# sdu-zyx/Multi-modal-Food-Recommendation

Hardware: NVIDIA B200
Metric: train_epochs_per_s (higher is better)
Workload: dtype f32

## Files before the change

### include/foodrec_b200.h

```cpp
#ifndef FOODREC_B200_H
#define FOODREC_B200_H

#include <stdint.h>

#ifdef __cplusplus
extern "C" {
#endif

#define FR_OK 0
#define FR_EINVAL (-1)
#define FR_EUNSUPPORTED (-2)
#define FR_ECUDA (-3)

#define FR_SPMM_SEG 128

int fr_version(void);
const char *fr_last_error(void);
int64_t fr_launch_count(void);
int fr_profile_enable(int on);
int fr_profile_dump(char *buf, int64_t cap);

int fr_spmm_plan_sizes(const int32_t *row_ptr_host, int32_t n_rows, int32_t seg_len, int64_t *n_seg,
                       int64_t *n_long, int64_t *n_part);
int fr_spmm_plan_fill(const int32_t *row_ptr_host, int32_t n_rows, int32_t seg_len, int32_t *seg_host,
                      int32_t *long_rows_host);
int fr_spmm_csr_f32(const int32_t *seg, int64_t n_seg, const int32_t *long_rows, int64_t n_long,
                    const int32_t *col_idx, const float *val, int32_t d, const float *X, const float *Z,
                    float alpha, float beta, const float *bias, int32_t act, float *Y, float *partial,
                    int32_t *counters, void *stream);

int fr_spmm_csr_f32_split(const int32_t *seg, int64_t n_seg, const int32_t *long_rows, int64_t n_long,
                          const int32_t *col_idx, const float *val, int32_t d, const float *X0, const float *X1,
                          int32_t x_split, const float *Z0, const float *Z1, int32_t z_split, float alpha, float beta,
                          const float *bias, int32_t act, float *Y, float *partial, int32_t *counters, void *stream);

int fr_spmm_csr_f32_masked(const int32_t *seg, int64_t n_seg, const int32_t *long_rows, int64_t n_long,
                           const int32_t *col_idx, const float *val, int32_t d, const float *X, const float *Z,
                           float alpha, float beta, float *Y, float *partial, int32_t *counters, const uint8_t *x_mask,
                           uint8_t *y_mask, void *stream);

#define FR_SPMM_MAX_TASKS 4
typedef struct fr_spmm_task {
    const int32_t *seg;
    int64_t n_seg;
    const int32_t *long_rows;
    int64_t n_long;
    const int32_t *col_idx;
    const float *val;
    const float *X0, *X1;
    int32_t x_split;
    const float *Z0, *Z1;
    int32_t z_split;
    float alpha, beta;
    float *Y, *partial;
    int32_t *counters;
} fr_spmm_task;
int64_t fr_spmm_task_blocks(int64_t n_seg);
int fr_spmm_csr_f32_grouped(const fr_spmm_task *tasks_host, int32_t n_tasks, int32_t d, const int32_t *blk_map,
                            int64_t n_blocks, void *stream);

#define FR_MAX_REG_GROUPS 6
int64_t fr_rank_loss_ws_floats(void);
int fr_rank_loss_fwd(const float *emb, int32_t d, int64_t item_off, const int64_t *u, const int64_t *p,
                     const int64_t *n, int32_t B, float gamma, int32_t n_groups,
                     const float *const *reg_tab_host, const int64_t *const *reg_idx_host,
                     const int64_t *reg_cnt_host, float reg_den, float *out, float *coef, float *gnorm,
                     float *ws, void *stream);
int fr_rank_loss_bwd(const float *emb, int32_t d, int64_t item_off, const int64_t *u, const int64_t *p,
                     const int64_t *n, int32_t B, const float *coef, const float *g_out, float *d_emb,
                     int32_t n_groups, const float *const *reg_tab_host, const int64_t *const *reg_idx_host,
                     const int64_t *reg_cnt_host, const int64_t *reg_pad_host, float reg_den,
                     const float *gnorm, float *const *d_tab_host, uint8_t *emb_mask ,
                     void *stream);

int fr_bpr_scores_fwd(const float *pos, const float *neg, int64_t n, float gamma, float *out, float *coef, void *stream);
int fr_l2_norm_f32(const float *x, int64_t n, float *out, void *stream);

int fr_csr_from_coo(const int64_t *coo_rows, int64_t nnz, int32_t n_rows, int32_t *row_ptr, int32_t *scratch,
                    void *stream);

int fr_sum_rows(const float *const *tab_host, int32_t n_tabs, int32_t d, int64_t rows, float *out, void *stream);
int fr_spread_rows(const float *g, int32_t d, int64_t rows, float *const *d_tab_host, const int64_t *rows_total_host,
                   int32_t n_tabs, int32_t accumulate ,
                   const uint8_t *src_mask ,
                   uint8_t *const *mask_host , void *stream);

int fr_gather_rows(const float *tab, int32_t d, const int64_t *idx, int64_t n, float *out, void *stream);
int fr_scatter_add_rows(const float *g, int32_t d, const int64_t *idx, int64_t n, float *d_tab, void *stream);
int fr_pair_scores(const float *user_tab, const float *item_tab, int32_t d, const int64_t *user,
                   const int64_t *item, int64_t n, float *scores, void *stream);

int64_t fr_dcor_ws_floats(int32_t n);
int fr_dcor_fwd(const float *const *tab_host, int32_t V, int32_t d, const int64_t *idx, int32_t n,
                const int32_t *pairs_host, int32_t P, float scale, float *Dm, float *rowmean, float *out ,
                float *dfds, float *gm, float *ws, void *stream);
int fr_dcor_bwd(const float *const *tab_host, int32_t V, int32_t d, const int64_t *idx, int32_t n,
                const int32_t *pairs_host, int32_t P, const float *Dm, const float *rowmean,
                const float *dfds, const float *gm, const float *g_out, float *const *d_tab_host,
                uint8_t *const *mask_host ,
                float *ws , void *stream);
int64_t fr_dcor_bwd_ws_floats(int32_t n);

int fr_f32_to_bf16(const float *x, void *y_bf16, int64_t rows, int32_t d, int32_t l2_normalise, void *stream);
int64_t fr_gemm_topk_ws_bytes(int32_t M);
int fr_gemm_topk_bf16(const void *A_bf16, int32_t M, const void *B_bf16, int32_t N, int32_t K, float scale,
                      const float *bias, const int64_t *row_ids, const int64_t *hist_ptr, const int32_t *hist_idx,
                      int32_t topk, float *out_val, int32_t *out_idx, void *ws, int64_t ws_bytes, void *stream);
int fr_max_row_norm(const float *B, int64_t rows, int32_t d, float *out , void *stream);
int fr_rescore_topk_f32(const float *A, const int64_t *a_rows, const float *B, int32_t d, float scale,
                        const float *bias, int32_t metric , const int32_t *cand,
                        const float *cand_val, int32_t kc, int32_t M, int32_t k, float *out_val, void *out_idx,
                        int32_t idx64, const float *bmax, uint8_t *cert, void *stream);
int fr_exact_topk_f32(const float *A, const int64_t *a_rows, int32_t Mf, const float *B, int32_t N, int32_t d,
                      float scale, const float *bias, int32_t metric, const int64_t *hist_rows,
                      const int64_t *hist_ptr, const int32_t *hist_idx, int32_t k, float *scores_ws, float *out_val,
                      int64_t *out_idx, void *stream);
int64_t fr_exact_topk_thr_ws_bytes(int32_t Mf);
int fr_exact_topk_thr_f32(const float *A, const int64_t *a_rows, int32_t Mf, const float *B, int32_t N, int32_t d,
                          float scale, const float *bias, int32_t metric, const int64_t *hist_rows,
                          const int64_t *hist_ptr, const int32_t *hist_idx, int32_t k, const float *thr, void *ws,
                          float *out_val, int64_t *out_idx, int32_t *overflow, void *stream);

int fr_cosine_mean_fwd(const float *A, const float *T, const int64_t *idx, int64_t n, int32_t d, float *out, float *cosv,
                       float *na, float *nt, void *stream);
int fr_cosine_mean_bwd(const float *A, const float *T, const int64_t *idx, int64_t n, int32_t d, const float *cosv,
                       const float *na, const float *nt, const float *g_out, float *dA, float *dT, void *stream);

int64_t fr_infonce_ws_floats(int32_t n);
int fr_infonce_fwd(const float *hidden, int32_t b, int32_t d, float temperature, int32_t normalise, float *hn,
                   float *norm, float *G, float *lse, float *out, float *ws, void *stream);
int fr_infonce_bwd(const float *hn, const float *norm, const float *G, const float *lse, int32_t b, int32_t d,
                   float temperature, int32_t normalise, const float *g_out, float *d_hidden, void *stream);

int fr_schgn_attend(const float *user_key, const float *user_comp, int32_t nu, const int32_t *codes, int32_t slots,
                    const int32_t *nums, int32_t n_items, const float *ingre_key, const float *ingre_final,
                    const float *ingre_comp, const float *img_key, const float *comp_keys, const float *h_ingre,
                    const float *h_comp, int32_t d, float *att, float *logits, void *stream);
int fr_schgn_score(const float *user_final, const float *user_hidden, int32_t nu, const float *W_item,
                   const float *W_prod, const float *w_out, const float *comps, const float *att, const float *logits,
                   int32_t n_items, int32_t d, float *scores, void *stream);
int64_t fr_schgn_score_topk_ws_bytes(int32_t nu, int32_t n_items, int32_t k);
int fr_schgn_score_topk(const float *user_final, const float *user_hidden, int32_t nu, const float *W_item,
                        const float *W_prod, const float *w_out, const float *comps, const float *att, const float *logits,
                        int32_t n_items, int32_t d, const int64_t *user_ids, const int64_t *hist_ptr,
                        const int32_t *hist_idx, int32_t k, void *ws, float *out_val, int64_t *out_idx, void *stream);
#define FR_PAIRS_BAD_PTR 1
#define FR_PAIRS_BAD_ITEM 2
int64_t fr_schgn_attend_pairs_ws_bytes(int32_t nu, int64_t n_pairs, int32_t n_items);
int fr_schgn_attend_pairs(const float *user_key, const float *user_comp, int32_t nu, const int64_t *ptr,
                          const int32_t *items, int64_t n_pairs, const int32_t *codes, int32_t slots, const int32_t *nums,
                          int32_t n_items, const float *ingre_key, const float *ingre_final, const float *ingre_comp,
                          const float *img_key, const float *comp_keys, const float *h_ingre, const float *h_comp,
                          int32_t d, void *ws, int64_t ws_bytes, float *att, float *logits, int32_t *status,
                          void *stream);
int fr_schgn_score_pairs(const float *user_final, const float *user_hidden, int32_t nu, const int64_t *ptr,
                         const int32_t *items, int64_t n_pairs, const float *W_item, const float *W_prod,
                         const float *w_out, const float *comps, const float *att, const float *logits, int32_t n_items,
                         int32_t d, float *scores, void *stream);

int fr_comm_version(void);
int fr_comm_unique_id(void *id128);
int fr_comm_init(const void *id128, int32_t rank, int32_t world, void **comm);
int fr_comm_destroy(void *comm);
int fr_allgather_rows(void *comm, const float *x_local, int64_t rows_per_rank, int32_t d, float *x_full, void *stream);
int fr_reduce_scatter_rows(void *comm, const float *g_full, int64_t rows_per_rank, int32_t d, float *g_local, void *stream);
int fr_peer_alloc(int64_t bytes, void **ptr, void *handle64);
int fr_peer_open(const void *handle64, void **ptr);
int fr_peer_close(void *ptr);
int fr_peer_free(void *ptr);
int fr_push_rows(const float *src, int64_t rows, int32_t d, float *const *peers_host, int32_t n_peers, int64_t row_off,
                 void *stream);
int fr_spmm_csr_f32_push(const int32_t *seg, int64_t n_seg, const int32_t *long_rows, int64_t n_long,
                         const int32_t *col_idx, const float *val, int32_t d, const float *X, const float *Z, float alpha,
                         float beta, float *Y, float *partial, int32_t *counters, float *const *peers_host,
                         int32_t n_peers, int64_t row_off, void *stream);

#define FR_ADAM_MAX_TENSORS 64
typedef struct fr_adam_tensor {
    float *param;
    const float *grad;
    float *exp_avg;
    float *exp_avg_sq;
    int64_t n;
} fr_adam_tensor;
int fr_adam_step(const fr_adam_tensor *tensors_host, int32_t n_tensors, double lr, double beta1, double beta2, double eps,
                 int32_t *step_dev, float *scalars_dev, void *stream);

int fr_probe_gather(const float *tab, int32_t d, const int32_t *idx, int64_t n_idx, int32_t inflight, int32_t blocks,
                    float *out, void *stream);

int fr_sample_negatives(const int64_t *excl_ptr, const int32_t *excl_idx, const int64_t *users, int64_t n,
                        int32_t n_items, uint64_t seed, uint64_t step, int64_t *out_neg, int32_t *fail_count,
                        void *stream);

#define FR_EVAL_MAX_CUTOFFS 8
#define FR_TOPK_METRICS 5
int64_t fr_eval_metrics_ws_bytes(void);
int fr_topk_metrics(const void *top, int32_t idx64, int64_t n, int32_t K, const int64_t *pos_ptr, const int32_t *pos_idx,
                    const int32_t *pos_len, const int32_t *cutoffs_host, int32_t n_cut, const float *disc,
                    const float *ideal, double *sums, double *per_user, void *ws, void *stream);
int fr_by_user_metrics(const float *scores, const int64_t *ptr, const int32_t *n_pos, int64_t n, int32_t neg_num,
                       const int32_t *cutoffs_host, int32_t n_cut, double *sums, double *per_user, void *ws,
                       void *stream);

#ifdef __cplusplus
}
#endif
#endif
```

### multi-modal-food-recommendation_b200/_lib.py

```python
from __future__ import annotations

import ctypes as C
import os

_HERE = os.path.dirname(os.path.abspath(__file__))
LIB_PATH = os.path.join(_HERE, "libfoodrec_b200.so")


class FoodRecError(RuntimeError):
    pass


def _load():
    if not os.path.exists(LIB_PATH):
        raise FoodRecError(
            f"{LIB_PATH} is not built: run `make` (or `python -c 'import __graft_entry__ as g; g.build()'`) "
            "at the repo root. foodrec_b200 has no CPU or eager fallback.")
    import torch
    return C.CDLL(LIB_PATH, mode=C.RTLD_GLOBAL)


lib = _load()

_p, _i32, _i64, _f32 = C.c_void_p, C.c_int32, C.c_int64, C.c_float

SIGNATURES = {
    "fr_version": (C.c_int, []),
    "fr_last_error": (C.c_char_p, []),
    "fr_launch_count": (_i64, []),
    "fr_profile_enable": (C.c_int, [C.c_int]),
    "fr_profile_dump": (C.c_int, [C.c_char_p, _i64]),
    "fr_spmm_plan_sizes": (C.c_int, [_p, _i32, _i32, C.POINTER(_i64), C.POINTER(_i64), C.POINTER(_i64)]),
    "fr_spmm_plan_fill": (C.c_int, [_p, _i32, _i32, _p, _p]),
    "fr_spmm_csr_f32": (C.c_int, [_p, _i64, _p, _i64, _p, _p, _i32, _p, _p, _f32, _f32, _p, _i32, _p, _p, _p, _p]),
    "fr_spmm_csr_f32_split": (C.c_int, [_p, _i64, _p, _i64, _p, _p, _i32, _p, _p, _i32, _p, _p, _i32, _f32, _f32, _p, _i32,
                                        _p, _p, _p, _p]),
    "fr_spmm_task_blocks": (_i64, [_i64]),
    "fr_spmm_csr_f32_grouped": (C.c_int, [_p, _i32, _i32, _p, _i64, _p]),
    "fr_adam_step": (C.c_int, [_p, _i32, C.c_double, C.c_double, C.c_double, C.c_double, _p, _p, _p]),
    "fr_rank_loss_ws_floats": (_i64, []),
    "fr_rank_loss_fwd": (C.c_int, [_p, _i32, _i64, _p, _p, _p, _i32, _f32, _i32, _p, _p, _p, _f32, _p, _p, _p, _p, _p]),
    "fr_rank_loss_bwd": (C.c_int, [_p, _i32, _i64, _p, _p, _p, _i32, _p, _p, _p, _i32, _p, _p, _p, _p, _f32, _p, _p, _p, _p]),
    "fr_bpr_scores_fwd": (C.c_int, [_p, _p, _i64, _f32, _p, _p, _p]),
    "fr_l2_norm_f32": (C.c_int, [_p, _i64, _p, _p]),
    "fr_spmm_csr_f32_masked": (C.c_int, [_p, _i64, _p, _i64, _p, _p, _i32, _p, _p, _f32, _f32, _p, _p, _p, _p, _p, _p]),
    "fr_dcor_ws_floats": (_i64, [_i32]),
    "fr_dcor_fwd": (C.c_int, [_p, _i32, _i32, _p, _i32, _p, _i32, _f32, _p, _p, _p, _p, _p, _p, _p]),
    "fr_sum_rows": (C.c_int, [_p, _i32, _i32, _i64, _p, _p]),
    "fr_spread_rows": (C.c_int, [_p, _i32, _i64, _p, _p, _i32, _i32, _p, _p, _p]),
    "fr_dcor_bwd": (C.c_int, [_p, _i32, _i32, _p, _i32, _p, _i32, _p, _p, _p, _p, _p, _p, _p, _p, _p]),
    "fr_dcor_bwd_ws_floats": (_i64, [_i32]),
    "fr_f32_to_bf16": (C.c_int, [_p, _p, _i64, _i32, _i32, _p]),
    "fr_gemm_topk_ws_bytes": (_i64, [_i32]),
    "fr_gemm_topk_bf16": (C.c_int, [_p, _i32, _p, _i32, _i32, _f32, _p, _p, _p, _p, _i32, _p, _p, _p, _i64, _p]),
    "fr_max_row_norm": (C.c_int, [_p, _i64, _i32, _p, _p]),
    "fr_rescore_topk_f32": (C.c_int, [_p, _p, _p, _i32, _f32, _p, _i32, _p, _p, _i32, _i32, _i32, _p, _p, _i32, _p, _p, _p]),
    "fr_exact_topk_f32": (C.c_int, [_p, _p, _i32, _p, _i32, _i32, _f32, _p, _i32, _p, _p, _p, _i32, _p, _p, _p, _p]),
    "fr_exact_topk_thr_ws_bytes": (_i64, [_i32]),
    "fr_exact_topk_thr_f32": (C.c_int, [_p, _p, _i32, _p, _i32, _i32, _f32, _p, _i32, _p, _p, _p, _i32, _p, _p, _p, _p, _p, _p]),
    "fr_csr_from_coo": (C.c_int, [_p, _i64, _i32, _p, _p, _p]),
    "fr_cosine_mean_fwd": (C.c_int, [_p, _p, _p, _i64, _i32, _p, _p, _p, _p, _p]),
    "fr_cosine_mean_bwd": (C.c_int, [_p, _p, _p, _i64, _i32, _p, _p, _p, _p, _p, _p, _p]),
    "fr_infonce_ws_floats": (_i64, [_i32]),
    "fr_infonce_fwd": (C.c_int, [_p, _i32, _i32, _f32, _i32, _p, _p, _p, _p, _p, _p, _p]),
    "fr_infonce_bwd": (C.c_int, [_p, _p, _p, _p, _i32, _i32, _f32, _i32, _p, _p, _p]),
    "fr_gather_rows": (C.c_int, [_p, _i32, _p, _i64, _p, _p]),
    "fr_scatter_add_rows": (C.c_int, [_p, _i32, _p, _i64, _p, _p]),
    "fr_pair_scores": (C.c_int, [_p, _p, _i32, _p, _p, _i64, _p, _p]),
    "fr_comm_version": (C.c_int, []),
    "fr_comm_unique_id": (C.c_int, [_p]),
    "fr_comm_init": (C.c_int, [_p, _i32, _i32, _p]),
    "fr_comm_destroy": (C.c_int, [_p]),
    "fr_allgather_rows": (C.c_int, [_p, _p, _i64, _i32, _p, _p]),
    "fr_reduce_scatter_rows": (C.c_int, [_p, _p, _i64, _i32, _p, _p]),
    "fr_peer_alloc": (C.c_int, [_i64, _p, _p]),
    "fr_peer_open": (C.c_int, [_p, _p]),
    "fr_peer_close": (C.c_int, [_p]),
    "fr_peer_free": (C.c_int, [_p]),
    "fr_push_rows": (C.c_int, [_p, _i64, _i32, _p, _i32, _i64, _p]),
    "fr_spmm_csr_f32_push": (C.c_int, [_p, _i64, _p, _i64, _p, _p, _i32, _p, _p, _f32, _f32, _p, _p, _p, _p, _i32, _i64, _p]),
    "fr_probe_gather": (C.c_int, [_p, _i32, _p, _i64, _i32, _i32, _p, _p]),
    "fr_sample_negatives": (C.c_int, [_p, _p, _p, _i64, _i32, C.c_uint64, C.c_uint64, _p, _p, _p]),
    "fr_schgn_attend": (C.c_int, [_p, _p, _i32, _p, _i32, _p, _i32, _p, _p, _p, _p, _p, _p, _p, _i32, _p, _p, _p]),
    "fr_schgn_score": (C.c_int, [_p, _p, _i32, _p, _p, _p, _p, _p, _p, _i32, _i32, _p, _p]),
    "fr_schgn_score_topk_ws_bytes": (_i64, [_i32, _i32, _i32]),
    "fr_schgn_score_topk": (C.c_int, [_p, _p, _i32, _p, _p, _p, _p, _p, _p, _i32, _i32, _p, _p, _p, _i32, _p, _p, _p, _p]),
    "fr_schgn_attend_pairs_ws_bytes": (_i64, [_i32, _i64, _i32]),
    "fr_schgn_attend_pairs": (C.c_int, [_p, _p, _i32, _p, _p, _i64, _p, _i32, _p, _i32, _p, _p, _p, _p, _p, _p, _p, _i32,
                                        _p, _i64, _p, _p, _p, _p]),
    "fr_schgn_score_pairs": (C.c_int, [_p, _p, _i32, _p, _p, _i64, _p, _p, _p, _p, _p, _p, _i32, _i32, _p, _p]),
    "fr_eval_metrics_ws_bytes": (_i64, []),
    "fr_topk_metrics": (C.c_int, [_p, _i32, _i64, _i32, _p, _p, _p, _p, _i32, _p, _p, _p, _p, _p, _p]),
    "fr_by_user_metrics": (C.c_int, [_p, _p, _p, _i64, _i32, _p, _i32, _p, _p, _p, _p]),
}

class SpmmTask(C.Structure):
    _fields_ = [("seg", _p), ("n_seg", _i64), ("long_rows", _p), ("n_long", _i64), ("col_idx", _p), ("val", _p),
                ("X0", _p), ("X1", _p), ("x_split", _i32), ("Z0", _p), ("Z1", _p), ("z_split", _i32),
                ("alpha", _f32), ("beta", _f32), ("Y", _p), ("partial", _p), ("counters", _p)]


class AdamTensor(C.Structure):
    _fields_ = [("param", _p), ("grad", _p), ("exp_avg", _p), ("exp_avg_sq", _p), ("n", _i64)]


for _name, (_res, _args) in SIGNATURES.items():
    _fn = getattr(lib, _name)
    _fn.restype = _res
    _fn.argtypes = _args


def check(rc: int, what: str = ""):
    if rc != 0:
        msg = lib.fr_last_error().decode("utf-8", "replace")
        raise FoodRecError(f"{what or 'foodrec_b200'} failed (rc={rc}): {msg}")


def ptr(t):
    if t is None:
        return None
    if hasattr(t, "data_ptr"):
        return t.data_ptr()
    return t.ctypes.data


def stream_ptr():
    import torch
    return torch.cuda.current_stream().cuda_stream


def launch_count() -> int:
    return int(lib.fr_launch_count())


class kernel_profile:

    def __enter__(self):
        lib.fr_profile_dump(None, 0)
        lib.fr_profile_enable(1)
        self.result = {}
        return self

    def __exit__(self, *exc):
        lib.fr_profile_enable(0)
        buf = C.create_string_buffer(1 << 16)
        lib.fr_profile_dump(buf, len(buf))
        for line in buf.value.decode().splitlines():
            name, n, us = line.rsplit(",", 2)
            self.result[name] = (int(n), float(us))
        return False
```

### multi-modal-food-recommendation_b200/csrc/dcor.cu

```cuda
#include "common.cuh"

namespace {

constexpr int kMaxV = 3;
constexpr int kMaxP = 3;
constexpr int kThreads = 256;
constexpr int kRB2 = 4;
constexpr int kMaxD = 128;
constexpr float kEpsD = 1e-8f;

struct Views {
    const float *tab[kMaxV];
    float *dtab[kMaxV];
    unsigned char *mask[kMaxV];
    int V;
};
struct Pairs {
    int a[kMaxP], b[kMaxP];
    int P;
};

__device__ __forceinline__ float block_sum(float v, float *sh) {
    v = fr::warp_sum(v);
    const int lane = threadIdx.x & 31, w = threadIdx.x >> 5;
    __syncthreads();
    if (lane == 0) sh[w] = v;
    __syncthreads();
    float t = 0.f;
    for (int i = 0; i < kThreads / 32; ++i) t += sh[i];
    return t;
}

__device__ __forceinline__ double block_sum_d(double v, double *sh) {
#pragma unroll
    for (int o = 16; o > 0; o >>= 1) v += __shfl_xor_sync(0xffffffffu, v, o);
    const int lane = threadIdx.x & 31, w = threadIdx.x >> 5;
    __syncthreads();
    if (lane == 0) sh[w] = v;
    __syncthreads();
    double t = 0.0;
    for (int i = 0; i < kThreads / 32; ++i) t += sh[i];
    return t;
}

constexpr int kT = 64;
template <int D>
__global__ void __launch_bounds__(kThreads)
dcor_dist_kernel(Views vw, const int64_t *__restrict__ idx, int n, float *__restrict__ Dm,
                 float *__restrict__ rowpart, int n_tiles) {
    __shared__ __align__(16) float Xi[D][kT + 4];
    __shared__ __align__(16) float Xj[D][kT + 4];
    const int v = blockIdx.z;
    const float *__restrict__ tab = vw.tab[v];
    const int i0 = blockIdx.y * kT, j0 = blockIdx.x * kT;
    for (int t = threadIdx.x; t < kT * D; t += kThreads) {
        const int r = t / D, k = t - r * D;
        Xi[k][r] = (i0 + r < n) ? __ldg(tab + (size_t)idx[i0 + r] * D + k) : 0.f;
        Xj[k][r] = (j0 + r < n) ? __ldg(tab + (size_t)idx[j0 + r] * D + k) : 0.f;
    }
    __syncthreads();
    const int ty = threadIdx.x >> 4, tx = threadIdx.x & 15;
    float acc[4][4], ri[4] = {0.f, 0.f, 0.f, 0.f}, rj[4] = {0.f, 0.f, 0.f, 0.f};
#pragma unroll
    for (int a = 0; a < 4; ++a)
#pragma unroll
        for (int b = 0; b < 4; ++b) acc[a][b] = 0.f;
#pragma unroll 8
    for (int k = 0; k < D; ++k) {
        const float4 av = *reinterpret_cast<const float4 *>(&Xi[k][ty * 4]);
        const float4 bv = *reinterpret_cast<const float4 *>(&Xj[k][tx * 4]);
        const float a4[4] = {av.x, av.y, av.z, av.w}, b4[4] = {bv.x, bv.y, bv.z, bv.w};
#pragma unroll
        for (int a = 0; a < 4; ++a) {
            ri[a] = fmaf(a4[a], a4[a], ri[a]);
            rj[a] = fmaf(b4[a], b4[a], rj[a]);
#pragma unroll
            for (int b = 0; b < 4; ++b) acc[a][b] = fmaf(a4[a], b4[b], acc[a][b]);
        }
    }
    float *__restrict__ Dv = Dm + (size_t)v * n * n;
#pragma unroll
    for (int a = 0; a < 4; ++a) {
        const int i = i0 + ty * 4 + a;
        float d4[4], rs = 0.f;
#pragma unroll
        for (int b = 0; b < 4; ++b) {
            const float m = (ri[a] - 2.f * acc[a][b]) + rj[b];
            d4[b] = sqrtf(fmaxf(m, 0.f) + kEpsD);
            if (j0 + tx * 4 + b < n) rs += d4[b];
        }
        if (i < n) {
            if (j0 + tx * 4 + 3 < n && (n & 3) == 0)
                *reinterpret_cast<float4 *>(Dv + (size_t)i * n + j0 + tx * 4) = make_float4(d4[0], d4[1], d4[2], d4[3]);
            else
                for (int b = 0; b < 4; ++b)
                    if (j0 + tx * 4 + b < n) Dv[(size_t)i * n + j0 + tx * 4 + b] = d4[b];
        }
        rs += __shfl_xor_sync(0xffffffffu, rs, 8);
        rs += __shfl_xor_sync(0xffffffffu, rs, 4);
        rs += __shfl_xor_sync(0xffffffffu, rs, 2);
        rs += __shfl_xor_sync(0xffffffffu, rs, 1);
        if (tx == 0 && i < n) rowpart[((size_t)v * n_tiles + blockIdx.x) * n + i] = rs;
    }
}

__global__ void dcor_rowmean_kernel(const float *__restrict__ rowpart, int n, int n_tiles, int V,
                                    float *__restrict__ rowmean, double *__restrict__ rowmean64) {
    const int i = blockIdx.x * blockDim.x + threadIdx.x;
    const int v = blockIdx.y;
    if (i >= n) return;
    double s = 0.0;
    for (int t = 0; t < n_tiles; ++t) s += (double)rowpart[((size_t)v * n_tiles + t) * n + i];
    s /= (double)n;
    rowmean64[(size_t)v * n + i] = s;
    rowmean[(size_t)v * n + i] = (float)s;
}

__global__ void __launch_bounds__(kThreads)
dcor_dot_kernel(int V, Pairs pr, int n, const float *__restrict__ Dm, const double *__restrict__ rowmean,
                float *__restrict__ out, float *__restrict__ dfds, float *__restrict__ gm_out,
                float *__restrict__ ws, float scale) {
    __shared__ double red[kThreads / 32];
    __shared__ double gm[kMaxV];
    __shared__ double fin[6];
    __shared__ int last;
    double *__restrict__ part = reinterpret_cast<double *>(ws + 8);
    for (int v = 0; v < V; ++v) {
        double s = 0.0;
        for (int j = threadIdx.x; j < n; j += kThreads) s += rowmean[(size_t)v * n + j];
        s = block_sum_d(s, red);
        if (threadIdx.x == 0) gm[v] = s / (double)n;
    }
    __syncthreads();
    double acc[6] = {0.0, 0.0, 0.0, 0.0, 0.0, 0.0};
    const int i0 = blockIdx.x * kRB2;
    for (int r = 0; r < kRB2 && i0 + r < n; ++r) {
        const int i = i0 + r;
        double rmi[kMaxV];
        for (int v = 0; v < kMaxV; ++v) rmi[v] = v < V ? rowmean[(size_t)v * n + i] : 0.0;
#pragma unroll 4
        for (int j = threadIdx.x; j < n; j += kThreads) {
            double A[kMaxV];
#pragma unroll
            for (int v = 0; v < kMaxV; ++v)
                A[v] = v < V ? ((((double)__ldg(Dm + ((size_t)v * n + i) * n + j) - rowmean[(size_t)v * n + j]) - rmi[v]) + gm[v])
                             : 0.0;
            acc[0] = fma(A[0], A[0], acc[0]);
            acc[1] = fma(A[0], A[1], acc[1]);
            acc[2] = fma(A[0], A[2], acc[2]);
            acc[3] = fma(A[1], A[1], acc[3]);
            acc[4] = fma(A[1], A[2], acc[4]);
            acc[5] = fma(A[2], A[2], acc[5]);
        }
    }
    for (int q = 0; q < 6; ++q) {
        const double s = block_sum_d(acc[q], red);
        if (threadIdx.x == 0) __stcg(part + (size_t)blockIdx.x * 8 + q, s);
    }
    __threadfence();
    __syncthreads();
    if (threadIdx.x == 0) last = (atomicAdd(reinterpret_cast<int *>(ws), 1) == (int)gridDim.x - 1);
    __syncthreads();
    if (!last) return;
    __threadfence();
    if (threadIdx.x < 6) {
        double s = 0.0;
        for (unsigned b = 0; b < gridDim.x; ++b) s += __ldcg(part + (size_t)b * 8 + threadIdx.x);
        fin[threadIdx.x] = s / ((double)n * (double)n);
    }
    __syncthreads();
    if (threadIdx.x == 0) {
        auto S = [&](int a, int b) -> double {
            if (a > b) { const int t = a; a = b; b = t; }
            return fin[a * 3 + b - (a * (a + 1)) / 2];
        };
        double total = 0.0;
        for (int p = 0; p < pr.P; ++p) {
            const int a = pr.a[p], b = pr.b[p];
            const double sab = S(a, b), saa = S(a, a), sbb = S(b, b);
            const double cab = sqrt(fmax(sab, 0.0) + 1e-8);
            const double caa = sqrt(fmax(saa, 0.0) + 1e-8);
            const double cbb = sqrt(fmax(sbb, 0.0) + 1e-8);
            const double q = sqrt(fmax(caa * cbb, 0.0) + 1e-10);
            const double o = (double)scale * (cab / q);
            out[p] = (float)o;
            total += o;
            const double dq = -cab / (2.0 * q * q * q);
            dfds[p * 3 + 0] = sab > 0.0 ? (float)((double)scale / (2.0 * cab * q)) : 0.f;
            dfds[p * 3 + 1] = saa > 0.0 ? (float)((double)scale * dq * cbb / (2.0 * caa)) : 0.f;
            dfds[p * 3 + 2] = sbb > 0.0 ? (float)((double)scale * dq * caa / (2.0 * cbb)) : 0.f;
        }
        out[pr.P] = (float)total;
        for (int v = 0; v < V; ++v) gm_out[v] = (float)gm[v];
        *reinterpret_cast<int *>(ws) = 0;
    }
}

__global__ void __launch_bounds__(kThreads)
dcor_w_kernel(int V, Pairs pr, int n, const float *__restrict__ Dm, const float *__restrict__ rowmean,
              const float *__restrict__ gm, const float *__restrict__ dfds, const float *__restrict__ g_out,
              float *__restrict__ W, float *__restrict__ wsum) {
    __shared__ float Cm[kMaxV][kMaxV];
    __shared__ float gms[kMaxV];
    __shared__ float red[kThreads / 32];
    if (threadIdx.x == 0) {
        float c[kMaxV][kMaxV] = {};
        const float inv = 1.f / ((float)n * (float)n);
        for (int p = 0; p < pr.P; ++p) {
            const float g = __ldg(g_out + p);
            const int a = pr.a[p], b = pr.b[p];
            c[a][b] += g * dfds[p * 3 + 0] * inv;
            c[a][a] += 2.f * g * dfds[p * 3 + 1] * inv;
            c[b][a] += g * dfds[p * 3 + 0] * inv;
            c[b][b] += 2.f * g * dfds[p * 3 + 2] * inv;
        }
        for (int v = 0; v < kMaxV; ++v) {
            gms[v] = v < V ? gm[v] : 0.f;
            for (int w = 0; w < kMaxV; ++w) Cm[v][w] = c[v][w];
        }
    }
    __syncthreads();
    const float eps_d = sqrtf(kEpsD);
    const int i0 = blockIdx.x * kRB2;
    for (int r = 0; r < kRB2 && i0 + r < n; ++r) {
        const int i = i0 + r;
        float rmi[kMaxV], ws[kMaxV] = {0.f, 0.f, 0.f};
#pragma unroll
        for (int u = 0; u < kMaxV; ++u) rmi[u] = u < V ? __ldg(rowmean + (size_t)u * n + i) : 0.f;
#pragma unroll 2
        for (int j = threadIdx.x; j < n; j += kThreads) {
            float d[kMaxV], A[kMaxV];
#pragma unroll
            for (int u = 0; u < kMaxV; ++u) {
                d[u] = u < V ? __ldg(Dm + ((size_t)u * n + i) * n + j) : 1.f;
                A[u] = u < V ? ((d[u] - __ldg(rowmean + (size_t)u * n + j)) - rmi[u]) + gms[u] : 0.f;
            }
#pragma unroll
            for (int v = 0; v < kMaxV; ++v) {
                if (v < V) {
                    float g = 0.f;
#pragma unroll
                    for (int u = 0; u < kMaxV; ++u) g = fmaf(Cm[v][u], A[u], g);
                    const float w = (i != j && d[v] > eps_d) ? g / (2.f * d[v]) : 0.f;
                    W[((size_t)v * n + i) * n + j] = w;
                    ws[v] += w;
                }
            }
        }
        for (int v = 0; v < V; ++v) {
            const float t = block_sum(ws[v], red);
            if (threadIdx.x == 0) wsum[(size_t)v * n + i] = t;
        }
    }
}

template <int D>
__global__ void __launch_bounds__(kThreads)
dcor_wx_kernel(Views vw, const int64_t *__restrict__ idx, int n, const float *__restrict__ W,
               const float *__restrict__ wsum) {
    constexpr int RB = 32, JT = 32, KQ = D / 4;
    constexpr int RPT = RB * KQ / kThreads;
    static_assert(RB * KQ % kThreads == 0 && RB * JT == 4 * kThreads && JT * KQ <= 2 * kThreads, "tile/threads mismatch");
    __shared__ __align__(16) float Ws[2][RB][JT + 4];
    __shared__ __align__(16) float Xs[2][JT][D];
    const int v = blockIdx.y;
    float *__restrict__ dtab = vw.dtab[v];
    if (dtab == nullptr) return;
    const float *__restrict__ tab = vw.tab[v];
    const float *__restrict__ Wv = W + (size_t)v * n * n;
    const int i0 = blockIdx.x * RB;
    const int jt_total = (n + JT - 1) / JT, jt_per = (jt_total + gridDim.z - 1) / gridDim.z;
    const int jt_lo = blockIdx.z * jt_per, jt_hi = min(jt_total, jt_lo + jt_per);
    const int okq = threadIdx.x % KQ, orow = (threadIdx.x / KQ) * RPT;
    const int wr = threadIdx.x / (JT / 4), wc = (threadIdx.x % (JT / 4)) * 4;
    float4 wreg, xreg[2];
    auto fetch = [&](int jt) {
        const int j0 = jt * JT;
        const int i = i0 + wr;
        wreg = make_float4(0.f, 0.f, 0.f, 0.f);
        if (i < n) {
            if (j0 + wc + 3 < n && (n & 3) == 0) wreg = fr::ldg_f4(Wv + (size_t)i * n + j0 + wc);
            else {
                float t[4] = {0.f, 0.f, 0.f, 0.f};
                for (int e = 0; e < 4; ++e)
                    if (j0 + wc + e < n) t[e] = __ldg(Wv + (size_t)i * n + j0 + wc + e);
                wreg = make_float4(t[0], t[1], t[2], t[3]);
            }
        }
#pragma unroll
        for (int e = 0; e < 2; ++e) {
            const int t = threadIdx.x + e * kThreads;
            xreg[e] = make_float4(0.f, 0.f, 0.f, 0.f);
            if (t < JT * KQ) {
                const int r = t / KQ, q = t % KQ;
                if (j0 + r < n) xreg[e] = fr::ldg_f4(tab + (size_t)__ldg(idx + j0 + r) * D + 4 * q);
            }
        }
    };
    auto stash = [&](int buf) {
        *reinterpret_cast<float4 *>(&Ws[buf][wr][wc]) = wreg;
#pragma unroll
        for (int e = 0; e < 2; ++e) {
            const int t = threadIdx.x + e * kThreads;
            if (t < JT * KQ) *reinterpret_cast<float4 *>(&Xs[buf][t / KQ][4 * (t % KQ)]) = xreg[e];
        }
    };
    float4 acc[RPT];
#pragma unroll
    for (int a = 0; a < RPT; ++a) acc[a] = make_float4(0.f, 0.f, 0.f, 0.f);
    if (jt_lo < jt_hi) {
        fetch(jt_lo);
        stash(0);
        __syncthreads();
        for (int jt = jt_lo; jt < jt_hi; ++jt) {
            const int buf = (jt - jt_lo) & 1;
            if (jt + 1 < jt_hi) fetch(jt + 1);
#pragma unroll 8
            for (int c = 0; c < JT; ++c) {
                const float4 x = *reinterpret_cast<const float4 *>(&Xs[buf][c][4 * okq]);
#pragma unroll
                for (int a = 0; a < RPT; ++a) fr::fma4(acc[a], Ws[buf][orow + a][c], x);
            }
            if (jt + 1 < jt_hi) stash(buf ^ 1);
            __syncthreads();
        }
    }
#pragma unroll
    for (int a = 0; a < RPT; ++a) {
        const int i = i0 + orow + a;
        if (i >= n) continue;
        const size_t row = (size_t)__ldg(idx + i);
        float4 o = make_float4(-4.f * acc[a].x, -4.f * acc[a].y, -4.f * acc[a].z, -4.f * acc[a].w);
        if (blockIdx.z == 0) {
            const float w4 = 4.f * __ldg(wsum + (size_t)v * n + i);
            const float4 xi = fr::ldg_f4(tab + row * D + 4 * okq);
            o.x = fmaf(w4, xi.x, o.x);
            o.y = fmaf(w4, xi.y, o.y);
            o.z = fmaf(w4, xi.z, o.z);
            o.w = fmaf(w4, xi.w, o.w);
            if (vw.mask[v] != nullptr && okq == 0) vw.mask[v][row] = 1;
        }
        atomicAdd(reinterpret_cast<float4 *>(dtab + row * D + 4 * okq), o);
    }
}

int fill(Views &vw, Pairs &pr, int V, const float *const *tab, float *const *dtab, int P, const int32_t *pairs) {
    FR_REQUIRE(V >= 1 && V <= kMaxV && P >= 1 && P <= kMaxP && tab && pairs, "dcor: V=%d P=%d out of range", V, P);
    vw.V = V;
    for (int v = 0; v < kMaxV; ++v) {
        vw.tab[v] = v < V ? tab[v] : nullptr;
        vw.dtab[v] = (v < V && dtab) ? dtab[v] : nullptr;
        vw.mask[v] = nullptr;
        FR_REQUIRE(v >= V || tab[v], "dcor: null view table %d", v);
    }
    pr.P = P;
    for (int p = 0; p < kMaxP; ++p) {
        pr.a[p] = p < P ? pairs[2 * p] : 0;
        pr.b[p] = p < P ? pairs[2 * p + 1] : 0;
        FR_REQUIRE(p >= P || (pr.a[p] >= 0 && pr.a[p] < V && pr.b[p] >= 0 && pr.b[p] < V && pr.a[p] != pr.b[p]),
                   "dcor: pair %d out of range", p);
    }
    return FR_OK;
}

}

static int64_t dot_blocks(int n) { return (n + kRB2 - 1) / kRB2; }
static int64_t rm64_off(int n) { return 8 + 16 * dot_blocks(n); }
static int64_t rowpart_off(int n) { return rm64_off(n) + 2 * (int64_t)kMaxV * n; }
extern "C" int64_t fr_dcor_ws_floats(int32_t n) {
    return rowpart_off(n) + (int64_t)kMaxV * ((n + kT - 1) / kT) * n;
}

extern "C" int fr_dcor_fwd(const float *const *tab_host, int32_t V, int32_t d, const int64_t *idx, int32_t n,
                           const int32_t *pairs_host, int32_t P, float scale, float *Dm, float *rowmean, float *out,
                           float *dfds, float *gm, float *ws, void *stream) {
    FR_REQUIRE(idx && Dm && rowmean && out && dfds && gm && ws && n > 0, "fr_dcor_fwd: bad argument");
    Views vw;
    Pairs pr;
    if (int rc = fill(vw, pr, V, tab_host, nullptr, P, pairs_host)) return rc;
    cudaStream_t st = (cudaStream_t)stream;
    const int n_tiles = (n + kT - 1) / kT;
    FR_REQUIRE(((uintptr_t)ws & 7) == 0, "fr_dcor_fwd: workspace must be 8-byte aligned");
    float *rowpart = ws + rowpart_off(n);
    double *rowmean64 = reinterpret_cast<double *>(ws + rm64_off(n));
    dim3 g1(n_tiles, n_tiles, V);
    {
    fr::LaunchTimer _lt("dcor_dist_kernel", st);
    if (d == 64) dcor_dist_kernel<64><<<g1, kThreads, 0, st>>>(vw, idx, n, Dm, rowpart, n_tiles);
    else if (d == 32) dcor_dist_kernel<32><<<g1, kThreads, 0, st>>>(vw, idx, n, Dm, rowpart, n_tiles);
    else {
        fr::set_error("fr_dcor_fwd: d=%d unsupported (32, 64)", d);
        return FR_EUNSUPPORTED;
    }
    }
    if (int rc = fr::check_launch("fr_dcor_fwd/dist")) return rc;
    dcor_rowmean_kernel<<<dim3((n + 255) / 256, V), 256, 0, st>>>(rowpart, n, n_tiles, V, rowmean, rowmean64);
    if (int rc = fr::check_launch("fr_dcor_fwd/rowmean")) return rc;
    fr::LaunchTimer _lt2("dcor_dot_kernel", st);
    dcor_dot_kernel<<<(n + kRB2 - 1) / kRB2, kThreads, 0, st>>>(V, pr, n, Dm, rowmean64, out, dfds, gm, ws, scale);
    return fr::check_launch("fr_dcor_fwd/dot");
}

extern "C" int64_t fr_dcor_bwd_ws_floats(int32_t n) { return (int64_t)kMaxV * n * n + (int64_t)kMaxV * n; }

extern "C" int fr_dcor_bwd(const float *const *tab_host, int32_t V, int32_t d, const int64_t *idx, int32_t n,
                           const int32_t *pairs_host, int32_t P, const float *Dm, const float *rowmean,
                           const float *dfds, const float *gm, const float *g_out, float *const *d_tab_host,
                           uint8_t *const *mask_host, float *ws, void *stream) {
    FR_REQUIRE(idx && Dm && rowmean && dfds && gm && g_out && d_tab_host && ws && n > 0, "fr_dcor_bwd: bad argument");
    FR_REQUIRE(((uintptr_t)ws & 15) == 0, "fr_dcor_bwd: workspace must be 16-byte aligned");
    Views vw;
    Pairs pr;
    if (int rc = fill(vw, pr, V, tab_host, d_tab_host, P, pairs_host)) return rc;
    for (int v = 0; v < V; ++v)
        FR_REQUIRE(vw.dtab[v] == nullptr || ((uintptr_t)vw.dtab[v] & 15) == 0, "fr_dcor_bwd: gradient tables must be 16-byte aligned");
    if (mask_host)
        for (int v = 0; v < V; ++v) vw.mask[v] = mask_host[v];
    cudaStream_t st = (cudaStream_t)stream;
    float *W = ws, *wsum = ws + (size_t)kMaxV * n * n;
    {
        fr::LaunchTimer _lt("dcor_w_kernel", st);
        dcor_w_kernel<<<(n + kRB2 - 1) / kRB2, kThreads, 0, st>>>(V, pr, n, Dm, rowmean, gm, dfds, g_out, W, wsum);
        if (int rc = fr::check_launch("fr_dcor_bwd/w")) return rc;
    }
    dim3 g((n + 31) / 32, V, 8);
    fr::LaunchTimer _lt("dcor_wx_kernel", st);
    if (d == 64) dcor_wx_kernel<64><<<g, kThreads, 0, st>>>(vw, idx, n, W, wsum);
    else if (d == 32) dcor_wx_kernel<32><<<g, kThreads, 0, st>>>(vw, idx, n, W, wsum);
    else {
        fr::set_error("fr_dcor_bwd: d=%d unsupported (32, 64)", d);
        return FR_EUNSUPPORTED;
    }
    return fr::check_launch("fr_dcor_bwd");
}
```

### multi-modal-food-recommendation_b200/csrc/gather.cu

```cuda
#include "common.cuh"

namespace {

__global__ void gather_rows_kernel(const float *__restrict__ tab, int d4, const int64_t *__restrict__ idx,
                                   long long n, float *__restrict__ out) {
    const long long total = n * d4;
    for (long long i = (long long)blockIdx.x * blockDim.x + threadIdx.x; i < total;
         i += (long long)gridDim.x * blockDim.x) {
        const long long r = i / d4;
        const int c = (int)(i - r * d4);
        reinterpret_cast<float4 *>(out)[i] = fr::ldg_f4(tab + ((size_t)idx[r] * d4 + c) * 4);
    }
}

__global__ void scatter_add_rows_kernel(const float *__restrict__ g, int d, const int64_t *__restrict__ idx,
                                        long long n, float *__restrict__ d_tab) {
    const long long total = n * d;
    for (long long i = (long long)blockIdx.x * blockDim.x + threadIdx.x; i < total;
         i += (long long)gridDim.x * blockDim.x) {
        const long long r = i / d;
        const int c = (int)(i - r * d);
        atomicAdd(d_tab + (size_t)idx[r] * d + c, __ldg(g + i));
    }
}

__global__ void pair_scores_kernel(const float *__restrict__ ut, const float *__restrict__ it, int d,
                                   const int64_t *__restrict__ user, const int64_t *__restrict__ item, long long n,
                                   float *__restrict__ scores) {
    const int lane = threadIdx.x & 31;
    const long long w = ((long long)blockIdx.x * blockDim.x + threadIdx.x) >> 5;
    if (w >= n) return;
    const float *a = ut + (size_t)user[w] * d, *b = it + (size_t)item[w] * d;
    float s = 0.f;
    for (int k = lane; k < d; k += 32) s = fmaf(__ldg(a + k), __ldg(b + k), s);
    s = fr::warp_sum(s);
    if (lane == 0) scores[w] = s;
}

int grid1d(long long work, int block) {
    long long b = (work + block - 1) / block;
    return (int)std::max<long long>(1, std::min<long long>(b, (long long)fr::num_sms() * 16));
}

}

extern "C" int fr_gather_rows(const float *tab, int32_t d, const int64_t *idx, int64_t n, float *out, void *stream) {
    FR_REQUIRE(n >= 0 && d > 0 && d % 4 == 0, "fr_gather_rows: n=%lld d=%d (d must be a multiple of 4)", (long long)n, d);
    if (n == 0) return FR_OK;
    FR_REQUIRE(tab && idx && out, "fr_gather_rows: null pointer");
    fr::LaunchTimer _lt("gather_rows_kernel", (cudaStream_t)stream);
    gather_rows_kernel<<<grid1d(n * (d / 4), 256), 256, 0, (cudaStream_t)stream>>>(tab, d / 4, idx, n, out);
    return fr::check_launch("fr_gather_rows");
}

extern "C" int fr_scatter_add_rows(const float *g, int32_t d, const int64_t *idx, int64_t n, float *d_tab,
                                   void *stream) {
    FR_REQUIRE(n >= 0 && d > 0, "fr_scatter_add_rows: n=%lld d=%d", (long long)n, d);
    if (n == 0) return FR_OK;
    FR_REQUIRE(g && idx && d_tab, "fr_scatter_add_rows: null pointer");
    fr::LaunchTimer _lt("scatter_add_rows_kernel", (cudaStream_t)stream);
    scatter_add_rows_kernel<<<grid1d(n * d, 256), 256, 0, (cudaStream_t)stream>>>(g, d, idx, n, d_tab);
    return fr::check_launch("fr_scatter_add_rows");
}

extern "C" int fr_pair_scores(const float *user_tab, const float *item_tab, int32_t d, const int64_t *user,
                              const int64_t *item, int64_t n, float *scores, void *stream) {
    FR_REQUIRE(n >= 0 && d > 0, "fr_pair_scores: n=%lld d=%d", (long long)n, d);
    if (n == 0) return FR_OK;
    FR_REQUIRE(user_tab && item_tab && user && item && scores, "fr_pair_scores: null pointer");
    const long long blocks = (n * 32 + 255) / 256;
    fr::LaunchTimer _lt("pair_scores_kernel", (cudaStream_t)stream);
    pair_scores_kernel<<<(unsigned)blocks, 256, 0, (cudaStream_t)stream>>>(user_tab, item_tab, d, user, item, n, scores);
    return fr::check_launch("fr_pair_scores");
}

namespace {
__global__ void coo_count_kernel(const int64_t *__restrict__ rows, long long nnz, int *__restrict__ cnt) {
    for (long long i = (long long)blockIdx.x * blockDim.x + threadIdx.x; i < nnz; i += (long long)gridDim.x * blockDim.x)
        atomicAdd(cnt + rows[i], 1);
}
__global__ void scan_rows_kernel(const int *__restrict__ cnt, int n, int *__restrict__ row_ptr) {
    __shared__ int carry;
    __shared__ int buf[1024];
    if (threadIdx.x == 0) { carry = 0; row_ptr[0] = 0; }
    __syncthreads();
    for (int base = 0; base < n; base += 1024) {
        const int i = base + threadIdx.x;
        buf[threadIdx.x] = i < n ? cnt[i] : 0;
        __syncthreads();
        for (int o = 1; o < 1024; o <<= 1) {
            const int v = threadIdx.x >= o ? buf[threadIdx.x - o] : 0;
            __syncthreads();
            buf[threadIdx.x] += v;
            __syncthreads();
        }
        if (i < n) row_ptr[i + 1] = carry + buf[threadIdx.x];
        __syncthreads();
        if (threadIdx.x == 1023) carry += buf[1023];
        __syncthreads();
    }
}
}

extern "C" int fr_csr_from_coo(const int64_t *coo_rows, int64_t nnz, int32_t n_rows, int32_t *row_ptr, int32_t *scratch,
                               void *stream) {
    FR_REQUIRE(nnz >= 0 && n_rows >= 0, "fr_csr_from_coo: nnz=%lld n_rows=%d", (long long)nnz, n_rows);
    FR_REQUIRE(row_ptr && scratch && (nnz == 0 || coo_rows), "fr_csr_from_coo: null pointer");
    cudaStream_t st = (cudaStream_t)stream;
    cudaMemsetAsync(scratch, 0, sizeof(int32_t) * (size_t)std::max(n_rows, 1), st);
    if (nnz > 0) {
        coo_count_kernel<<<grid1d(nnz, 256), 256, 0, st>>>(coo_rows, nnz, scratch);
        if (int rc = fr::check_launch("fr_csr_from_coo/count")) return rc;
    }
    scan_rows_kernel<<<1, 1024, 0, st>>>(scratch, n_rows, row_ptr);
    return fr::check_launch("fr_csr_from_coo/scan");
}


namespace {
struct Tabs4 {
    const float *in[4];
    float *out[4];
    unsigned char *mask[4];
    long long rows_total[4];
    int n;
};
__global__ void sum_rows_kernel(Tabs4 t, long long n4, float *__restrict__ out) {
    for (long long i = (long long)blockIdx.x * blockDim.x + threadIdx.x; i < n4; i += (long long)gridDim.x * blockDim.x) {
        float4 a = fr::ldg_f4(t.in[0] + 4 * i);
        for (int v = 1; v < t.n; ++v) fr::add4(a, fr::ldg_f4(t.in[v] + 4 * i));
        reinterpret_cast<float4 *>(out)[i] = a;
    }
}
__global__ void spread_rows_kernel(Tabs4 t, long long n4_src, const float *__restrict__ g, int accumulate,
                                   const unsigned char *__restrict__ src_mask, int d4) {
    const int v = blockIdx.y;
    float4 *dst = reinterpret_cast<float4 *>(t.out[v]);
    if (dst == nullptr) return;
    if (t.mask[v] != nullptr) {
        const long long rows_src = n4_src / d4, rows_tot = t.rows_total[v] / d4;
        for (long long r = (long long)blockIdx.x * blockDim.x + threadIdx.x; r < (accumulate ? rows_src : rows_tot);
             r += (long long)gridDim.x * blockDim.x) {
            const unsigned char m = r < rows_src ? (src_mask ? src_mask[r] : (unsigned char)1) : (unsigned char)0;
            if (accumulate) { if (m) t.mask[v][r] = 1; }
            else t.mask[v][r] = m;
        }
    }
    if (accumulate) {
        for (long long i = (long long)blockIdx.x * blockDim.x + threadIdx.x; i < n4_src; i += (long long)gridDim.x * blockDim.x) {
            float4 a = dst[i];
            fr::add4(a, fr::ldg_f4(g + 4 * i));
            dst[i] = a;
        }
        return;
    }
    const long long tot4 = t.rows_total[v];
    for (long long i = (long long)blockIdx.x * blockDim.x + threadIdx.x; i < tot4; i += (long long)gridDim.x * blockDim.x)
        dst[i] = i < n4_src ? fr::ldg_f4(g + 4 * i) : make_float4(0.f, 0.f, 0.f, 0.f);
}
}

extern "C" int fr_sum_rows(const float *const *tab_host, int32_t n_tabs, int32_t d, int64_t rows, float *out, void *stream) {
    FR_REQUIRE(n_tabs >= 1 && n_tabs <= 4 && d > 0 && d % 4 == 0 && rows >= 0 && tab_host && out, "fr_sum_rows: bad argument");
    if (rows == 0) return FR_OK;
    Tabs4 t{};
    t.n = n_tabs;
    for (int v = 0; v < n_tabs; ++v) {
        FR_REQUIRE(tab_host[v], "fr_sum_rows: null table %d", v);
        t.in[v] = tab_host[v];
    }
    const long long n4 = rows * (d / 4);
    fr::LaunchTimer _lt("sum_rows_kernel", (cudaStream_t)stream);
    sum_rows_kernel<<<grid1d(n4, 256), 256, 0, (cudaStream_t)stream>>>(t, n4, out);
    return fr::check_launch("fr_sum_rows");
}

extern "C" int fr_spread_rows(const float *g, int32_t d, int64_t rows, float *const *d_tab_host, const int64_t *rows_total_host,
                              int32_t n_tabs, int32_t accumulate, const uint8_t *src_mask, uint8_t *const *mask_host,
                              void *stream) {
    FR_REQUIRE(n_tabs >= 1 && n_tabs <= 4 && d > 0 && d % 4 == 0 && rows >= 0 && g && d_tab_host && rows_total_host,
               "fr_spread_rows: bad argument");
    Tabs4 t{};
    t.n = n_tabs;
    long long mx = 0;
    for (int v = 0; v < n_tabs; ++v) {
        FR_REQUIRE(rows_total_host[v] >= rows, "fr_spread_rows: table %d shorter than the source", v);
        t.out[v] = d_tab_host[v];
        t.mask[v] = mask_host ? mask_host[v] : nullptr;
        t.rows_total[v] = rows_total_host[v] * (d / 4);
        mx = std::max(mx, t.rows_total[v]);
    }
    if (mx == 0) return FR_OK;
    fr::LaunchTimer _lt("spread_rows_kernel", (cudaStream_t)stream);
    spread_rows_kernel<<<dim3(grid1d(mx, 256), n_tabs), 256, 0, (cudaStream_t)stream>>>(t, rows * (d / 4), g, accumulate, src_mask, d / 4);
    return fr::check_launch("fr_spread_rows");
}

namespace {
__global__ void cosine_mean_fwd_kernel(const float *__restrict__ A, const float *__restrict__ T, const int64_t *__restrict__ idx,
                                       long long n, int d, float *__restrict__ cosv, float *__restrict__ na, float *__restrict__ nt) {
    const int lane = threadIdx.x & 31;
    const long long i = ((long long)blockIdx.x * blockDim.x + threadIdx.x) >> 5;
    if (i >= n) return;
    const float *a = A + (size_t)i * d, *t = T + (size_t)idx[i] * d;
    float dot = 0.f, sa = 0.f, st = 0.f;
    for (int k = lane; k < d; k += 32) {
        const float x = a[k], y = __ldg(t + k);
        dot = fmaf(x, y, dot);
        sa = fmaf(x, x, sa);
        st = fmaf(y, y, st);
    }
    dot = fr::warp_sum(dot);
    sa = fr::warp_sum(sa);
    st = fr::warp_sum(st);
    if (lane == 0) {
        const float x = fmaxf(sqrtf(sa), 1e-8f), y = fmaxf(sqrtf(st), 1e-8f);
        na[i] = x;
        nt[i] = y;
        cosv[i] = dot / (x * y);
    }
}
__global__ void mean_kernel(const float *__restrict__ v, long long n, float *__restrict__ out) {
    __shared__ float red[32];
    float s = 0.f;
    for (long long i = threadIdx.x; i < n; i += blockDim.x) s += v[i];
    s = fr::warp_sum(s);
    if ((threadIdx.x & 31) == 0) red[threadIdx.x >> 5] = s;
    __syncthreads();
    if (threadIdx.x == 0) {
        float t = 0.f;
        for (int w = 0; w < (int)(blockDim.x >> 5); ++w) t += red[w];
        out[0] = t / (float)n;
    }
}
__global__ void cosine_mean_bwd_kernel(const float *__restrict__ A, const float *__restrict__ T, const int64_t *__restrict__ idx,
                                       long long n, int d, const float *__restrict__ cosv, const float *__restrict__ na,
                                       const float *__restrict__ nt, const float *__restrict__ g_out, float *__restrict__ dA,
                                       float *__restrict__ dT) {
    const int lane = threadIdx.x & 31;
    const long long i = ((long long)blockIdx.x * blockDim.x + threadIdx.x) >> 5;
    if (i >= n) return;
    const size_t ao = (size_t)i * d, to = (size_t)idx[i] * d;
    const float g = __ldg(g_out) / (float)n, c = cosv[i], x = na[i], y = nt[i];
    const bool ax = x > 1e-8f, ty = y > 1e-8f;
    for (int k = lane; k < d; k += 32) {
        const float a = A[ao + k], t = __ldg(T + to + k);
        if (dA != nullptr) dA[ao + k] = g * (t / (x * y) - (ax ? c * a / (x * x) : 0.f));
        if (dT != nullptr) atomicAdd(dT + to + k, g * (a / (x * y) - (ty ? c * t / (y * y) : 0.f)));
    }
}
}

extern "C" int fr_cosine_mean_fwd(const float *A, const float *T, const int64_t *idx, int64_t n, int32_t d, float *out,
                                  float *cosv, float *na, float *nt, void *stream) {
    FR_REQUIRE(A && T && idx && out && cosv && na && nt && n > 0 && d > 0, "fr_cosine_mean_fwd: bad argument");
    cudaStream_t st = (cudaStream_t)stream;
    {
        fr::LaunchTimer _lt("cosine_mean_fwd_kernel", st);
        cosine_mean_fwd_kernel<<<(unsigned)((n * 32 + 255) / 256), 256, 0, st>>>(A, T, idx, n, d, cosv, na, nt);
    }
    if (int rc = fr::check_launch("fr_cosine_mean_fwd")) return rc;
    mean_kernel<<<1, 1024, 0, st>>>(cosv, n, out);
    return fr::check_launch("fr_cosine_mean_fwd/mean");
}

extern "C" int fr_cosine_mean_bwd(const float *A, const float *T, const int64_t *idx, int64_t n, int32_t d, const float *cosv,
                                  const float *na, const float *nt, const float *g_out, float *dA, float *dT, void *stream) {
    FR_REQUIRE(A && T && idx && cosv && na && nt && g_out && n > 0 && d > 0, "fr_cosine_mean_bwd: bad argument");
    fr::LaunchTimer _lt("cosine_mean_bwd_kernel", (cudaStream_t)stream);
    cosine_mean_bwd_kernel<<<(unsigned)((n * 32 + 255) / 256), 256, 0, (cudaStream_t)stream>>>(A, T, idx, n, d, cosv, na, nt,
                                                                                              g_out, dA, dT);
    return fr::check_launch("fr_cosine_mean_bwd");
}
```

### multi-modal-food-recommendation_b200/csrc/rank_loss.cu

```cuda
#include "common.cuh"

namespace {

constexpr int kWarps = 8;

struct Groups {
    const float *tab[FR_MAX_REG_GROUPS];
    const int64_t *idx[FR_MAX_REG_GROUPS];
    float *dtab[FR_MAX_REG_GROUPS];
    long long start[FR_MAX_REG_GROUPS + 1];
    long long pad[FR_MAX_REG_GROUPS];
    int n;
};

__device__ __forceinline__ float dot_rows(const float *__restrict__ a, const float *__restrict__ b, int d, int lane) {
    float s = 0.f;
    for (int k = lane; k < d; k += 32) s = fmaf(__ldg(a + k), __ldg(b + k), s);
    return s;
}

__global__ void __launch_bounds__(kWarps * 32)
rank_loss_fwd_kernel(const float *__restrict__ emb, int d, long long item_off, const int64_t *__restrict__ u,
                     const int64_t *__restrict__ p, const int64_t *__restrict__ n, int B, float gamma, Groups g,
                     float reg_den, float *__restrict__ out, float *__restrict__ coef, float *__restrict__ gnorm,
                     float *__restrict__ ws) {
    __shared__ float sh[kWarps][1 + FR_MAX_REG_GROUPS];
    __shared__ int last;
    const int lane = threadIdx.x & 31, wib = threadIdx.x >> 5;
    const long long n_tasks = B + g.start[g.n];
    const long long warps_total = (long long)gridDim.x * kWarps;
    float part[1 + FR_MAX_REG_GROUPS];
#pragma unroll
    for (int i = 0; i <= FR_MAX_REG_GROUPS; ++i) part[i] = 0.f;

    for (long long t = (long long)blockIdx.x * kWarps + wib; t < n_tasks; t += warps_total) {
        if (t < B) {
            const float *ue = emb + (size_t)u[t] * d;
            const float *pe = emb + (size_t)(item_off + p[t]) * d;
            const float *ne = emb + (size_t)(item_off + n[t]) * d;
            float x = 0.f;
            for (int k = lane; k < d; k += 32) {
                const float uv = __ldg(ue + k);
                x = fmaf(uv, __ldg(pe + k) - __ldg(ne + k), x);
            }
            x = fr::warp_sum(x);
            const float sg = 1.f / (1.f + expf(-x));
            part[0] += -logf(gamma + sg);
            if (lane == 0) coef[t] = -(sg * (1.f - sg)) / ((gamma + sg) * (float)B);
        } else {
            const long long q = t - B;
            int gi = 0;
#pragma unroll
            for (int i = 1; i < FR_MAX_REG_GROUPS; ++i)
                if (i < g.n && q >= g.start[i]) gi = i;
            const long long id = g.idx[gi][q - g.start[gi]];
            const float *row = g.tab[gi] + (size_t)id * d;
            const float s = fr::warp_sum(dot_rows(row, row, d, lane));
#pragma unroll
            for (int i = 0; i < FR_MAX_REG_GROUPS; ++i)
                if (i == gi) part[1 + i] += s;
        }
    }
    if (lane == 0) {
#pragma unroll
        for (int i = 0; i <= FR_MAX_REG_GROUPS; ++i) sh[wib][i] = part[i];
    }
    __syncthreads();
    if (threadIdx.x <= FR_MAX_REG_GROUPS) {
        float s = 0.f;
        for (int w = 0; w < kWarps; ++w) s += sh[w][threadIdx.x];
        __stcg(ws + 8 + (size_t)blockIdx.x * 8 + threadIdx.x, s);
    }
    __threadfence();
    __syncthreads();
    if (threadIdx.x == 0) last = (atomicAdd(reinterpret_cast<int *>(ws), 1) == (int)gridDim.x - 1);
    __syncthreads();
    if (!last) return;
    __threadfence();
    if (threadIdx.x <= FR_MAX_REG_GROUPS) {
        float s = 0.f;
        for (unsigned b = 0; b < gridDim.x; ++b) s += __ldcg(ws + 8 + (size_t)b * 8 + threadIdx.x);
        sh[0][threadIdx.x] = s;
    }
    __syncthreads();
    if (threadIdx.x == 0) {
        out[0] = sh[0][0] / (float)B;
        float r = 0.f;
        for (int i = 0; i < g.n; ++i) {
            const float nr = sqrtf(sh[0][1 + i]);
            gnorm[i] = nr;
            r += nr;
        }
        out[1] = r / reg_den;
        *reinterpret_cast<int *>(ws) = 0;
    }
}

__global__ void __launch_bounds__(kWarps * 32)
rank_loss_bwd_kernel(const float *__restrict__ emb, int d, long long item_off, const int64_t *__restrict__ u,
                     const int64_t *__restrict__ p, const int64_t *__restrict__ n, int B,
                     const float *__restrict__ coef, const float *__restrict__ g_out, float *__restrict__ d_emb,
                     Groups g, float reg_den, const float *__restrict__ gnorm, unsigned char *__restrict__ emb_mask) {
    const int lane = threadIdx.x & 31, wib = threadIdx.x >> 5;
    const long long n_tasks = B + g.start[g.n];
    const long long warps_total = (long long)gridDim.x * kWarps;
    const float g_mf = __ldg(g_out), g_reg = __ldg(g_out + 1);
    for (long long t = (long long)blockIdx.x * kWarps + wib; t < n_tasks; t += warps_total) {
        if (t < B) {
            if (d_emb == nullptr) continue;
            const size_t ur = (size_t)u[t] * d, pr = (size_t)(item_off + p[t]) * d, nr = (size_t)(item_off + n[t]) * d;
            const float c = coef[t] * g_mf;
            if (emb_mask != nullptr && lane < 3)
                emb_mask[lane == 0 ? u[t] : (item_off + (lane == 1 ? p[t] : n[t]))] = 1;
            for (int k = lane; k < d; k += 32) {
                const float uv = __ldg(emb + ur + k), pv = __ldg(emb + pr + k), nv = __ldg(emb + nr + k);
                atomicAdd(d_emb + ur + k, c * (pv - nv));
                atomicAdd(d_emb + pr + k, c * uv);
                atomicAdd(d_emb + nr + k, -c * uv);
            }
        } else {
            const long long q = t - B;
            int gi = 0;
#pragma unroll
            for (int i = 1; i < FR_MAX_REG_GROUPS; ++i)
                if (i < g.n && q >= g.start[i]) gi = i;
            if (g.dtab[gi] == nullptr) continue;
            const long long id = g.idx[gi][q - g.start[gi]];
            if (id == g.pad[gi]) continue;
            const float nr = __ldg(gnorm + gi);
            const float sc = nr > 0.f ? g_reg / (reg_den * nr) : 0.f;
            const float *row = g.tab[gi] + (size_t)id * d;
            float *drow = g.dtab[gi] + (size_t)id * d;
            for (int k = lane; k < d; k += 32) atomicAdd(drow + k, sc * __ldg(row + k));
        }
    }
}

__global__ void __launch_bounds__(1024)
bpr_scores_kernel(const float *__restrict__ pos, const float *__restrict__ neg, long long n, float gamma,
                  float *__restrict__ out, float *__restrict__ coef) {
    __shared__ float sh[32];
    float s = 0.f;
    for (long long i = threadIdx.x; i < n; i += blockDim.x) {
        const float x = pos[i] - neg[i];
        const float sg = 1.f / (1.f + expf(-x));
        s += -logf(gamma + sg);
        coef[i] = -(sg * (1.f - sg)) / ((gamma + sg) * (float)n);
    }
    s = fr::warp_sum(s);
    if ((threadIdx.x & 31) == 0) sh[threadIdx.x >> 5] = s;
    __syncthreads();
    if (threadIdx.x < 32) {
        s = fr::warp_sum(threadIdx.x < (blockDim.x >> 5) ? sh[threadIdx.x] : 0.f);
        if (threadIdx.x == 0) out[0] = s / (float)n;
    }
}

__global__ void __launch_bounds__(1024)
l2_norm_kernel(const float *__restrict__ x, long long n, float *__restrict__ out) {
    __shared__ float sh[32];
    float s = 0.f;
    for (long long i = threadIdx.x; i < n; i += blockDim.x) s = fmaf(x[i], x[i], s);
    s = fr::warp_sum(s);
    if ((threadIdx.x & 31) == 0) sh[threadIdx.x >> 5] = s;
    __syncthreads();
    if (threadIdx.x < 32) {
        s = fr::warp_sum(threadIdx.x < (blockDim.x >> 5) ? sh[threadIdx.x] : 0.f);
        if (threadIdx.x == 0) out[0] = sqrtf(s);
    }
}

int fill_groups(Groups &g, int n_groups, const float *const *tab, const int64_t *const *idx, const int64_t *cnt,
                const int64_t *pad, float *const *dtab) {
    FR_REQUIRE(n_groups >= 0 && n_groups <= FR_MAX_REG_GROUPS, "rank_loss: n_groups=%d out of range", n_groups);
    g.n = n_groups;
    g.start[0] = 0;
    for (int i = 0; i < FR_MAX_REG_GROUPS; ++i) {
        const bool on = i < n_groups;
        FR_REQUIRE(!on || (tab[i] && cnt[i] >= 0 && (idx[i] || cnt[i] == 0)), "rank_loss: bad regulariser group %d", i);
        g.tab[i] = on ? tab[i] : nullptr;
        g.idx[i] = on ? idx[i] : nullptr;
        g.dtab[i] = (on && dtab) ? dtab[i] : nullptr;
        g.pad[i] = (on && pad) ? pad[i] : -1;
        g.start[i + 1] = g.start[i] + (on ? cnt[i] : 0);
    }
    return FR_OK;
}

int grid_for(long long n_tasks) {
    long long b = (n_tasks + kWarps - 1) / kWarps;
    const long long cap = (long long)fr::num_sms() * 4;
    return (int)std::max<long long>(1, std::min(b, cap));
}

}

extern "C" int64_t fr_rank_loss_ws_floats(void) { return 8 + 8 * (int64_t)fr::num_sms() * 4; }

extern "C" int fr_rank_loss_fwd(const float *emb, int32_t d, int64_t item_off, const int64_t *u, const int64_t *p,
                                const int64_t *n, int32_t B, float gamma, int32_t n_groups,
                                const float *const *reg_tab_host, const int64_t *const *reg_idx_host,
                                const int64_t *reg_cnt_host, float reg_den, float *out, float *coef, float *gnorm,
                                float *ws, void *stream) {
    FR_REQUIRE(emb && u && p && n && out && coef && gnorm && ws, "fr_rank_loss_fwd: null pointer");
    FR_REQUIRE(B > 0 && d > 0, "fr_rank_loss_fwd: B=%d d=%d", B, d);
    Groups g;
    if (int rc = fill_groups(g, n_groups, reg_tab_host, reg_idx_host, reg_cnt_host, nullptr, nullptr)) return rc;
    const int grid = grid_for(B + g.start[g.n]);
    fr::LaunchTimer _lt("rank_loss_fwd_kernel", (cudaStream_t)stream);
    rank_loss_fwd_kernel<<<grid, kWarps * 32, 0, (cudaStream_t)stream>>>(emb, d, item_off, u, p, n, B, gamma, g,
                                                                         reg_den, out, coef, gnorm, ws);
    return fr::check_launch("fr_rank_loss_fwd");
}

extern "C" int fr_rank_loss_bwd(const float *emb, int32_t d, int64_t item_off, const int64_t *u, const int64_t *p,
                                const int64_t *n, int32_t B, const float *coef, const float *g_out, float *d_emb,
                                int32_t n_groups, const float *const *reg_tab_host,
                                const int64_t *const *reg_idx_host, const int64_t *reg_cnt_host,
                                const int64_t *reg_pad_host, float reg_den, const float *gnorm,
                                float *const *d_tab_host, uint8_t *emb_mask, void *stream) {
    FR_REQUIRE(emb && u && p && n && coef && g_out && gnorm, "fr_rank_loss_bwd: null pointer");
    FR_REQUIRE(B > 0 && d > 0, "fr_rank_loss_bwd: B=%d d=%d", B, d);
    Groups g;
    if (int rc = fill_groups(g, n_groups, reg_tab_host, reg_idx_host, reg_cnt_host, reg_pad_host, d_tab_host))
        return rc;
    const int grid = grid_for(B + g.start[g.n]);
    fr::LaunchTimer _lt("rank_loss_bwd_kernel", (cudaStream_t)stream);
    rank_loss_bwd_kernel<<<grid, kWarps * 32, 0, (cudaStream_t)stream>>>(emb, d, item_off, u, p, n, B, coef, g_out,
                                                                         d_emb, g, reg_den, gnorm, emb_mask);
    return fr::check_launch("fr_rank_loss_bwd");
}

extern "C" int fr_bpr_scores_fwd(const float *pos, const float *neg, int64_t n, float gamma, float *out, float *coef,
                                 void *stream) {
    FR_REQUIRE(pos && neg && out && coef, "fr_bpr_scores_fwd: null pointer");
    FR_REQUIRE(n > 0, "fr_bpr_scores_fwd: n=%lld", (long long)n);
    fr::LaunchTimer _lt("bpr_scores_kernel", (cudaStream_t)stream);
    bpr_scores_kernel<<<1, 1024, 0, (cudaStream_t)stream>>>(pos, neg, n, gamma, out, coef);
    return fr::check_launch("fr_bpr_scores_fwd");
}

extern "C" int fr_l2_norm_f32(const float *x, int64_t n, float *out, void *stream) {
    FR_REQUIRE(x && out, "fr_l2_norm_f32: null pointer");
    FR_REQUIRE(n > 0, "fr_l2_norm_f32: n=%lld", (long long)n);
    fr::LaunchTimer _lt("l2_norm_kernel", (cudaStream_t)stream);
    l2_norm_kernel<<<1, 1024, 0, (cudaStream_t)stream>>>(x, n, out);
    return fr::check_launch("fr_l2_norm_f32");
}
```

### multi-modal-food-recommendation_b200/csrc/spmm.cu

```cuda
#include <stdlib.h>

#include <algorithm>
#include <vector>

#include "common.cuh"

namespace {

constexpr int kWarpsPerBlock = 8;
#ifndef FR_GROUP_MIN_BLOCKS
#define FR_GROUP_MIN_BLOCKS 4
#endif

struct Split {
    const float *X1_adj;
    int x_split;
    const float *Z1_adj;
    int z_split;
    const unsigned char *x_mask;
    unsigned char *y_mask;
    float *peer[8];
    int n_peers;
    long long row_off;
};

template <int D, int ACT, bool PUSH = false>
__device__ __forceinline__ bool epilogue_store(float4 acc, int row, int off, const float *__restrict__ Z,
                                               float alpha, float beta, const float *__restrict__ bias,
                                               float *__restrict__ Y, const Split *sp = nullptr) {
    float4 y = make_float4(alpha * acc.x, alpha * acc.y, alpha * acc.z, alpha * acc.w);
    const size_t o = (size_t)row * D + off;
    if (Z != nullptr) {
        const float4 z = fr::ldg_f4(Z + o);
        y.x = fmaf(beta, z.x, y.x);
        y.y = fmaf(beta, z.y, y.y);
        y.z = fmaf(beta, z.z, y.z);
        y.w = fmaf(beta, z.w, y.w);
    }
    if (bias != nullptr) {
        const float4 b = fr::ldg_f4(bias + off);
        fr::add4(y, b);
    }
    if (ACT == 1) {
        y.x = tanhf(y.x);
        y.y = tanhf(y.y);
        y.z = tanhf(y.z);
        y.w = tanhf(y.w);
    }
    if (!PUSH || Y != nullptr) *reinterpret_cast<float4 *>(Y + o) = y;
    if (PUSH) {
        const size_t po = (size_t)(sp->row_off + row) * D + off;
#pragma unroll
        for (int q = 0; q < 8; ++q)
            if (q < sp->n_peers) *reinterpret_cast<float4 *>(sp->peer[q] + po) = y;
    }
    return (y.x != 0.f) | (y.y != 0.f) | (y.z != 0.f) | (y.w != 0.f);
}

template <int D, int LPR, int U, int ACT, bool SPLIT, bool MASKED, bool PUSH = false>
__device__ __forceinline__ void
spmm_group_body(const long long w, const int4 *__restrict__ seg, long long n_seg, const int4 *__restrict__ long_rows,
                const int *__restrict__ col, const float *__restrict__ val, const float *__restrict__ X,
                const float *__restrict__ Z, float alpha, float beta, const float *__restrict__ bias,
                float *__restrict__ Y, float *__restrict__ partial, int *__restrict__ counters, const Split &sp) {
    constexpr int G = 32 / LPR, VPL = D / (4 * LPR);
    static_assert(VPL >= 1 && LPR % U == 0, "bad group shape");
    if (w * G >= n_seg) return;
    const int lane = threadIdx.x & 31;
    const int g = lane / LPR, lg = lane % LPR;
    const long long sidx = w * G + g;
    int4 s = make_int4(0, 0, 0, -2);
    if (sidx < n_seg) s = __ldg(seg + sidx);
    int maxlen = s.z;
#pragma unroll
    for (int o = 16; o >= LPR; o >>= 1) maxlen = max(maxlen, __shfl_xor_sync(0xffffffffu, maxlen, o));
    const int *__restrict__ cp = col + s.y;
    const float *__restrict__ vp = val + s.y;
    const float *__restrict__ Xo = X + lg * 4;
    const float *__restrict__ X1o = sp.X1_adj + lg * 4;

    float4 acc[VPL];
#pragma unroll
    for (int t = 0; t < VPL; ++t) acc[t] = make_float4(0.f, 0.f, 0.f, 0.f);
    for (int base = 0; base < maxlen; base += LPR) {
        const int cnt = max(0, min(LPR, s.z - base));
        int c = 0;
        float v = 0.f;
        if (lg < cnt) {
            c = __ldg(cp + base + lg);
            v = __ldg(vp + base + lg);
            if (MASKED && sp.x_mask[c] == 0) c = -1;
        }
        const int lim = min(LPR, maxlen - base);
        for (int j = 0; j < lim; j += U) {
            float4 x[U][VPL];
            float vv[U];
#pragma unroll
            for (int u = 0; u < U; ++u) {
                const int e = j + u;
                const int cj = __shfl_sync(0xffffffffu, c, e, LPR);
                vv[u] = __shfl_sync(0xffffffffu, v, e, LPR);
                const float *xr = ((!SPLIT || cj < sp.x_split) ? Xo : X1o) + (size_t)cj * D;
                if (e < cnt && (!MASKED || cj >= 0)) {
#pragma unroll
                    for (int t = 0; t < VPL; ++t) x[u][t] = fr::ldg_f4(xr + 4 * LPR * t);
                } else {
                    vv[u] = 0.f;
#pragma unroll
                    for (int t = 0; t < VPL; ++t) x[u][t] = make_float4(0.f, 0.f, 0.f, 0.f);
                }
            }
#pragma unroll
            for (int u = 0; u < U; ++u)
#pragma unroll
                for (int t = 0; t < VPL; ++t) fr::fma4(acc[t], vv[u], x[u][t]);
        }
    }
    if (s.w == -2) return;
    const unsigned gmask = (LPR == 32) ? 0xffffffffu : (((1u << LPR) - 1u) << (g * LPR));
    if (s.w < 0) {
        bool nz = false;
#pragma unroll
        for (int t = 0; t < VPL; ++t)
            nz |= epilogue_store<D, ACT, PUSH>(acc[t], s.x, 4 * (lg + LPR * t),
                                               (Z != nullptr && s.x >= sp.z_split) ? sp.Z1_adj : Z, alpha, beta, bias, Y, &sp);
        if (sp.y_mask != nullptr) {
            nz = __any_sync(gmask, nz);
            if (lg == 0) sp.y_mask[s.x] = nz ? 1 : 0;
        }
        return;
    }
    int id = s.w;
    int4 lr = __ldg(long_rows + id);
    int slot = s.x;
    for (;;) {
#pragma unroll
        for (int t = 0; t < VPL; ++t)
            __stcg(reinterpret_cast<float4 *>(partial + ((size_t)lr.z + slot) * D + 4 * (lg + LPR * t)), acc[t]);
        __threadfence();
        __syncwarp(gmask);
        int ticket = 0;
        if (lg == 0) ticket = atomicAdd(counters + id, 1);
        ticket = __shfl_sync(gmask, ticket, g * LPR);
        if (ticket != lr.y - 1) return;
        __threadfence();
#pragma unroll
        for (int t = 0; t < VPL; ++t) {
            float4 tot = make_float4(0.f, 0.f, 0.f, 0.f);
            const float *pp = partial + (size_t)lr.z * D + 4 * (lg + LPR * t);
            int k = 0;
            for (; k + 8 <= lr.y; k += 8) {
                float4 p8[8];
#pragma unroll
                for (int u = 0; u < 8; ++u) p8[u] = fr::ldcg_f4(pp + (size_t)(k + u) * D);
#pragma unroll
                for (int u = 0; u < 8; ++u) fr::add4(tot, p8[u]);
            }
            for (; k < lr.y; ++k) fr::add4(tot, fr::ldcg_f4(pp + (size_t)k * D));
            acc[t] = tot;
        }
        if (lg == 0) counters[id] = 0;
        if (lr.w >= 0) break;
        const int parent = -lr.w - 1;
        const int4 pr = __ldg(long_rows + parent);
        slot = id - pr.x;
        id = parent;
        lr = pr;
    }
    bool nz_long = false;
#pragma unroll
    for (int t = 0; t < VPL; ++t)
        nz_long |= epilogue_store<D, ACT, PUSH>(acc[t], lr.w, 4 * (lg + LPR * t),
                                                (Z != nullptr && lr.w >= sp.z_split) ? sp.Z1_adj : Z, alpha, beta, bias, Y, &sp);
    if (sp.y_mask != nullptr) {
        nz_long = __any_sync(gmask, nz_long);
        if (lg == 0) sp.y_mask[lr.w] = nz_long ? 1 : 0;
    }
}

template <int D, int LPR, int U, int ACT, bool SPLIT, bool MASKED, bool PUSH = false>
__global__ void __launch_bounds__(kWarpsPerBlock * 32, FR_GROUP_MIN_BLOCKS)
spmm_group_kernel(const int4 *__restrict__ seg, long long n_seg, const int4 *__restrict__ long_rows,
                  const int *__restrict__ col, const float *__restrict__ val, const float *__restrict__ X,
                  const float *__restrict__ Z, float alpha, float beta, const float *__restrict__ bias,
                  float *__restrict__ Y, float *__restrict__ partial, int *__restrict__ counters, Split sp) {
    const long long w = ((long long)blockIdx.x * blockDim.x + threadIdx.x) >> 5;
    spmm_group_body<D, LPR, U, ACT, SPLIT, MASKED, PUSH>(w, seg, n_seg, long_rows, col, val, X, Z, alpha, beta, bias, Y, partial,
                                                         counters, sp);
}

struct GroupedTask {
    const int4 *seg;
    long long n_seg;
    const int4 *long_rows;
    const int *col;
    const float *val;
    const float *X, *X1_adj, *Z, *Z1_adj;
    float *Y, *partial;
    int *counters;
    int x_split, z_split;
    float alpha, beta;
};
struct GroupedParams {
    GroupedTask t[FR_SPMM_MAX_TASKS];
};

template <int D>
__global__ void __launch_bounds__(kWarpsPerBlock * 32, FR_GROUP_MIN_BLOCKS)
spmm_grouped_kernel(const __grid_constant__ GroupedParams P, const int2 *__restrict__ blk_map) {
    const int2 m = __ldg(blk_map + blockIdx.x);
    const GroupedTask &T = P.t[m.x];
    Split sp;
    sp.X1_adj = T.X1_adj;
    sp.x_split = T.x_split;
    sp.Z1_adj = T.Z1_adj;
    sp.z_split = T.z_split;
    sp.x_mask = nullptr;
    sp.y_mask = nullptr;
    sp.n_peers = 0;
    sp.row_off = 0;
    const long long w = (long long)m.y * kWarpsPerBlock + (threadIdx.x >> 5);
    spmm_group_body<D, 8, 4, 0, true, false, false>(w, T.seg, T.n_seg, T.long_rows, T.col, T.val, T.X, T.Z, T.alpha, T.beta,
                                                    nullptr, T.Y, T.partial, T.counters, sp);
}

template <int D, int LPR, int U, int ACT>
int launch_group_shape(const int4 *seg, int64_t n_seg, const int4 *lrows, const int *col, const float *val,
                       const float *X, const float *Z, float alpha, float beta, const float *bias, float *Y,
                       float *partial, int *counters, cudaStream_t st, Split sp) {
    constexpr int G = 32 / LPR;
    const long long warps = (n_seg + G - 1) / G;
    const long long blocks = (warps + kWarpsPerBlock - 1) / kWarpsPerBlock;
    if (blocks > 0x7fffffffLL) {
        fr::set_error("fr_spmm_csr_f32: too many segments (%lld)", (long long)n_seg);
        return FR_EUNSUPPORTED;
    }
    fr::LaunchTimer _lt("spmm_group_kernel", st);
    if (sp.n_peers > 0) {
        if constexpr (ACT == 0 && LPR == 8 && U == 4) {
            spmm_group_kernel<D, LPR, U, 0, false, false, true><<<(unsigned)blocks, kWarpsPerBlock * 32, 0, st>>>(
                seg, n_seg, lrows, col, val, X, Z, alpha, beta, bias, Y, partial, counters, sp);
            return fr::check_launch("fr_spmm_csr_f32_push");
        } else {
            fr::set_error("fr_spmm_csr_f32_push: needs act = 0 and the default kernel shape");
            return FR_EUNSUPPORTED;
        }
    }
    if (sp.x_split != 0x7fffffff)
        spmm_group_kernel<D, LPR, U, ACT, true, false><<<(unsigned)blocks, kWarpsPerBlock * 32, 0, st>>>(
            seg, n_seg, lrows, col, val, X, Z, alpha, beta, bias, Y, partial, counters, sp);
    else if (sp.x_mask != nullptr)
        spmm_group_kernel<D, LPR, U, ACT, false, true><<<(unsigned)blocks, kWarpsPerBlock * 32, 0, st>>>(
            seg, n_seg, lrows, col, val, X, Z, alpha, beta, bias, Y, partial, counters, sp);
    else
        spmm_group_kernel<D, LPR, U, ACT, false, false><<<(unsigned)blocks, kWarpsPerBlock * 32, 0, st>>>(
            seg, n_seg, lrows, col, val, X, Z, alpha, beta, bias, Y, partial, counters, sp);
    return fr::check_launch("fr_spmm_csr_f32(group)");
}

template <int D>
int launch(const int4 *seg, int64_t n_seg, const int4 *lrows, const int *col, const float *val, const float *X,
           const float *Z, float alpha, float beta, const float *bias, int act, float *Y, float *partial,
           int *counters, cudaStream_t st, Split sp) {
    if (act == 0) return launch_group_shape<D, 8, 4, 0>(seg, n_seg, lrows, col, val, X, Z, alpha, beta, bias, Y, partial, counters, st, sp);
    return launch_group_shape<D, 8, 4, 1>(seg, n_seg, lrows, col, val, X, Z, alpha, beta, bias, Y, partial, counters, st, sp);
}

struct PlanCounts {
    int64_t n_seg = 0, n_long = 0, n_part = 0;
};

constexpr int64_t kFlatFold = 16;
struct FoldShape {
    int64_t per, children;
};
FoldShape fold_shape(int64_t k) {
    if (k <= kFlatFold) return {k, 0};
    int64_t per = 1;
    while (per * per < k) ++per;
    return {per, (k + per - 1) / per};
}

PlanCounts count_plan(const int32_t *rp, int32_t n_rows, int64_t SEG) {
    PlanCounts c;
    for (int32_t r = 0; r < n_rows; ++r) {
        const int64_t deg = (int64_t)rp[r + 1] - rp[r];
        const int64_t k = deg <= SEG ? 1 : (deg + SEG - 1) / SEG;
        c.n_seg += k;
        if (k > 1) {
            const FoldShape f = fold_shape(k);
            c.n_long += f.children ? f.children + 1 : 1;
            c.n_part += k + f.children;
        }
    }
    return c;
}

}

extern "C" int fr_spmm_plan_sizes(const int32_t *row_ptr_host, int32_t n_rows, int32_t seg_len, int64_t *n_seg,
                                  int64_t *n_long, int64_t *n_part) {
    FR_REQUIRE(row_ptr_host && n_seg && n_long && n_part && n_rows >= 0, "fr_spmm_plan_sizes: bad argument");
    FR_REQUIRE(seg_len >= 8 && seg_len <= FR_SPMM_SEG, "fr_spmm_plan_sizes: seg_len=%d outside [8, %d]", seg_len, FR_SPMM_SEG);
    for (int32_t r = 0; r < n_rows; ++r)
        FR_REQUIRE(row_ptr_host[r + 1] >= row_ptr_host[r], "fr_spmm_plan_sizes: row_ptr not monotone at %d", r);
    const PlanCounts c = count_plan(row_ptr_host, n_rows, seg_len);
    FR_REQUIRE(c.n_long <= 0x7fffffffLL && c.n_part <= 0x7fffffffLL && c.n_seg <= 0x7fffffffLL,
               "fr_spmm_plan_sizes: plan too large for 32-bit ids");
    *n_seg = c.n_seg;
    *n_long = c.n_long;
    *n_part = c.n_part;
    return FR_OK;
}

extern "C" int fr_spmm_plan_fill(const int32_t *row_ptr_host, int32_t n_rows, int32_t seg_len, int32_t *seg_host,
                                 int32_t *long_rows_host) {
    FR_REQUIRE(row_ptr_host && seg_host && n_rows >= 0, "fr_spmm_plan_fill: bad argument");
    FR_REQUIRE(seg_len >= 8 && seg_len <= FR_SPMM_SEG, "fr_spmm_plan_fill: seg_len=%d outside [8, %d]", seg_len, FR_SPMM_SEG);
    const int64_t SEG = seg_len;
    const int32_t *rp = row_ptr_host;
    int64_t s = 0, nl = 0, pb = 0;
    struct LongSeg { int32_t key, q[4]; };
    std::vector<LongSeg> lsegs;
    const bool by_position = n_rows >= 262144;
    for (int32_t r = 0; r < n_rows; ++r) {
        const int64_t deg = (int64_t)rp[r + 1] - rp[r];
        if (deg <= SEG) continue;
        FR_REQUIRE(long_rows_host, "fr_spmm_plan_fill: long_rows_host is null but row %d is long", r);
        const int64_t k = (deg + SEG - 1) / SEG;
        const FoldShape f = fold_shape(k);
        const int64_t entries = f.children ? f.children : 1;
        const int64_t parent = nl + entries;
        for (int64_t c = 0; c < entries; ++c) {
            const int64_t first = c * f.per, cnt = std::min<int64_t>(f.per, k - first);
            int32_t *lr = long_rows_host + 4 * (nl + c);
            lr[0] = (int32_t)first;
            lr[1] = (int32_t)cnt;
            lr[2] = (int32_t)pb;
            lr[3] = f.children ? (int32_t)(-(parent + 1)) : r;
            for (int64_t i = first; i < first + cnt; ++i, ++s) {
                LongSeg ls;
                ls.key = by_position ? (int32_t)((i << 16) / k) : 0;
                ls.q[0] = (int32_t)(i - first);
                ls.q[1] = rp[r] + (int32_t)(i * SEG);
                ls.q[2] = (int32_t)std::min<int64_t>(SEG, deg - i * SEG);
                ls.q[3] = (int32_t)(nl + c);
                lsegs.push_back(ls);
            }
            pb += cnt;
        }
        if (f.children) {
            int32_t *lr = long_rows_host + 4 * parent;
            lr[0] = (int32_t)nl;
            lr[1] = (int32_t)f.children;
            lr[2] = (int32_t)pb;
            lr[3] = r;
            pb += f.children;
        }
        nl += entries + (f.children ? 1 : 0);
    }
    std::stable_sort(lsegs.begin(), lsegs.end(), [](const LongSeg &a, const LongSeg &b) { return a.key < b.key; });
    for (size_t i = 0; i < lsegs.size(); ++i)
        for (int j = 0; j < 4; ++j) seg_host[4 * i + j] = lsegs[i].q[j];
    std::vector<int64_t> start((size_t)SEG + 2, 0);
    for (int32_t r = 0; r < n_rows; ++r) {
        const int64_t deg = (int64_t)rp[r + 1] - rp[r];
        if (deg <= SEG) start[SEG - deg + 1] += 1;
    }
    for (int i = 1; i <= SEG + 1; ++i) start[i] += start[i - 1];
    for (int32_t r = 0; r < n_rows; ++r) {
        const int64_t deg = (int64_t)rp[r + 1] - rp[r];
        if (deg > SEG) continue;
        int32_t *q = seg_host + 4 * (s + start[SEG - deg]++);
        q[0] = r;
        q[1] = rp[r];
        q[2] = (int32_t)deg;
        q[3] = -1;
    }
    return FR_OK;
}

static int spmm_entry(const int32_t *seg, int64_t n_seg, const int32_t *long_rows, int64_t n_long,
                      const int32_t *col_idx, const float *val, int32_t d, const float *X0, const float *X1,
                      int32_t x_split, const float *Z0, const float *Z1, int32_t z_split, float alpha,
                      float beta, const float *bias, int32_t act, float *Y, float *partial,
                      int32_t *counters, const uint8_t *x_mask, uint8_t *y_mask, void *stream,
                      float *const *peers_host = nullptr, int32_t n_peers = 0, int64_t row_off = 0) {
    FR_REQUIRE(n_seg >= 0 && n_long >= 0, "fr_spmm_csr_f32: negative extent");
    if (n_seg == 0) return FR_OK;
    FR_REQUIRE(seg && X0 && (Y || n_peers > 0), "fr_spmm_csr_f32: null seg/X/Y");
    FR_REQUIRE(n_long == 0 || (long_rows && partial && counters), "fr_spmm_csr_f32: long rows need workspace");
    FR_REQUIRE(act == 0 || act == 1, "fr_spmm_csr_f32: act must be 0 or 1");
    FR_REQUIRE((((uintptr_t)X0 | (uintptr_t)X1 | (uintptr_t)Y | (uintptr_t)Z0 | (uintptr_t)Z1 | (uintptr_t)bias |
                 (uintptr_t)partial | (uintptr_t)seg | (uintptr_t)long_rows) & 15) == 0,
               "fr_spmm_csr_f32: pointers must be 16-byte aligned");
    FR_REQUIRE(Y == nullptr || (X0 != Y && X1 != Y), "fr_spmm_csr_f32: in-place propagation is not supported");
    FR_REQUIRE(x_split >= 0 && z_split >= 0 && (X1 != nullptr || x_split == 0) && (Z1 == nullptr || Z0 != nullptr),
               "fr_spmm_csr_f32_split: bad split arguments");
    Split sp;
    sp.x_split = X1 ? x_split : 0x7fffffff;
    sp.X1_adj = X1 ? X1 - (size_t)x_split * d : X0;
    sp.z_split = Z1 ? z_split : 0x7fffffff;
    sp.Z1_adj = Z1 ? Z1 - (size_t)z_split * d : Z0;
    FR_REQUIRE(x_mask == nullptr || X1 == nullptr, "fr_spmm_csr_f32_masked: a row mask needs a single-table X");
    sp.x_mask = x_mask;
    sp.y_mask = y_mask;
    FR_REQUIRE(n_peers >= 0 && n_peers <= 8 && row_off >= 0 && (n_peers == 0 || peers_host != nullptr),
               "fr_spmm_csr_f32_push: 1..8 peer tables");
    FR_REQUIRE(n_peers == 0 || (X1 == nullptr && Z1 == nullptr && x_mask == nullptr && y_mask == nullptr && act == 0),
               "fr_spmm_csr_f32_push: single-table operands, no masks, no activation");
    sp.n_peers = n_peers;
    sp.row_off = row_off;
    for (int q = 0; q < 8; ++q) {
        sp.peer[q] = q < n_peers ? peers_host[q] : nullptr;
        FR_REQUIRE(q >= n_peers || (sp.peer[q] != nullptr && ((uintptr_t)sp.peer[q] & 15) == 0 && sp.peer[q] != X0),
                   "fr_spmm_csr_f32_push: peer tables must be non-null, 16-byte aligned and distinct from X");
    }
    cudaStream_t st = (cudaStream_t)stream;
    const int4 *sg = reinterpret_cast<const int4 *>(seg);
    const int4 *lr = reinterpret_cast<const int4 *>(long_rows);
    switch (d) {
        case 32: return launch<32>(sg, n_seg, lr, col_idx, val, X0, Z0, alpha, beta, bias, act, Y, partial, counters, st, sp);
        case 64: return launch<64>(sg, n_seg, lr, col_idx, val, X0, Z0, alpha, beta, bias, act, Y, partial, counters, st, sp);
        case 128: return launch<128>(sg, n_seg, lr, col_idx, val, X0, Z0, alpha, beta, bias, act, Y, partial, counters, st, sp);
        default:
            fr::set_error("fr_spmm_csr_f32: d=%d unsupported (32, 64, 128)", d);
            return FR_EUNSUPPORTED;
    }
}

extern "C" int fr_spmm_csr_f32_split(const int32_t *seg, int64_t n_seg, const int32_t *long_rows, int64_t n_long,
                                     const int32_t *col_idx, const float *val, int32_t d, const float *X0, const float *X1,
                                     int32_t x_split, const float *Z0, const float *Z1, int32_t z_split, float alpha,
                                     float beta, const float *bias, int32_t act, float *Y, float *partial,
                                     int32_t *counters, void *stream) {
    return spmm_entry(seg, n_seg, long_rows, n_long, col_idx, val, d, X0, X1, x_split, Z0, Z1, z_split, alpha, beta, bias, act,
                      Y, partial, counters, nullptr, nullptr, stream);
}

extern "C" int fr_spmm_csr_f32_push(const int32_t *seg, int64_t n_seg, const int32_t *long_rows, int64_t n_long,
                                    const int32_t *col_idx, const float *val, int32_t d, const float *X, const float *Z,
                                    float alpha, float beta, float *Y, float *partial, int32_t *counters,
                                    float *const *peers_host, int32_t n_peers, int64_t row_off, void *stream) {
    FR_REQUIRE(n_peers >= 1, "fr_spmm_csr_f32_push: at least one destination table");
    return spmm_entry(seg, n_seg, long_rows, n_long, col_idx, val, d, X, nullptr, 0, Z, nullptr, 0, alpha, beta, nullptr, 0, Y,
                      partial, counters, nullptr, nullptr, stream, peers_host, n_peers, row_off);
}

extern "C" int fr_spmm_csr_f32_masked(const int32_t *seg, int64_t n_seg, const int32_t *long_rows, int64_t n_long,
                                      const int32_t *col_idx, const float *val, int32_t d, const float *X, const float *Z,
                                      float alpha, float beta, float *Y, float *partial, int32_t *counters,
                                      const uint8_t *x_mask, uint8_t *y_mask, void *stream) {
    return spmm_entry(seg, n_seg, long_rows, n_long, col_idx, val, d, X, nullptr, 0, Z, nullptr, 0, alpha, beta, nullptr, 0, Y,
                      partial, counters, x_mask, y_mask, stream);
}

extern "C" int fr_spmm_csr_f32(const int32_t *seg, int64_t n_seg, const int32_t *long_rows, int64_t n_long,
                               const int32_t *col_idx, const float *val, int32_t d, const float *X, const float *Z,
                               float alpha, float beta, const float *bias, int32_t act, float *Y, float *partial,
                               int32_t *counters, void *stream) {
    return fr_spmm_csr_f32_split(seg, n_seg, long_rows, n_long, col_idx, val, d, X, nullptr, 0, Z, nullptr, 0, alpha, beta,
                                 bias, act, Y, partial, counters, stream);
}

extern "C" int64_t fr_spmm_task_blocks(int64_t n_seg) {
    return (n_seg + 4 * kWarpsPerBlock - 1) / (4 * kWarpsPerBlock);
}

extern "C" int fr_spmm_csr_f32_grouped(const fr_spmm_task *tasks_host, int32_t n_tasks, int32_t d, const int32_t *blk_map,
                                       int64_t n_blocks, void *stream) {
    FR_REQUIRE(tasks_host && n_tasks >= 1 && n_tasks <= FR_SPMM_MAX_TASKS, "fr_spmm_csr_f32_grouped: 1..%d tasks", FR_SPMM_MAX_TASKS);
    FR_REQUIRE(blk_map && n_blocks >= 0 && n_blocks <= 0x7fffffffLL, "fr_spmm_csr_f32_grouped: bad block map");
    if (n_blocks == 0) return FR_OK;
    GroupedParams P;
    int64_t blocks = 0;
    for (int t = 0; t < FR_SPMM_MAX_TASKS; ++t) {
        GroupedTask &T = P.t[t];
        if (t >= n_tasks) {
            T = P.t[0];
            continue;
        }
        const fr_spmm_task &h = tasks_host[t];
        FR_REQUIRE(h.n_seg >= 0 && h.n_long >= 0 && h.seg && h.X0 && h.Y, "fr_spmm_csr_f32_grouped: task %d: null pointer", t);
        FR_REQUIRE(h.n_long == 0 || (h.long_rows && h.partial && h.counters), "fr_spmm_csr_f32_grouped: task %d: long rows need workspace", t);
        FR_REQUIRE((((uintptr_t)h.X0 | (uintptr_t)h.X1 | (uintptr_t)h.Y | (uintptr_t)h.Z0 | (uintptr_t)h.Z1 | (uintptr_t)h.partial |
                     (uintptr_t)h.seg | (uintptr_t)h.long_rows) & 15) == 0, "fr_spmm_csr_f32_grouped: task %d: pointers must be 16-byte aligned", t);
        FR_REQUIRE(h.X0 != h.Y && h.X1 != h.Y, "fr_spmm_csr_f32_grouped: task %d: in-place propagation is not supported", t);
        FR_REQUIRE(h.x_split >= 0 && h.z_split >= 0 && (h.X1 != nullptr || h.x_split == 0) && (h.Z1 == nullptr || h.Z0 != nullptr),
                   "fr_spmm_csr_f32_grouped: task %d: bad split arguments", t);
        T.seg = reinterpret_cast<const int4 *>(h.seg);
        T.n_seg = h.n_seg;
        T.long_rows = reinterpret_cast<const int4 *>(h.long_rows);
        T.col = h.col_idx;
        T.val = h.val;
        T.X = h.X0;
        T.x_split = h.X1 ? h.x_split : 0x7fffffff;
        T.X1_adj = h.X1 ? h.X1 - (size_t)h.x_split * d : h.X0;
        T.Z = h.Z0;
        T.z_split = h.Z1 ? h.z_split : 0x7fffffff;
        T.Z1_adj = h.Z1 ? h.Z1 - (size_t)h.z_split * d : h.Z0;
        T.Y = h.Y;
        T.partial = h.partial;
        T.counters = h.counters;
        T.alpha = h.alpha;
        T.beta = h.beta;
        blocks += fr_spmm_task_blocks(h.n_seg);
    }
    FR_REQUIRE(blocks == n_blocks, "fr_spmm_csr_f32_grouped: block map has %lld entries, the tasks need %lld", (long long)n_blocks,
               (long long)blocks);
    cudaStream_t st = (cudaStream_t)stream;
    const int2 *bm = reinterpret_cast<const int2 *>(blk_map);
    fr::LaunchTimer _lt("spmm_grouped_kernel", st);
    switch (d) {
        case 32: spmm_grouped_kernel<32><<<(unsigned)n_blocks, kWarpsPerBlock * 32, 0, st>>>(P, bm); break;
        case 64: spmm_grouped_kernel<64><<<(unsigned)n_blocks, kWarpsPerBlock * 32, 0, st>>>(P, bm); break;
        case 128: spmm_grouped_kernel<128><<<(unsigned)n_blocks, kWarpsPerBlock * 32, 0, st>>>(P, bm); break;
        default:
            fr::set_error("fr_spmm_csr_f32_grouped: d=%d unsupported (32, 64, 128)", d);
            return FR_EUNSUPPORTED;
    }
    return fr::check_launch("fr_spmm_csr_f32_grouped");
}
```

### multi-modal-food-recommendation_b200/models/pricai_modelx.py

```python
from __future__ import annotations

import numpy as np
import torch
import torch.nn as nn

from .. import graph as G
from .. import ops
from ..common.init import xavier_uniform_initialization
from ..common.loss import BPRLoss, EmbLoss
from ._base import DotProductRecommender


class PRICAI_ModelX(DotProductRecommender):
    def __init__(self, config, dataset):
        super().__init__(config, dataset)
        self.config = config
        self.dataset = dataset
        self.n_ingredients = dataset.num_ingredients
        self.n_cal_level = dataset.num_calories_level
        self.n_health_level = (len(dataset.health_level_multi_hot[0]) if config["use_health_level_multi_hot"]
                               else dataset.num_health_level)
        self.interaction_matrix = dataset.train_coo_matrix
        self.latent_dim = config["embedding_size"]
        self.n_ri_layers = config["n_ri_layers"]
        self.n_mm_layers = config["n_mm_layers"]
        self.n_ui_layers = config["n_ui_layers"]
        self.reg_weight = config["reg_weight"]
        self.loss_cl = config["loss_cl"]
        self.knn_k = config["knn_k"]
        self.mm_image_weight = config["mm_image_weight"]
        self.n_cluster = config["n_cluster"]

        self.user_embedding = nn.Embedding(self.n_users, self.latent_dim)
        self.item_embedding = nn.Embedding(self.n_items, self.latent_dim)
        self.ingre_embedding = nn.Embedding(self.n_ingredients + 1, self.latent_dim, padding_idx=self.n_ingredients)
        self.mf_loss = BPRLoss()
        self.reg_loss = EmbLoss()

        dev = self.device
        self.g_ui = G.norm_adj_user_item(self.interaction_matrix, self.n_users, self.n_items, dev)
        self.g_image = G.norm_adj_item_side(dataset.image_cluster_triples, self.n_items, self.n_cluster, dev)
        self.g_text = G.norm_adj_item_side(dataset.text_cluster_triples, self.n_items, self.n_cluster, dev)
        self.g_ingre = G.norm_adj_item_side(dataset.rIngre_triples, self.n_items, self.n_ingredients, dev)

        self.proj_ingre = nn.Linear(self.latent_dim, self.latent_dim)
        self.proj_text = nn.Linear(self.latent_dim, self.latent_dim)
        self.proj_image = nn.Linear(self.latent_dim, self.latent_dim)
        self.image_prototype_embedding = nn.Embedding(self.n_cluster, self.latent_dim)
        self.text_prototype_embedding = nn.Embedding(self.n_cluster, self.latent_dim)
        self.apply(xavier_uniform_initialization)

        self.v_center = self.t_center = None
        if config["use_center_embedding"]:
            root = config["interaction_data_path"]
            self.v_center = torch.tensor(np.load(root + "mm_cluster/image_center.npy").astype(np.float32)).to(dev)
            self.t_center = torch.tensor(np.load(root + "mm_cluster/text_center.npy").astype(np.float32)).to(dev)
        if self.v_center is not None:
            self.image_prototype_embedding = nn.Embedding.from_pretrained(self.v_center, freeze=False)
            self.image_trs = nn.Linear(self.v_center.shape[1], self.latent_dim)
            nn.init.xavier_normal_(self.image_trs.weight)
        if self.t_center is not None:
            self.text_prototype_embedding = nn.Embedding.from_pretrained(self.t_center, freeze=False)
            self.text_trs = nn.Linear(self.t_center.shape[1], self.latent_dim)
            nn.init.xavier_normal_(self.text_trs.weight)

    def _side_streams(self):
        st = getattr(self, "_streams", None)
        if st is None:
            dev = self.item_embedding.weight.device
            st = self._streams = [torch.cuda.Stream(device=dev) for _ in range(2)]
        return st

    def _propagate_all(self, side_fn=None):
        I = self.n_items
        item_w = self.item_embedding.weight
        cur = torch.cuda.current_stream()
        if getattr(self, "fork_streams", True):
            s1, s2 = self._side_streams()
        else:
            s1 = s2 = cur
        if getattr(self, "group_item_graphs", True):
            image_proto = self.image_prototype_embedding.weight
            if self.v_center is not None:
                image_proto = self.image_trs(image_proto)
            text_proto = self.text_prototype_embedding.weight
            if self.t_center is not None:
                text_proto = self.text_trs(text_proto)
            grp = getattr(self, "_item_group", None)
            if grp is None:
                grp = self._item_group = ops.PropGroup([self.g_ingre, self.g_image, self.g_text])
            ing, img, txt = ops.propagate_mean_grouped(grp, [item_w, item_w, item_w],
                                                       [self.ingre_embedding.weight[:-1], image_proto, text_proto],
                                                       self.n_ri_layers)
        else:
            s1.wait_stream(cur)
            s2.wait_stream(cur)
            ing = ops.propagate_mean(self.g_ingre, item_w, self.n_ri_layers, bottom=self.ingre_embedding.weight[:-1])
            with torch.cuda.stream(s1):
                image_proto = self.image_prototype_embedding.weight
                if self.v_center is not None:
                    image_proto = self.image_trs(image_proto)
                img = ops.propagate_mean(self.g_image, item_w, self.n_ri_layers, bottom=image_proto)
            with torch.cuda.stream(s2):
                text_proto = self.text_prototype_embedding.weight
                if self.t_center is not None:
                    text_proto = self.text_trs(text_proto)
                txt = ops.propagate_mean(self.g_text, item_w, self.n_ri_layers, bottom=text_proto)
            cur.wait_stream(s1)
            cur.wait_stream(s2)
            for t in (img, txt):
                t.record_stream(cur)
        side = None
        if side_fn is not None:
            item_emb, side = side_fn(img, txt, ing)
        else:
            item_emb = ing[:I] + img[:I] + txt[:I]
        all_emb = ops.propagate_mean(self.g_ui, self.user_embedding.weight, self.n_ui_layers, bottom=item_emb)
        if side_fn is not None:
            return all_emb, (img, txt, ing), side
        return all_emb, (img, txt, ing)

    def forward(self):
        all_emb, (img, txt, ing) = self._propagate_all()
        I = self.n_items
        return all_emb[:self.n_users], all_emb[self.n_users:], (img[:I], txt[:I], ing[:I])

    def calculate_loss(self, batch_data):
        user, pos_item, neg_item = batch_data["u_id"], batch_data["pos_i_id"], batch_data["neg_i_id"]
        all_item = torch.cat([pos_item, neg_item], dim=0)
        fork = getattr(self, "fork_streams", True)

        def views(img, txt, ing):
            return ops.item_views([img, txt, ing], all_item, [(0, 1), (0, 2), (2, 1)], self.loss_cl, self.n_items,
                                  side_stream=self._side_streams()[0] if fork else None)
        all_emb, _, cl_loss = self._propagate_all(side_fn=views)
        uw, iw = self.user_embedding.weight, self.item_embedding.weight
        mf_loss_g, reg = ops.rank_loss(all_emb, self.n_users, user, pos_item, neg_item,
                                       [(uw, user), (iw, pos_item), (iw, neg_item)],
                                       reg_den=float(neg_item.shape[0]) / self.reg_weight, gamma=self.mf_loss.gamma)
        if fork:
            cur = torch.cuda.current_stream()
            cur.wait_stream(self._side_streams()[0])
            cl_loss.record_stream(cur)
        return mf_loss_g, cl_loss, reg.reshape(1)

    def CL_loss(self, hidden, hidden_norm=True, temperature=0.5):
        return ops.info_nce(hidden, temperature=temperature, hidden_norm=hidden_norm)

    def correlation_distance(self, x, y):
        return ops.correlation_distance(x, y)
```

### multi-modal-food-recommendation_b200/ops.py

```python
from __future__ import annotations

import ctypes as C

import torch

from . import _lib
from .graph import PropGraph

_L = _lib.lib
PROFILE = None


def _chk_f32(t: torch.Tensor, name: str):
    if t.device.type != "cuda":
        raise _lib.FoodRecError(f"{name} must be a CUDA tensor (foodrec_b200 has no CPU path), got {t.device}")
    if t.dtype != torch.float32 or not t.is_contiguous():
        raise _lib.FoodRecError(f"{name} must be contiguous float32, got {t.dtype} contiguous={t.is_contiguous()}")


def _idx(t: torch.Tensor, name: str) -> torch.Tensor:
    if t.device.type != "cuda":
        raise _lib.FoodRecError(f"{name} must be a CUDA tensor, got {t.device}")
    return t.contiguous() if t.dtype == torch.int64 else t.to(torch.int64).contiguous()


_ROW_MASKS = {}
USE_ROW_MASKS = True


def _register_mask(t: torch.Tensor, mask: torch.Tensor):
    if USE_ROW_MASKS:
        _ROW_MASKS[(t.data_ptr(), tuple(t.shape))] = (t, mask)


def _take_mask(t: torch.Tensor):
    hit = _ROW_MASKS.pop((t.data_ptr(), tuple(t.shape)), None)
    if hit is None:
        return None
    mask = hit[1]
    base = mask._base if mask._base is not None else mask
    base.record_stream(torch.cuda.current_stream())
    return mask


def spmm_masked(graph: PropGraph, X, Z, alpha, beta, x_mask, want_mask: bool):
    d = X.shape[1]
    out = torch.empty((graph.n_rows, d), dtype=torch.float32, device=X.device)
    y_mask = torch.empty(graph.n_rows, dtype=torch.uint8, device=X.device) if want_mask else None
    prof = PROFILE
    if prof is not None:
        ev0 = torch.cuda.Event(enable_timing=True)
        ev0.record()
    _lib.check(_L.fr_spmm_csr_f32_masked(
        graph.seg.data_ptr(), graph.n_seg, graph.long_rows.data_ptr(), graph.n_long, graph.col.data_ptr(),
        graph.val.data_ptr(), d, X.data_ptr(), _lib.ptr(Z), float(alpha), float(beta), out.data_ptr(),
        graph.partial(d).data_ptr(), graph.counters.data_ptr(), x_mask.data_ptr(), _lib.ptr(y_mask),
        _lib.stream_ptr()), "fr_spmm_csr_f32_masked")
    if prof is not None:
        ev1 = torch.cuda.Event(enable_timing=True)
        ev1.record()
        prof.append((ev0, ev1, graph.spmm_bytes(d), graph, Z is not None))
    return out, y_mask


def propagate_mean_masked(graph: PropGraph, g: torch.Tensor, n_layers: int, mask: torch.Tensor):
    inv = 1.0 / (n_layers + 1)
    t, m = g, mask
    for layer in range(n_layers):
        last = layer == n_layers - 1
        t, m = spmm_masked(graph, t, g, inv if last else 1.0, inv if last else 1.0, m, want_mask=True)
    return t, m


def spmm(graph: PropGraph, X: torch.Tensor, Z: torch.Tensor | None = None, alpha: float = 1.0, beta: float = 0.0,
         bias: torch.Tensor | None = None, act: int = 0, out: torch.Tensor | None = None,
         X1: torch.Tensor | None = None, Z1: torch.Tensor | None = None) -> torch.Tensor:
    _chk_f32(X, "X")
    rows = X.shape[0] + (X1.shape[0] if X1 is not None else 0)
    if rows != graph.n_cols:
        raise _lib.FoodRecError(f"X has {rows} rows, graph has {graph.n_cols} columns")
    d = X.shape[1]
    if out is None:
        out = torch.empty((graph.n_rows, d), dtype=torch.float32, device=X.device)
    for t, name in ((X1, "X1"), (Z, "Z"), (Z1, "Z1"), (bias, "bias")):
        if t is not None:
            _chk_f32(t, name)
    if Z is not None and Z.shape[0] + (Z1.shape[0] if Z1 is not None else 0) != graph.n_rows:
        raise _lib.FoodRecError("Z does not have one row per graph row")
    prof = PROFILE
    if prof is not None:
        ev0 = torch.cuda.Event(enable_timing=True)
        ev0.record()
    _lib.check(_L.fr_spmm_csr_f32_split(
        graph.seg.data_ptr(), graph.n_seg, graph.long_rows.data_ptr(), graph.n_long, graph.col.data_ptr(),
        graph.val.data_ptr(), d, X.data_ptr(), _lib.ptr(X1), X.shape[0] if X1 is not None else 0, _lib.ptr(Z), _lib.ptr(Z1),
        Z.shape[0] if (Z is not None and Z1 is not None) else 0, float(alpha), float(beta), _lib.ptr(bias), int(act), out.data_ptr(),
        graph.partial(d).data_ptr(), graph.counters.data_ptr(), _lib.stream_ptr()), "fr_spmm_csr_f32")
    if prof is not None:
        ev1 = torch.cuda.Event(enable_timing=True)
        ev1.record()
        prof.append((ev0, ev1, graph.spmm_bytes(d), graph, Z is not None))
    return out


def propagate_mean_raw(graph: PropGraph, ego: torch.Tensor, n_layers: int, ego1: torch.Tensor | None = None) -> torch.Tensor:
    if n_layers == 0:
        return ego.clone() if ego1 is None else torch.cat((ego, ego1), 0)
    inv = 1.0 / (n_layers + 1)
    t, t1 = ego, ego1
    for layer in range(n_layers):
        last = layer == n_layers - 1
        t = spmm(graph, t, Z=ego, alpha=inv if last else 1.0, beta=inv if last else 1.0, X1=t1, Z1=ego1)
        t1 = None
    return t


class _PropagateMean(torch.autograd.Function):
    @staticmethod
    def forward(ctx, ego, graph, n_layers):
        ctx.graph, ctx.n_layers = graph, n_layers
        return propagate_mean_raw(graph, ego.contiguous(), n_layers)

    @staticmethod
    def backward(ctx, g):
        gt = ctx.graph.T
        if gt is None:
            raise _lib.FoodRecError("graph has no transpose plan; build it with a `.T`")
        g = g.contiguous()
        mask = _take_mask(g) if ctx.n_layers > 0 else None
        if mask is not None:
            r, rm = propagate_mean_masked(gt, g, ctx.n_layers, mask)
            _register_mask(r, rm)
            return r, None, None
        return propagate_mean_raw(gt, g, ctx.n_layers), None, None


class _PropagateMean2(torch.autograd.Function):

    @staticmethod
    def forward(ctx, top, bottom, graph, n_layers):
        ctx.graph, ctx.n_layers, ctx.n_top = graph, n_layers, top.shape[0]
        return propagate_mean_raw(graph, top.contiguous(), n_layers, bottom.contiguous())

    @staticmethod
    def backward(ctx, g):
        gt = ctx.graph.T
        if gt is None:
            raise _lib.FoodRecError("graph has no transpose plan; build it with a `.T`")
        g = g.contiguous()
        mask = _take_mask(g) if ctx.n_layers > 0 else None
        if mask is not None:
            r, rm = propagate_mean_masked(gt, g, ctx.n_layers, mask)
            top, bottom = r[:ctx.n_top], r[ctx.n_top:]
            _register_mask(top, rm[:ctx.n_top])
            _register_mask(bottom, rm[ctx.n_top:])
            return top, bottom, None, None
        r = propagate_mean_raw(gt, g, ctx.n_layers)
        return r[:ctx.n_top], r[ctx.n_top:], None, None


def propagate_mean(graph: PropGraph, ego: torch.Tensor, n_layers: int, bottom: torch.Tensor | None = None) -> torch.Tensor:
    if bottom is None:
        return _PropagateMean.apply(ego, graph, n_layers)
    return _PropagateMean2.apply(ego, bottom, graph, n_layers)


class PropGroup:

    def __init__(self, graphs):
        import numpy as np
        self.graphs = list(graphs)
        if not 1 <= len(self.graphs) <= 4:
            raise _lib.FoodRecError("a PropGroup holds 1..4 graphs")
        nb = [int(_L.fr_spmm_task_blocks(g.n_seg)) for g in self.graphs]
        task = np.concatenate([np.full(n, t, dtype=np.int32) for t, n in enumerate(nb)])
        blk = np.concatenate([np.arange(n, dtype=np.int32) for n in nb])
        key = np.concatenate([(np.arange(n) + 0.5) / max(n, 1) for n in nb])
        order = np.argsort(key, kind="stable")
        self.n_blocks = int(task.size)
        self.blk_map = torch.from_numpy(np.stack([task[order], blk[order]], 1).copy()).to(self.graphs[0].device)
        self._T = None

    @property
    def T(self):
        if self._T is None:
            ts = [g.T for g in self.graphs]
            if any(t is None for t in ts):
                raise _lib.FoodRecError("a graph of the group has no transpose plan")
            self._T = self if all(t is g for t, g in zip(ts, self.graphs)) else PropGroup(ts)
        return self._T


def spmm_grouped(group: PropGroup, Xs, Zs, alpha: float, beta: float, X1s=None, Z1s=None, outs=None):
    n = len(group.graphs)
    X1s = X1s or [None] * n
    Z1s = Z1s or [None] * n
    d = Xs[0].shape[1]
    given, outs, tasks = outs, [], (_lib.SpmmTask * n)()
    prof = PROFILE
    for t, g in enumerate(group.graphs):
        X, X1, Z, Z1 = Xs[t], X1s[t], Zs[t], Z1s[t]
        for a, name in ((X, "X"), (X1, "X1"), (Z, "Z"), (Z1, "Z1")):
            if a is not None:
                _chk_f32(a, name)
        if X.shape[0] + (X1.shape[0] if X1 is not None else 0) != g.n_cols or X.shape[1] != d:
            raise _lib.FoodRecError(f"task {t}: operand rows do not match the graph")
        out = given[t] if given is not None else torch.empty((g.n_rows, d), dtype=torch.float32, device=X.device)
        outs.append(out)
        tk = tasks[t]
        tk.seg, tk.n_seg, tk.long_rows, tk.n_long = g.seg.data_ptr(), g.n_seg, g.long_rows.data_ptr(), g.n_long
        tk.col_idx, tk.val = g.col.data_ptr(), g.val.data_ptr()
        tk.X0, tk.X1, tk.x_split = X.data_ptr(), _lib.ptr(X1), X.shape[0] if X1 is not None else 0
        tk.Z0, tk.Z1 = _lib.ptr(Z), _lib.ptr(Z1)
        tk.z_split = Z.shape[0] if (Z is not None and Z1 is not None) else 0
        tk.alpha, tk.beta = float(alpha), float(beta)
        tk.Y, tk.partial, tk.counters = out.data_ptr(), g.partial(d).data_ptr(), g.counters.data_ptr()
    if prof is not None:
        ev0 = torch.cuda.Event(enable_timing=True)
        ev0.record()
    _lib.check(_L.fr_spmm_csr_f32_grouped(tasks, n, d, group.blk_map.data_ptr(), group.n_blocks, _lib.stream_ptr()),
               "fr_spmm_csr_f32_grouped")
    if prof is not None:
        ev1 = torch.cuda.Event(enable_timing=True)
        ev1.record()
        prof.append((ev0, ev1, sum(g.spmm_bytes(d) for g in group.graphs), group, Zs[0] is not None))
    return outs


def _propagate_mean_grouped_raw(group, tops, bottoms, n_layers):
    inv = 1.0 / (n_layers + 1)
    t, t1 = list(tops), list(bottoms)
    for layer in range(n_layers):
        last = layer == n_layers - 1
        t = spmm_grouped(group, t, list(tops), inv if last else 1.0, inv if last else 1.0, X1s=t1, Z1s=list(bottoms))
        t1 = [None] * len(t)
    return t


class _PropagateMeanGrouped(torch.autograd.Function):

    @staticmethod
    def forward(ctx, group, n_layers, *tabs):
        n = len(group.graphs)
        tops, bottoms = [t.contiguous() for t in tabs[:n]], [t.contiguous() for t in tabs[n:]]
        ctx.group, ctx.n_layers, ctx.n_top = group, n_layers, [t.shape[0] for t in tops]
        ctx.shared_top = n > 1 and all(t.data_ptr() == tops[0].data_ptr() and t.shape == tops[0].shape for t in tops)
        return tuple(_propagate_mean_grouped_raw(group, tops, bottoms, n_layers))

    @staticmethod
    def backward(ctx, *gs):
        gt = ctx.group.T
        gs = list(gs)
        d = next(g.shape[1] for g in gs if g is not None)
        for k, g in enumerate(gs):
            if g is None:
                gr = ctx.group.graphs[k]
                gs[k] = torch.zeros((gr.n_rows, d), dtype=torch.float32, device=gr.device)
            else:
                gs[k] = g.contiguous()
                _take_mask(gs[k])
        r = _propagate_mean_grouped_raw(gt, gs, [None] * len(gs), ctx.n_layers)
        tops = [x[:nt] for x, nt in zip(r, ctx.n_top)]
        bottoms = [x[nt:] for x, nt in zip(r, ctx.n_top)]
        if ctx.shared_top:
            total = torch.empty((ctx.n_top[0], d), dtype=torch.float32, device=r[0].device)
            _lib.check(_L.fr_sum_rows(_ptr_array(r), len(r), d, ctx.n_top[0], total.data_ptr(), _lib.stream_ptr()), "fr_sum_rows")
            tops = [total] + [None] * (len(r) - 1)
        return (None, None, *tops, *bottoms)


def propagate_mean_grouped(group: PropGroup, tops, bottoms, n_layers: int):
    if n_layers == 0:
        return [torch.cat((a, b), 0) for a, b in zip(tops, bottoms)]
    return list(_PropagateMeanGrouped.apply(group, n_layers, *tops, *bottoms))


class _SpmmBiasTanh(torch.autograd.Function):
    @staticmethod
    def forward(ctx, x, bias, graph):
        y = spmm(graph, x.contiguous(), bias=bias.contiguous(), act=1)
        ctx.save_for_backward(y)
        ctx.graph = graph
        return y

    @staticmethod
    def backward(ctx, g):
        (y,) = ctx.saved_tensors
        dpre = (g * (1.0 - y * y)).contiguous()
        return spmm(ctx.graph.T, dpre), dpre.sum(0), None


def gcn_propagate_tanh(graph: PropGraph, h: torch.Tensor, bias: torch.Tensor) -> torch.Tensor:
    return _SpmmBiasTanh.apply(h, bias, graph)


_WS = {}


def _workspace(device) -> torch.Tensor:
    ws = _WS.get(device)
    if ws is None:
        ws = torch.zeros(int(_L.fr_rank_loss_ws_floats()), dtype=torch.float32, device=device)
        _WS[device] = ws
    return ws


def _ptr_array(tensors):
    return (C.c_void_p * max(len(tensors), 1))(*[None if t is None else t.data_ptr() for t in tensors])


class _RankLoss(torch.autograd.Function):

    @staticmethod
    def forward(ctx, emb, item_off, u, p, n, gamma, reg_den, reg_idx, reg_pad, *reg_tabs):
        _chk_f32(emb, "emb")
        B, d = u.numel(), emb.shape[1]
        for t in reg_tabs:
            _chk_f32(t, "regulariser table")
            if t.shape[1] != d:
                raise _lib.FoodRecError("regulariser tables must share the embedding width")
        dev = emb.device
        out = torch.empty(2, dtype=torch.float32, device=dev)
        coef = torch.empty(B, dtype=torch.float32, device=dev)
        gnorm = torch.empty(max(len(reg_tabs), 1), dtype=torch.float32, device=dev)
        cnt = (C.c_int64 * max(len(reg_tabs), 1))(*[int(i.numel()) for i in reg_idx])
        _lib.check(_L.fr_rank_loss_fwd(
            emb.data_ptr(), d, int(item_off), u.data_ptr(), p.data_ptr(), n.data_ptr(), B, float(gamma),
            len(reg_tabs), _ptr_array(reg_tabs), _ptr_array(reg_idx), cnt, float(reg_den), out.data_ptr(),
            coef.data_ptr(), gnorm.data_ptr(), _workspace(dev).data_ptr(), _lib.stream_ptr()), "fr_rank_loss_fwd")
        ctx.save_for_backward(emb, u, p, n, coef, gnorm, *reg_idx, *reg_tabs)
        ctx.meta = (int(item_off), float(reg_den), len(reg_tabs), tuple(int(x) for x in reg_pad))
        return out[0], out[1]

    @staticmethod
    def backward(ctx, g_mf, g_reg):
        item_off, reg_den, ng, pads = ctx.meta
        emb, u, p, n, coef, gnorm = ctx.saved_tensors[:6]
        reg_idx = ctx.saved_tensors[6:6 + ng]
        reg_tabs = ctx.saved_tensors[6 + ng:6 + 2 * ng]
        B, d = u.numel(), emb.shape[1]
        g_out = torch.stack([g_mf.reshape(()), g_reg.reshape(())]).to(torch.float32).contiguous()
        shapes = [emb.shape] if ctx.needs_input_grad[0] else []
        keys = []
        for k, t in enumerate(reg_tabs):
            if ctx.needs_input_grad[9 + k] and t.data_ptr() not in keys:
                keys.append(t.data_ptr())
                shapes.append(t.shape)
        _ROW_MASKS.clear()
        n_flat = sum(sh[0] * sh[1] for sh in shapes)
        want_mask = USE_ROW_MASKS and ctx.needs_input_grad[0]
        n_mask_words = (emb.shape[0] + 3) // 4 if want_mask else 0
        flat = torch.zeros(n_flat + n_mask_words, dtype=torch.float32, device=emb.device)
        emb_mask = flat[n_flat:].view(torch.uint8)[:emb.shape[0]] if want_mask else None
        views, o = [], 0
        for sh in shapes:
            views.append(flat[o:o + sh[0] * sh[1]].view(sh[0], sh[1]))
            o += sh[0] * sh[1]
        d_emb = views.pop(0) if ctx.needs_input_grad[0] else None
        uniq = dict(zip(keys, views))
        d_tabs = [uniq[t.data_ptr()] if ctx.needs_input_grad[9 + k] else None for k, t in enumerate(reg_tabs)]
        cnt = (C.c_int64 * max(ng, 1))(*[int(i.numel()) for i in reg_idx])
        pad = (C.c_int64 * max(ng, 1))(*pads)
        _lib.check(_L.fr_rank_loss_bwd(
            emb.data_ptr(), d, item_off, u.data_ptr(), p.data_ptr(), n.data_ptr(), B, coef.data_ptr(),
            g_out.data_ptr(), _lib.ptr(d_emb), ng, _ptr_array(reg_tabs), _ptr_array(reg_idx), cnt, pad, reg_den,
            gnorm.data_ptr(), _ptr_array(d_tabs), _lib.ptr(emb_mask), _lib.stream_ptr()), "fr_rank_loss_bwd")
        if emb_mask is not None:
            _register_mask(d_emb, emb_mask)
        seen, grads = set(), []
        for k, t in enumerate(reg_tabs):
            if d_tabs[k] is None or t.data_ptr() in seen:
                grads.append(None)
            else:
                seen.add(t.data_ptr())
                grads.append(d_tabs[k])
        return (d_emb, None, None, None, None, None, None, None, None, *grads)


def rank_loss(emb: torch.Tensor, item_off: int, u, p, n, reg_groups, reg_den: float, gamma: float = 1e-10):
    u, p, n = _idx(u, "u"), _idx(p, "p"), _idx(n, "n")
    tabs = [g[0] for g in reg_groups]
    idxs = [_idx(g[1].reshape(-1), "reg idx") for g in reg_groups]
    pads = [(-1 if (len(g) < 3 or g[2] is None) else int(g[2])) for g in reg_groups]
    return _RankLoss.apply(emb, item_off, u, p, n, gamma, reg_den, idxs, pads, *tabs)


class _GatherRows(torch.autograd.Function):
    @staticmethod
    def forward(ctx, tab, idx):
        _chk_f32(tab, "table")
        out = torch.empty((idx.numel(), tab.shape[1]), dtype=torch.float32, device=tab.device)
        _lib.check(_L.fr_gather_rows(tab.data_ptr(), tab.shape[1], idx.data_ptr(), idx.numel(), out.data_ptr(),
                                     _lib.stream_ptr()), "fr_gather_rows")
        ctx.save_for_backward(idx)
        ctx.shape = tab.shape
        return out

    @staticmethod
    def backward(ctx, g):
        (idx,) = ctx.saved_tensors
        d_tab = torch.zeros(ctx.shape, dtype=torch.float32, device=g.device)
        g = g.contiguous()
        _lib.check(_L.fr_scatter_add_rows(g.data_ptr(), g.shape[1], idx.data_ptr(), idx.numel(), d_tab.data_ptr(),
                                          _lib.stream_ptr()), "fr_scatter_add_rows")
        return d_tab, None


def gather_rows(tab: torch.Tensor, idx: torch.Tensor) -> torch.Tensor:
    return _GatherRows.apply(tab.contiguous(), _idx(idx, "idx"))


class _CosineMean(torch.autograd.Function):
    @staticmethod
    def forward(ctx, A, T, idx):
        _chk_f32(A, "A")
        _chk_f32(T, "table")
        n, d, dev = A.shape[0], A.shape[1], A.device
        out = torch.empty(1, dtype=torch.float32, device=dev)
        state = torch.empty((3, n), dtype=torch.float32, device=dev)
        _lib.check(_L.fr_cosine_mean_fwd(A.data_ptr(), T.data_ptr(), idx.data_ptr(), n, d, out.data_ptr(),
                                         state[0].data_ptr(), state[1].data_ptr(), state[2].data_ptr(), _lib.stream_ptr()),
                   "fr_cosine_mean_fwd")
        ctx.save_for_backward(A, T, idx, state)
        return out[0]

    @staticmethod
    def backward(ctx, g):
        A, T, idx, state = ctx.saved_tensors
        n, d = A.shape
        g = g.to(torch.float32).reshape(1).contiguous()
        dA = torch.empty_like(A) if ctx.needs_input_grad[0] else None
        dT = torch.zeros_like(T) if ctx.needs_input_grad[1] else None
        _lib.check(_L.fr_cosine_mean_bwd(A.data_ptr(), T.data_ptr(), idx.data_ptr(), n, d, state[0].data_ptr(),
                                         state[1].data_ptr(), state[2].data_ptr(), g.data_ptr(), _lib.ptr(dA), _lib.ptr(dT),
                                         _lib.stream_ptr()), "fr_cosine_mean_bwd")
        return dA, dT, None


def cosine_mean(A: torch.Tensor, table: torch.Tensor, idx: torch.Tensor) -> torch.Tensor:
    return _CosineMean.apply(A.contiguous(), table.contiguous(), _idx(idx.reshape(-1), "idx"))


def pair_scores(user_tab: torch.Tensor, item_tab: torch.Tensor, user: torch.Tensor, item: torch.Tensor):
    user_tab, item_tab = user_tab.detach(), item_tab.detach()
    if not user_tab.is_contiguous():
        user_tab = user_tab.contiguous()
    if not item_tab.is_contiguous():
        item_tab = item_tab.contiguous()
    _chk_f32(user_tab, "user table")
    _chk_f32(item_tab, "item table")
    user, item = _idx(user, "user"), _idx(item, "item")
    out = torch.empty(user.numel(), dtype=torch.float32, device=user_tab.device)
    _lib.check(_L.fr_pair_scores(user_tab.data_ptr(), item_tab.data_ptr(), user_tab.shape[1], user.data_ptr(),
                                 item.data_ptr(), user.numel(), out.data_ptr(), _lib.stream_ptr()), "fr_pair_scores")
    return out


_DCOR_WS = {}


def _dcor_ws(device, n):
    need = int(_L.fr_dcor_ws_floats(n))
    ws = _DCOR_WS.get(device)
    if ws is None or ws.numel() < need:
        ws = torch.zeros(need, dtype=torch.float32, device=device)
        _DCOR_WS[device] = ws
    return ws


def _dcor_forward(tabs, idx, pairs, scale):
    V, P, n, d = len(tabs), len(pairs), idx.numel(), tabs[0].shape[1]
    for t in tabs:
        _chk_f32(t, "view table")
    dev = tabs[0].device
    Dm = torch.empty((V, n, n), dtype=torch.float32, device=dev)
    rowmean = torch.empty((V, n), dtype=torch.float32, device=dev)
    out = torch.empty(P + 1, dtype=torch.float32, device=dev)
    dfds = torch.empty(3 * P, dtype=torch.float32, device=dev)
    gm = torch.empty(V, dtype=torch.float32, device=dev)
    pr = (C.c_int32 * (2 * P))(*[int(x) for ab in pairs for x in ab])
    _lib.check(_L.fr_dcor_fwd(_ptr_array(tabs), V, d, idx.data_ptr(), n, pr, P, float(scale), Dm.data_ptr(),
                              rowmean.data_ptr(), out.data_ptr(), dfds.data_ptr(), gm.data_ptr(),
                              _dcor_ws(dev, n).data_ptr(), _lib.stream_ptr()), "fr_dcor_fwd")
    return out, (Dm, rowmean, dfds, gm)


def _dcor_backward(tabs, idx, pairs, state, g_terms, d_tabs, masks=None):
    Dm, rowmean, dfds, gm = state
    V, P, n, d = len(tabs), len(pairs), idx.numel(), tabs[0].shape[1]
    pr = (C.c_int32 * (2 * P))(*[x for ab in pairs for x in ab])
    ws = torch.empty(int(_L.fr_dcor_bwd_ws_floats(n)), dtype=torch.float32, device=idx.device)
    _lib.check(_L.fr_dcor_bwd(_ptr_array(tabs), V, d, idx.data_ptr(), n, pr, P, Dm.data_ptr(), rowmean.data_ptr(),
                              dfds.data_ptr(), gm.data_ptr(), g_terms.data_ptr(), _ptr_array(d_tabs),
                              _ptr_array(masks) if masks is not None else None, ws.data_ptr(), _lib.stream_ptr()), "fr_dcor_bwd")


def _term_grads(g_terms, g_total, P):
    if g_terms is None:
        return g_total.to(torch.float32).reshape(1).expand(P).contiguous()
    g = g_terms.to(torch.float32)
    if g_total is not None:
        g = g + g_total.reshape(1)
    return g.contiguous()


class _DcorTerms(torch.autograd.Function):

    @staticmethod
    def forward(ctx, idx, pairs, scale, *tabs):
        pairs = [tuple(int(x) for x in ab) for ab in pairs]
        out, state = _dcor_forward(tabs, idx, pairs, scale)
        ctx.save_for_backward(idx, *state, *tabs)
        ctx.pairs = pairs
        return out[:len(pairs)], out[len(pairs):]

    @staticmethod
    def backward(ctx, g_terms, g_total):
        idx = ctx.saved_tensors[0]
        state, tabs = ctx.saved_tensors[1:5], ctx.saved_tensors[5:]
        g = _term_grads(g_terms, g_total, len(ctx.pairs))
        d_tabs = [torch.zeros_like(t) if ctx.needs_input_grad[3 + k] else None for k, t in enumerate(tabs)]
        _dcor_backward(tabs, idx, ctx.pairs, state, g, d_tabs)
        return (None, None, None, *d_tabs)


def dcor_terms(tabs, idx: torch.Tensor, pairs, scale: float = 1.0, with_total: bool = False):
    terms, total = _DcorTerms.apply(_idx(idx.reshape(-1), "idx"), list(pairs), float(scale), *[t.contiguous() for t in tabs])
    return (terms, total) if with_total else terms


class _GradHolder:

    def __init__(self):
        self.d_tabs = None
        self.masks = None
        self.stream = None
        self.done = False
        self.consumed = False
        self._armed = False

    def arm(self):
        if self._armed:
            return
        self._armed = True

        def _end_of_pass():
            lost = self.done and not self.consumed
            self.d_tabs = self.masks = self.stream = None
            self.done = self.consumed = self._armed = False
            if lost:
                raise _lib.FoodRecError(
                    "ops.item_views: the contrastive total was back-propagated without item_emb in the same backward "
                    "pass, so its table gradients were not delivered. Differentiate the summed loss in one pass, or "
                    "use ops.dcor_terms(...) for a stand-alone contrastive term.")
        torch.autograd.Variable._execution_engine.queue_callback(_end_of_pass)


class _DcorTotalInto(torch.autograd.Function):
    @staticmethod
    def forward(ctx, idx, pairs, scale, holder, *tabs):
        pairs = [tuple(int(x) for x in ab) for ab in pairs]
        out, state = _dcor_forward(tabs, idx, pairs, scale)
        ctx.save_for_backward(idx, *state, *tabs)
        ctx.pairs, ctx.holder = pairs, holder
        return out[len(pairs):]

    @staticmethod
    def backward(ctx, g_total):
        idx = ctx.saved_tensors[0]
        state, tabs = ctx.saved_tensors[1:5], ctx.saved_tensors[5:]
        h = ctx.holder
        h.arm()
        d_tabs = [torch.zeros_like(t) for t in tabs]
        masks = None
        if USE_ROW_MASKS and not h.consumed:
            masks = [torch.zeros(t.shape[0], dtype=torch.uint8, device=t.device) for t in tabs]
        _dcor_backward(tabs, idx, ctx.pairs, state, _term_grads(None, g_total, len(ctx.pairs)), d_tabs, masks)
        if h.consumed:
            return (None, None, None, None, *d_tabs)
        h.d_tabs, h.masks, h.stream, h.done = d_tabs, masks, torch.cuda.current_stream(), True
        return (None, None, None, None) + (None,) * len(tabs)


class _SumRowsInto(torch.autograd.Function):
    @staticmethod
    def forward(ctx, n_items, holder, *tabs):
        d = tabs[0].shape[1]
        for t in tabs:
            _chk_f32(t, "table")
        out = torch.empty((n_items, d), dtype=torch.float32, device=tabs[0].device)
        _lib.check(_L.fr_sum_rows(_ptr_array(tabs), len(tabs), d, n_items, out.data_ptr(), _lib.stream_ptr()), "fr_sum_rows")
        ctx.n_items, ctx.holder = n_items, holder
        ctx.shapes = [tuple(t.shape) for t in tabs]
        ctx.dev = tabs[0].device
        return out

    @staticmethod
    def backward(ctx, g_item):
        h, d = ctx.holder, ctx.shapes[0][1]
        h.arm()
        g_item = g_item.contiguous()
        rows = (C.c_int64 * len(ctx.shapes))(*[int(sh[0]) for sh in ctx.shapes])
        src_mask = _take_mask(g_item)
        if h.done and not h.consumed:
            cur = torch.cuda.current_stream()
            if h.stream is not None and h.stream != cur:
                cur.wait_stream(h.stream)
                for t in h.d_tabs + (h.masks or []):
                    t.record_stream(cur)
            d_tabs, masks, acc = h.d_tabs, h.masks, 1
        else:
            d_tabs, acc = [torch.empty(sh, dtype=torch.float32, device=ctx.dev) for sh in ctx.shapes], 0
            masks = ([torch.empty(sh[0], dtype=torch.uint8, device=ctx.dev) for sh in ctx.shapes]
                     if (USE_ROW_MASKS and src_mask is not None) else None)
        h.consumed = True
        _lib.check(_L.fr_spread_rows(g_item.data_ptr(), d, ctx.n_items, _ptr_array(d_tabs), rows, len(d_tabs), acc,
                                     _lib.ptr(src_mask), _ptr_array(masks) if masks is not None else None,
                                     _lib.stream_ptr()), "fr_spread_rows")
        if masks is not None:
            for t, m in zip(d_tabs, masks):
                _register_mask(t, m)
        return (None, None, *d_tabs)


def item_views(tabs, idx: torch.Tensor, pairs, scale: float, n_items: int, side_stream=None):
    tabs = [t.contiguous() for t in tabs]
    idx = _idx(idx.reshape(-1), "idx")
    holder = _GradHolder()
    item_emb = _SumRowsInto.apply(int(n_items), holder, *tabs)
    if side_stream is None:
        total = _DcorTotalInto.apply(idx, list(pairs), float(scale), holder, *tabs)
    else:
        cur = torch.cuda.current_stream()
        side_stream.wait_stream(cur)
        with torch.cuda.stream(side_stream):
            total = _DcorTotalInto.apply(idx, list(pairs), float(scale), holder, *tabs)
    return item_emb, total


def correlation_distance(x: torch.Tensor, y: torch.Tensor) -> torch.Tensor:
    idx = torch.arange(x.shape[0], device=x.device)
    return dcor_terms([x, y], idx, [(0, 1)])


class _InfoNCE(torch.autograd.Function):
    @staticmethod
    def forward(ctx, hidden, temperature, hidden_norm):
        _chk_f32(hidden, "hidden")
        b, d = hidden.shape[0] // 2, hidden.shape[1]
        n, dev = 2 * b, hidden.device
        hn = torch.empty((n, d), dtype=torch.float32, device=dev)
        norm = torch.empty(n, dtype=torch.float32, device=dev)
        G = torch.empty((n, n), dtype=torch.float32, device=dev)
        lse = torch.empty(n, dtype=torch.float32, device=dev)
        out = torch.empty(1, dtype=torch.float32, device=dev)
        ws = torch.empty(int(_L.fr_infonce_ws_floats(n)), dtype=torch.float32, device=dev)
        _lib.check(_L.fr_infonce_fwd(hidden.data_ptr(), b, d, float(temperature), int(bool(hidden_norm)), hn.data_ptr(),
                                     norm.data_ptr(), G.data_ptr(), lse.data_ptr(), out.data_ptr(), ws.data_ptr(),
                                     _lib.stream_ptr()), "fr_infonce_fwd")
        ctx.save_for_backward(hn, norm, G, lse)
        ctx.meta = (b, d, float(temperature), int(bool(hidden_norm)), hidden.shape[0])
        return out[0]

    @staticmethod
    def backward(ctx, g):
        hn, norm, G, lse = ctx.saved_tensors
        b, d, tau, nrm, rows = ctx.meta
        g = g.to(torch.float32).reshape(1).contiguous()
        dh = torch.empty((rows, d), dtype=torch.float32, device=hn.device)
        if rows > 2 * b:
            dh[2 * b:].zero_()
        _lib.check(_L.fr_infonce_bwd(hn.data_ptr(), norm.data_ptr(), G.data_ptr(), lse.data_ptr(), b, d, tau, nrm,
                                     g.data_ptr(), dh.data_ptr(), _lib.stream_ptr()), "fr_infonce_bwd")
        return dh, None, None


def info_nce(hidden: torch.Tensor, temperature: float = 0.5, hidden_norm: bool = True) -> torch.Tensor:
    return _InfoNCE.apply(hidden.contiguous(), float(temperature), bool(hidden_norm))
```

### multi-modal-food-recommendation_b200/train.py

```python
from __future__ import annotations

import torch


def mark_parameters_updated(model):
    model._param_generation = getattr(model, "_param_generation", 0) + 1
    if getattr(model, "_eval_cache", None) is not None:
        model._eval_cache = None


def eager_step(model, optimizer, batch, grad_hook=None):
    optimizer.zero_grad()
    losses = model.calculate_loss(batch)
    loss = sum(losses) if isinstance(losses, tuple) else losses
    loss.backward()
    if grad_hook is not None:
        grad_hook(model)
    optimizer.step()
    mark_parameters_updated(model)
    return losses


def allreduce_mean_grads(group=None):
    import torch.distributed as dist
    world = dist.get_world_size(group)

    def hook(model):
        for p in model.parameters():
            if p.grad is not None:
                dist.all_reduce(p.grad, group=group)
                p.grad.div_(world)
    return hook


class OverlappedGradAllReduce:

    def __init__(self, model, group=None):
        import torch.distributed as dist
        self.dist, self.group = dist, group
        dev = next(model.parameters()).device
        self.comm = torch.cuda.Stream(device=dev)
        self.handles = [p.register_post_accumulate_grad_hook(self._hook) for p in model.parameters() if p.requires_grad]

    def _hook(self, p):
        cur = torch.cuda.current_stream()
        self.comm.wait_stream(cur)
        with torch.cuda.stream(self.comm):
            self.dist.all_reduce(p.grad, op=self.dist.ReduceOp.AVG, group=self.group)

    def __call__(self, model=None):
        torch.cuda.current_stream().wait_stream(self.comm)

    def remove(self):
        for h in self.handles:
            h.remove()


class FusedAdam(torch.optim.Optimizer):

    def __init__(self, params, lr=1e-3, betas=(0.9, 0.999), eps=1e-8):
        super().__init__(params, dict(lr=lr, betas=betas, eps=eps))
        self._dev_state = {}

    @torch.no_grad()
    def step(self, closure=None):
        from . import _lib
        loss = None
        if closure is not None:
            with torch.enable_grad():
                loss = closure()
        for gi, group in enumerate(self.param_groups):
            ps = [p for p in group["params"] if p.grad is not None]
            if not ps:
                continue
            dev = ps[0].device
            if dev.type != "cuda":
                raise _lib.FoodRecError("FusedAdam needs CUDA parameters (foodrec_b200 has no CPU path)")
            ds = self._dev_state.get(gi)
            if ds is None:
                ds = self._dev_state[gi] = (torch.zeros(1, dtype=torch.int32, device=dev),
                                            torch.zeros(2, dtype=torch.float32, device=dev))
            tensors = (_lib.AdamTensor * len(ps))()
            for t, p in zip(tensors, ps):
                if p.dtype != torch.float32 or not p.is_contiguous() or p.grad.is_sparse:
                    raise _lib.FoodRecError("FusedAdam handles contiguous fp32 parameters with dense gradients")
                st = self.state[p]
                if not st:
                    st["exp_avg"] = torch.zeros_like(p, memory_format=torch.preserve_format)
                    st["exp_avg_sq"] = torch.zeros_like(p, memory_format=torch.preserve_format)
                g = p.grad if p.grad.is_contiguous() else p.grad.contiguous()
                t.param, t.grad, t.exp_avg, t.exp_avg_sq = p.data_ptr(), g.data_ptr(), st["exp_avg"].data_ptr(), st["exp_avg_sq"].data_ptr()
                t.n = p.numel()
            b1, b2 = group["betas"]
            _lib.check(_lib.lib.fr_adam_step(tensors, len(ps), float(group["lr"]), float(b1), float(b2), float(group["eps"]),
                                             ds[0].data_ptr(), ds[1].data_ptr(), _lib.stream_ptr()), "fr_adam_step")
        return loss


class GraphedTrainStep:

    def __init__(self, model, optimizer, example_batch: dict, keys=None, warmup: int = 3, grad_hook=None):
        self.model, self.optimizer = model, optimizer
        dev = next(model.parameters()).device
        self.keys = list(keys) if keys is not None else list(example_batch.keys())
        self.static = {k: torch.empty_like(example_batch[k], device=dev).copy_(example_batch[k]) for k in self.keys}
        side = torch.cuda.Stream(device=dev)
        side.wait_stream(torch.cuda.current_stream(dev))
        with torch.cuda.stream(side):
            for _ in range(warmup):
                eager_step(model, optimizer, self.static, grad_hook)
        torch.cuda.current_stream(dev).wait_stream(side)
        torch.cuda.synchronize(dev)
        self.graph = torch.cuda.CUDAGraph()
        optimizer.zero_grad(set_to_none=True)
        with torch.cuda.graph(self.graph):
            losses = model.calculate_loss(self.static)
            loss = sum(losses) if isinstance(losses, tuple) else losses
            loss.backward()
            if grad_hook is not None:
                grad_hook(model)
            optimizer.step()
            self.losses = losses if isinstance(losses, tuple) else (losses,)
            self.loss_vec = torch.stack([l.detach().reshape(()).float() for l in self.losses])

    def __call__(self, batch: dict):
        for k in self.keys:
            self.static[k].copy_(batch[k], non_blocking=True)
        self.graph.replay()
        mark_parameters_updated(self.model)
        return self.losses

    def loss_values(self):
        return self.loss_vec.tolist()


class DeviceBatchSampler:

    def __init__(self, dataset, batch_size: int, device, seed: int = 0, drop_last: bool = False):
        import numpy as np
        coo = dataset.train_coo_matrix
        self.n_items, self.batch_size, self.device = int(dataset.n_items), int(batch_size), torch.device(device)
        u = np.asarray(coo.row, dtype=np.int64)
        i = np.asarray(coo.col, dtype=np.int64)
        self.users = torch.from_numpy(u).to(self.device)
        self.items = torch.from_numpy(i).to(self.device)
        eu, ei = [u], [i]
        n_users = int(dataset.n_users)
        vt = getattr(dataset, "validTestRatings", None)
        if vt is not None:
            us = np.fromiter((uu for uu, items in vt.items() for _ in items), dtype=np.int64)
            it = np.fromiter((j for items in vt.values() for j in items), dtype=np.int64)
            eu.append(us)
            ei.append(it)
        else:
            for name, owners in (("validRatings", "valid_users"), ("testRatings", "test_users")):
                lists = getattr(dataset, name, None)
                if lists is None:
                    continue
                ids = getattr(dataset, owners, None)
                if ids is None:
                    if len(lists) != n_users:
                        raise ValueError(f"dataset.{name} has {len(lists)} lists for {n_users} users and no "
                                         f"dataset.{owners} to map them: cannot attribute held-out items")
                    ids = np.arange(n_users, dtype=np.int64)
                ids = np.asarray(ids, dtype=np.int64)
                if ids.shape[0] != len(lists):
                    raise ValueError(f"dataset.{owners} and dataset.{name} differ in length")
                lens = np.fromiter((len(x) for x in lists), dtype=np.int64, count=len(lists))
                eu.append(np.repeat(ids, lens))
                ei.append(np.fromiter((j for x in lists for j in x), dtype=np.int64, count=int(lens.sum())))
        keys = np.unique(np.concatenate(eu) * self.n_items + np.concatenate(ei))
        ptr = np.zeros(int(dataset.n_users) + 1, dtype=np.int64)
        np.cumsum(np.bincount(keys // self.n_items, minlength=int(dataset.n_users)), out=ptr[1:])
        self.excl_ptr = torch.from_numpy(ptr).to(self.device)
        self.excl_idx = torch.from_numpy((keys % self.n_items).astype(np.int32)).to(self.device)
        self.seed, self.drop_last, self._step = int(seed), drop_last, 0
        self._fail = torch.zeros(1, dtype=torch.int32, device=self.device)
        self._gen = torch.Generator(device=self.device)
        self._gen.manual_seed(self.seed)

    def __len__(self):
        n = self.users.numel()
        return n // self.batch_size if self.drop_last else -(-n // self.batch_size)

    def negatives(self, users: torch.Tensor) -> torch.Tensor:
        from . import _lib
        users = users.to(self.device, torch.int64).contiguous()
        out = torch.empty_like(users)
        self._step += 1
        _lib.check(_lib.lib.fr_sample_negatives(
            self.excl_ptr.data_ptr(), self.excl_idx.data_ptr(), users.data_ptr(), users.numel(), self.n_items,
            self.seed & (2 ** 64 - 1), self._step, out.data_ptr(), self._fail.data_ptr(), _lib.stream_ptr()),
            "fr_sample_negatives")
        return out

    def failures(self) -> int:
        return int(self._fail.item())

    def __iter__(self):
        perm = torch.randperm(self.users.numel(), device=self.device, generator=self._gen)
        for b in range(len(self)):
            sel = perm[b * self.batch_size:(b + 1) * self.batch_size]
            u = self.users[sel]
            yield {"u_id": u, "pos_i_id": self.items[sel], "neg_i_id": self.negatives(u)}
```

Measured before the change: 0.9037.

## Compact dcor gradients into per-row buffers and fuse them into spread_rows

The dcor backward now writes gradients into a compact (V, n, d) buffer indexed by sampled row, instead of zeroing and atomically accumulating into full-size gradient tables. Those compact rows are then atomically added during the spread_rows pass that already writes the item-table gradients. This removes the full-table zeros_like allocations and a separate accumulate pass. The change also passes separate MF and reg gradient seeds to rank loss so it can produce sparse gradients, and calls backward on the loss terms directly rather than on their sum. In exchange it adds a row-range partitioned spread kernel with a capped grid and a per-row atomic add loop, which could reduce parallelism on large tables.

```diff
diff --git a/include/foodrec_b200.h b/include/foodrec_b200.h
--- a/include/foodrec_b200.h
+++ b/include/foodrec_b200.h
@@ -37,7 +37,8 @@
 int fr_spmm_csr_f32_masked(const int32_t *seg, int64_t n_seg, const int32_t *long_rows, int64_t n_long,
                            const int32_t *col_idx, const float *val, int32_t d, const float *X, const float *Z,
                            float alpha, float beta, float *Y, float *partial, int32_t *counters, const uint8_t *x_mask,
-                           uint8_t *y_mask, void *stream);
+                           uint8_t *y_mask, const uint8_t *z_mask ,
+                           void *stream);
 
 #define FR_SPMM_MAX_TASKS 4
 typedef struct fr_spmm_task {
@@ -65,9 +66,9 @@
                      const int64_t *n, int32_t B, float gamma, int32_t n_groups,
                      const float *const *reg_tab_host, const int64_t *const *reg_idx_host,
                      const int64_t *reg_cnt_host, float reg_den, float *out, float *coef, float *gnorm,
-                     float *ws, void *stream);
+                     float *ws, float *d_emb, uint8_t *emb_mask, int64_t n_rows, void *stream);
 int fr_rank_loss_bwd(const float *emb, int32_t d, int64_t item_off, const int64_t *u, const int64_t *p,
-                     const int64_t *n, int32_t B, const float *coef, const float *g_out, float *d_emb,
+                     const int64_t *n, int32_t B, const float *coef, const float *g_mf, const float *g_reg, float *d_emb,
                      int32_t n_groups, const float *const *reg_tab_host, const int64_t *const *reg_idx_host,
                      const int64_t *reg_cnt_host, const int64_t *reg_pad_host, float reg_den,
                      const float *gnorm, float *const *d_tab_host, uint8_t *emb_mask ,
@@ -84,6 +85,9 @@
                    int32_t n_tabs, int32_t accumulate ,
                    const uint8_t *src_mask ,
                    uint8_t *const *mask_host , void *stream);
+int fr_spread_rows_add(const float *g, int32_t d, int64_t rows, float *const *d_tab_host, const int64_t *rows_total_host,
+                       int32_t n_tabs, int32_t accumulate, const uint8_t *src_mask, uint8_t *const *mask_host,
+                       const float *const *add_host, const int64_t *add_idx, int32_t n_add, void *stream);
 
 int fr_gather_rows(const float *tab, int32_t d, const int64_t *idx, int64_t n, float *out, void *stream);
 int fr_scatter_add_rows(const float *g, int32_t d, const int64_t *idx, int64_t n, float *d_tab, void *stream);
@@ -100,6 +104,10 @@
                 uint8_t *const *mask_host ,
                 float *ws , void *stream);
 int64_t fr_dcor_bwd_ws_floats(int32_t n);
+int fr_dcor_bwd_rows(const float *const *tab_host, int32_t V, int32_t d, const int64_t *idx, int32_t n,
+                     const int32_t *pairs_host, int32_t P, const float *Dm, const float *rowmean,
+                     const float *dfds, const float *gm, const float *g_out, float *const *d_rows_host,
+                     float *ws, void *stream);
 
 int fr_f32_to_bf16(const float *x, void *y_bf16, int64_t rows, int32_t d, int32_t l2_normalise, void *stream);
 int64_t fr_gemm_topk_ws_bytes(int32_t M);
diff --git a/multi-modal-food-recommendation_b200/_lib.py b/multi-modal-food-recommendation_b200/_lib.py
--- a/multi-modal-food-recommendation_b200/_lib.py
+++ b/multi-modal-food-recommendation_b200/_lib.py
@@ -39,17 +39,21 @@
     "fr_spmm_csr_f32_grouped": (C.c_int, [_p, _i32, _i32, _p, _i64, _p]),
     "fr_adam_step": (C.c_int, [_p, _i32, C.c_double, C.c_double, C.c_double, C.c_double, _p, _p, _p]),
     "fr_rank_loss_ws_floats": (_i64, []),
-    "fr_rank_loss_fwd": (C.c_int, [_p, _i32, _i64, _p, _p, _p, _i32, _f32, _i32, _p, _p, _p, _f32, _p, _p, _p, _p, _p]),
-    "fr_rank_loss_bwd": (C.c_int, [_p, _i32, _i64, _p, _p, _p, _i32, _p, _p, _p, _i32, _p, _p, _p, _p, _f32, _p, _p, _p, _p]),
+    "fr_rank_loss_fwd": (C.c_int, [_p, _i32, _i64, _p, _p, _p, _i32, _f32, _i32, _p, _p, _p, _f32, _p, _p, _p, _p, _p, _p, _i64,
+                                   _p]),
+    "fr_rank_loss_bwd": (C.c_int, [_p, _i32, _i64, _p, _p, _p, _i32, _p, _p, _p, _p, _i32, _p, _p, _p, _p, _f32, _p, _p, _p,
+                                   _p]),
     "fr_bpr_scores_fwd": (C.c_int, [_p, _p, _i64, _f32, _p, _p, _p]),
     "fr_l2_norm_f32": (C.c_int, [_p, _i64, _p, _p]),
-    "fr_spmm_csr_f32_masked": (C.c_int, [_p, _i64, _p, _i64, _p, _p, _i32, _p, _p, _f32, _f32, _p, _p, _p, _p, _p, _p]),
+    "fr_spmm_csr_f32_masked": (C.c_int, [_p, _i64, _p, _i64, _p, _p, _i32, _p, _p, _f32, _f32, _p, _p, _p, _p, _p, _p, _p]),
     "fr_dcor_ws_floats": (_i64, [_i32]),
     "fr_dcor_fwd": (C.c_int, [_p, _i32, _i32, _p, _i32, _p, _i32, _f32, _p, _p, _p, _p, _p, _p, _p]),
     "fr_sum_rows": (C.c_int, [_p, _i32, _i32, _i64, _p, _p]),
     "fr_spread_rows": (C.c_int, [_p, _i32, _i64, _p, _p, _i32, _i32, _p, _p, _p]),
     "fr_dcor_bwd": (C.c_int, [_p, _i32, _i32, _p, _i32, _p, _i32, _p, _p, _p, _p, _p, _p, _p, _p, _p]),
     "fr_dcor_bwd_ws_floats": (_i64, [_i32]),
+    "fr_dcor_bwd_rows": (C.c_int, [_p, _i32, _i32, _p, _i32, _p, _i32, _p, _p, _p, _p, _p, _p, _p, _p]),
+    "fr_spread_rows_add": (C.c_int, [_p, _i32, _i64, _p, _p, _i32, _i32, _p, _p, _p, _p, _i32, _p]),
     "fr_f32_to_bf16": (C.c_int, [_p, _p, _i64, _i32, _i32, _p]),
     "fr_gemm_topk_ws_bytes": (_i64, [_i32]),
     "fr_gemm_topk_bf16": (C.c_int, [_p, _i32, _p, _i32, _i32, _f32, _p, _p, _p, _p, _i32, _p, _p, _p, _i64, _p]),
diff --git a/multi-modal-food-recommendation_b200/csrc/dcor.cu b/multi-modal-food-recommendation_b200/csrc/dcor.cu
--- a/multi-modal-food-recommendation_b200/csrc/dcor.cu
+++ b/multi-modal-food-recommendation_b200/csrc/dcor.cu
@@ -14,6 +14,7 @@
     float *dtab[kMaxV];
     unsigned char *mask[kMaxV];
     int V;
+    int compact;
 };
 struct Pairs {
     int a[kMaxP], b[kMaxP];
@@ -199,10 +200,16 @@
 __global__ void __launch_bounds__(kThreads)
 dcor_w_kernel(int V, Pairs pr, int n, const float *__restrict__ Dm, const float *__restrict__ rowmean,
               const float *__restrict__ gm, const float *__restrict__ dfds, const float *__restrict__ g_out,
-              float *__restrict__ W, float *__restrict__ wsum) {
+              float *__restrict__ W, float *__restrict__ wsum, Views vw, int d) {
     __shared__ float Cm[kMaxV][kMaxV];
     __shared__ float gms[kMaxV];
     __shared__ float red[kThreads / 32];
+    if (vw.compact)
+        for (int v = 0; v < V; ++v) {
+            if (vw.dtab[v] == nullptr) continue;
+            const int r0 = blockIdx.x * kRB2, r1 = min(n, r0 + kRB2);
+            for (int e = threadIdx.x; e < (r1 - r0) * d; e += kThreads) vw.dtab[v][(size_t)r0 * d + e] = 0.f;
+        }
     if (threadIdx.x == 0) {
         float c[kMaxV][kMaxV] = {};
         const float inv = 1.f / ((float)n * (float)n);
@@ -330,6 +337,7 @@
         const int i = i0 + orow + a;
         if (i >= n) continue;
         const size_t row = (size_t)__ldg(idx + i);
+        const size_t drow = vw.compact ? (size_t)i : row;
         float4 o = make_float4(-4.f * acc[a].x, -4.f * acc[a].y, -4.f * acc[a].z, -4.f * acc[a].w);
         if (blockIdx.z == 0) {
             const float w4 = 4.f * __ldg(wsum + (size_t)v * n + i);
@@ -340,13 +348,14 @@
             o.w = fmaf(w4, xi.w, o.w);
             if (vw.mask[v] != nullptr && okq == 0) vw.mask[v][row] = 1;
         }
-        atomicAdd(reinterpret_cast<float4 *>(dtab + row * D + 4 * okq), o);
+        atomicAdd(reinterpret_cast<float4 *>(dtab + drow * D + 4 * okq), o);
     }
 }
 
 int fill(Views &vw, Pairs &pr, int V, const float *const *tab, float *const *dtab, int P, const int32_t *pairs) {
     FR_REQUIRE(V >= 1 && V <= kMaxV && P >= 1 && P <= kMaxP && tab && pairs, "dcor: V=%d P=%d out of range", V, P);
     vw.V = V;
+    vw.compact = 0;
     for (int v = 0; v < kMaxV; ++v) {
         vw.tab[v] = v < V ? tab[v] : nullptr;
         vw.dtab[v] = (v < V && dtab) ? dtab[v] : nullptr;
@@ -404,15 +413,16 @@
 
 extern "C" int64_t fr_dcor_bwd_ws_floats(int32_t n) { return (int64_t)kMaxV * n * n + (int64_t)kMaxV * n; }
 
-extern "C" int fr_dcor_bwd(const float *const *tab_host, int32_t V, int32_t d, const int64_t *idx, int32_t n,
-                           const int32_t *pairs_host, int32_t P, const float *Dm, const float *rowmean,
-                           const float *dfds, const float *gm, const float *g_out, float *const *d_tab_host,
-                           uint8_t *const *mask_host, float *ws, void *stream) {
+static int dcor_bwd(const float *const *tab_host, int32_t V, int32_t d, const int64_t *idx, int32_t n,
+                    const int32_t *pairs_host, int32_t P, const float *Dm, const float *rowmean, const float *dfds,
+                    const float *gm, const float *g_out, float *const *d_tab_host, uint8_t *const *mask_host, float *ws,
+                    int compact, void *stream) {
     FR_REQUIRE(idx && Dm && rowmean && dfds && gm && g_out && d_tab_host && ws && n > 0, "fr_dcor_bwd: bad argument");
     FR_REQUIRE(((uintptr_t)ws & 15) == 0, "fr_dcor_bwd: workspace must be 16-byte aligned");
     Views vw;
     Pairs pr;
     if (int rc = fill(vw, pr, V, tab_host, d_tab_host, P, pairs_host)) return rc;
+    vw.compact = compact;
     for (int v = 0; v < V; ++v)
         FR_REQUIRE(vw.dtab[v] == nullptr || ((uintptr_t)vw.dtab[v] & 15) == 0, "fr_dcor_bwd: gradient tables must be 16-byte aligned");
     if (mask_host)
@@ -421,7 +431,7 @@
     float *W = ws, *wsum = ws + (size_t)kMaxV * n * n;
     {
         fr::LaunchTimer _lt("dcor_w_kernel", st);
-        dcor_w_kernel<<<(n + kRB2 - 1) / kRB2, kThreads, 0, st>>>(V, pr, n, Dm, rowmean, gm, dfds, g_out, W, wsum);
+        dcor_w_kernel<<<(n + kRB2 - 1) / kRB2, kThreads, 0, st>>>(V, pr, n, Dm, rowmean, gm, dfds, g_out, W, wsum, vw, d);
         if (int rc = fr::check_launch("fr_dcor_bwd/w")) return rc;
     }
     dim3 g((n + 31) / 32, V, 8);
@@ -434,3 +444,17 @@
     }
     return fr::check_launch("fr_dcor_bwd");
 }
+
+extern "C" int fr_dcor_bwd(const float *const *tab_host, int32_t V, int32_t d, const int64_t *idx, int32_t n,
+                           const int32_t *pairs_host, int32_t P, const float *Dm, const float *rowmean,
+                           const float *dfds, const float *gm, const float *g_out, float *const *d_tab_host,
+                           uint8_t *const *mask_host, float *ws, void *stream) {
+    return dcor_bwd(tab_host, V, d, idx, n, pairs_host, P, Dm, rowmean, dfds, gm, g_out, d_tab_host, mask_host, ws, 0, stream);
+}
+
+extern "C" int fr_dcor_bwd_rows(const float *const *tab_host, int32_t V, int32_t d, const int64_t *idx, int32_t n,
+                                const int32_t *pairs_host, int32_t P, const float *Dm, const float *rowmean,
+                                const float *dfds, const float *gm, const float *g_out, float *const *d_rows_host,
+                                float *ws, void *stream) {
+    return dcor_bwd(tab_host, V, d, idx, n, pairs_host, P, Dm, rowmean, dfds, gm, g_out, d_rows_host, nullptr, ws, 1, stream);
+}
diff --git a/multi-modal-food-recommendation_b200/csrc/gather.cu b/multi-modal-food-recommendation_b200/csrc/gather.cu
--- a/multi-modal-food-recommendation_b200/csrc/gather.cu
+++ b/multi-modal-food-recommendation_b200/csrc/gather.cu
@@ -122,6 +122,7 @@
     const float *in[4];
     float *out[4];
     unsigned char *mask[4];
+    const float *add[4];
     long long rows_total[4];
     int n;
 };
@@ -133,30 +134,43 @@
     }
 }
 __global__ void spread_rows_kernel(Tabs4 t, long long n4_src, const float *__restrict__ g, int accumulate,
-                                   const unsigned char *__restrict__ src_mask, int d4) {
+                                   const unsigned char *__restrict__ src_mask, int d4, const int64_t *__restrict__ add_idx,
+                                   int n_add) {
     const int v = blockIdx.y;
     float4 *dst = reinterpret_cast<float4 *>(t.out[v]);
     if (dst == nullptr) return;
+    const long long rows_src = n4_src / d4, rows_tot = t.rows_total[v] / d4;
+    const long long R = accumulate ? rows_src : rows_tot;
+    const long long per = (R + gridDim.x - 1) / gridDim.x;
+    const long long r0 = blockIdx.x * per, r1 = min(R, r0 + per);
+    if (r0 >= r1) return;
     if (t.mask[v] != nullptr) {
-        const long long rows_src = n4_src / d4, rows_tot = t.rows_total[v] / d4;
-        for (long long r = (long long)blockIdx.x * blockDim.x + threadIdx.x; r < (accumulate ? rows_src : rows_tot);
-             r += (long long)gridDim.x * blockDim.x) {
+        for (long long r = r0 + threadIdx.x; r < r1; r += blockDim.x) {
             const unsigned char m = r < rows_src ? (src_mask ? src_mask[r] : (unsigned char)1) : (unsigned char)0;
             if (accumulate) { if (m) t.mask[v][r] = 1; }
             else t.mask[v][r] = m;
         }
     }
     if (accumulate) {
-        for (long long i = (long long)blockIdx.x * blockDim.x + threadIdx.x; i < n4_src; i += (long long)gridDim.x * blockDim.x) {
+        for (long long i = r0 * d4 + threadIdx.x; i < r1 * d4; i += blockDim.x) {
             float4 a = dst[i];
             fr::add4(a, fr::ldg_f4(g + 4 * i));
             dst[i] = a;
         }
         return;
     }
-    const long long tot4 = t.rows_total[v];
-    for (long long i = (long long)blockIdx.x * blockDim.x + threadIdx.x; i < tot4; i += (long long)gridDim.x * blockDim.x)
+    for (long long i = r0 * d4 + threadIdx.x; i < r1 * d4; i += blockDim.x)
         dst[i] = i < n4_src ? fr::ldg_f4(g + 4 * i) : make_float4(0.f, 0.f, 0.f, 0.f);
+    const float *add = t.add[v];
+    if (add == nullptr) return;
+    __syncthreads();
+    for (int i = threadIdx.x; i < n_add; i += blockDim.x) {
+        const long long r = __ldg(add_idx + i);
+        if (r < r0 || r >= r1) continue;
+        for (int q = 0; q < d4; ++q)
+            atomicAdd(dst + r * d4 + q, fr::ldg_f4(add + ((size_t)i * d4 + q) * 4));
+        if (t.mask[v] != nullptr) t.mask[v][r] = 1;
+    }
 }
 }
 
@@ -175,11 +189,14 @@
     return fr::check_launch("fr_sum_rows");
 }
 
-extern "C" int fr_spread_rows(const float *g, int32_t d, int64_t rows, float *const *d_tab_host, const int64_t *rows_total_host,
-                              int32_t n_tabs, int32_t accumulate, const uint8_t *src_mask, uint8_t *const *mask_host,
-                              void *stream) {
+extern "C" int fr_spread_rows_add(const float *g, int32_t d, int64_t rows, float *const *d_tab_host,
+                                  const int64_t *rows_total_host, int32_t n_tabs, int32_t accumulate, const uint8_t *src_mask,
+                                  uint8_t *const *mask_host, const float *const *add_host, const int64_t *add_idx, int32_t n_add,
+                                  void *stream) {
     FR_REQUIRE(n_tabs >= 1 && n_tabs <= 4 && d > 0 && d % 4 == 0 && rows >= 0 && g && d_tab_host && rows_total_host,
                "fr_spread_rows: bad argument");
+    FR_REQUIRE(n_add >= 0 && (n_add == 0 || (add_host && add_idx && !accumulate)),
+               "fr_spread_rows_add: compact rows need their indices and accumulate = 0");
     Tabs4 t{};
     t.n = n_tabs;
     long long mx = 0;
@@ -187,13 +204,24 @@
         FR_REQUIRE(rows_total_host[v] >= rows, "fr_spread_rows: table %d shorter than the source", v);
         t.out[v] = d_tab_host[v];
         t.mask[v] = mask_host ? mask_host[v] : nullptr;
+        t.add[v] = n_add > 0 ? add_host[v] : nullptr;
+        FR_REQUIRE(t.add[v] == nullptr || ((uintptr_t)t.add[v] & 15) == 0, "fr_spread_rows_add: rows of table %d not 16-byte aligned", v);
         t.rows_total[v] = rows_total_host[v] * (d / 4);
         mx = std::max(mx, t.rows_total[v]);
     }
     if (mx == 0) return FR_OK;
+    const int grid = n_add > 0 ? std::min(grid1d(mx, 256), fr::num_sms() * 4) : grid1d(mx, 256);
     fr::LaunchTimer _lt("spread_rows_kernel", (cudaStream_t)stream);
-    spread_rows_kernel<<<dim3(grid1d(mx, 256), n_tabs), 256, 0, (cudaStream_t)stream>>>(t, rows * (d / 4), g, accumulate, src_mask, d / 4);
+    spread_rows_kernel<<<dim3(grid, n_tabs), 256, 0, (cudaStream_t)stream>>>(t, rows * (d / 4), g, accumulate, src_mask, d / 4,
+                                                                             add_idx, n_add);
     return fr::check_launch("fr_spread_rows");
+}
+
+extern "C" int fr_spread_rows(const float *g, int32_t d, int64_t rows, float *const *d_tab_host, const int64_t *rows_total_host,
+                              int32_t n_tabs, int32_t accumulate, const uint8_t *src_mask, uint8_t *const *mask_host,
+                              void *stream) {
+    return fr_spread_rows_add(g, d, rows, d_tab_host, rows_total_host, n_tabs, accumulate, src_mask, mask_host, nullptr, nullptr,
+                              0, stream);
 }
 
 namespace {
diff --git a/multi-modal-food-recommendation_b200/csrc/rank_loss.cu b/multi-modal-food-recommendation_b200/csrc/rank_loss.cu
--- a/multi-modal-food-recommendation_b200/csrc/rank_loss.cu
+++ b/multi-modal-food-recommendation_b200/csrc/rank_loss.cu
@@ -23,7 +23,8 @@
 rank_loss_fwd_kernel(const float *__restrict__ emb, int d, long long item_off, const int64_t *__restrict__ u,
                      const int64_t *__restrict__ p, const int64_t *__restrict__ n, int B, float gamma, Groups g,
                      float reg_den, float *__restrict__ out, float *__restrict__ coef, float *__restrict__ gnorm,
-                     float *__restrict__ ws) {
+                     float *__restrict__ ws, float *__restrict__ d_emb, unsigned char *__restrict__ emb_mask,
+                     long long n_rows) {
     __shared__ float sh[kWarps][1 + FR_MAX_REG_GROUPS];
     __shared__ int last;
     const int lane = threadIdx.x & 31, wib = threadIdx.x >> 5;
@@ -32,6 +33,9 @@
     float part[1 + FR_MAX_REG_GROUPS];
 #pragma unroll
     for (int i = 0; i <= FR_MAX_REG_GROUPS; ++i) part[i] = 0.f;
+    if (emb_mask != nullptr)
+        for (long long r = (long long)blockIdx.x * blockDim.x + threadIdx.x; r < n_rows; r += (long long)gridDim.x * blockDim.x)
+            emb_mask[r] = 0;
 
     for (long long t = (long long)blockIdx.x * kWarps + wib; t < n_tasks; t += warps_total) {
         if (t < B) {
@@ -44,6 +48,12 @@
                 x = fmaf(uv, __ldg(pe + k) - __ldg(ne + k), x);
             }
             x = fr::warp_sum(x);
+            if (d_emb != nullptr)
+                for (int k = lane; k < d; k += 32) {
+                    d_emb[(size_t)u[t] * d + k] = 0.f;
+                    d_emb[(size_t)(item_off + p[t]) * d + k] = 0.f;
+                    d_emb[(size_t)(item_off + n[t]) * d + k] = 0.f;
+                }
             const float sg = 1.f / (1.f + expf(-x));
             part[0] += -logf(gamma + sg);
             if (lane == 0) coef[t] = -(sg * (1.f - sg)) / ((gamma + sg) * (float)B);
@@ -99,12 +109,13 @@
 __global__ void __launch_bounds__(kWarps * 32)
 rank_loss_bwd_kernel(const float *__restrict__ emb, int d, long long item_off, const int64_t *__restrict__ u,
                      const int64_t *__restrict__ p, const int64_t *__restrict__ n, int B,
-                     const float *__restrict__ coef, const float *__restrict__ g_out, float *__restrict__ d_emb,
+                     const float *__restrict__ coef, const float *__restrict__ g_mf_p, const float *__restrict__ g_reg_p,
+                     float *__restrict__ d_emb,
                      Groups g, float reg_den, const float *__restrict__ gnorm, unsigned char *__restrict__ emb_mask) {
     const int lane = threadIdx.x & 31, wib = threadIdx.x >> 5;
     const long long n_tasks = B + g.start[g.n];
     const long long warps_total = (long long)gridDim.x * kWarps;
-    const float g_mf = __ldg(g_out), g_reg = __ldg(g_out + 1);
+    const float g_mf = __ldg(g_mf_p), g_reg = __ldg(g_reg_p);
     for (long long t = (long long)blockIdx.x * kWarps + wib; t < n_tasks; t += warps_total) {
         if (t < B) {
             if (d_emb == nullptr) continue;
@@ -201,33 +212,37 @@
                                 const int64_t *n, int32_t B, float gamma, int32_t n_groups,
                                 const float *const *reg_tab_host, const int64_t *const *reg_idx_host,
                                 const int64_t *reg_cnt_host, float reg_den, float *out, float *coef, float *gnorm,
-                                float *ws, void *stream) {
+                                float *ws, float *d_emb, uint8_t *emb_mask, int64_t n_rows, void *stream) {
     FR_REQUIRE(emb && u && p && n && out && coef && gnorm && ws, "fr_rank_loss_fwd: null pointer");
     FR_REQUIRE(B > 0 && d > 0, "fr_rank_loss_fwd: B=%d d=%d", B, d);
+    FR_REQUIRE((d_emb == nullptr && emb_mask == nullptr) || (d_emb != nullptr && emb_mask != nullptr && n_rows > 0),
+               "fr_rank_loss_fwd: d_emb and emb_mask are cleared together");
     Groups g;
     if (int rc = fill_groups(g, n_groups, reg_tab_host, reg_idx_host, reg_cnt_host, nullptr, nullptr)) return rc;
     const int grid = grid_for(B + g.start[g.n]);
     fr::LaunchTimer _lt("rank_loss_fwd_kernel", (cudaStream_t)stream);
     rank_loss_fwd_kernel<<<grid, kWarps * 32, 0, (cudaStream_t)stream>>>(emb, d, item_off, u, p, n, B, gamma, g,
-                                                                         reg_den, out, coef, gnorm, ws);
+                                                                         reg_den, out, coef, gnorm, ws, d_emb, emb_mask,
+                                                                         n_rows);
     return fr::check_launch("fr_rank_loss_fwd");
 }
 
 extern "C" int fr_rank_loss_bwd(const float *emb, int32_t d, int64_t item_off, const int64_t *u, const int64_t *p,
-                                const int64_t *n, int32_t B, const float *coef, const float *g_out, float *d_emb,
+                                const int64_t *n, int32_t B, const float *coef, const float *g_mf, const float *g_reg,
+                                float *d_emb,
                                 int32_t n_groups, const float *const *reg_tab_host,
                                 const int64_t *const *reg_idx_host, const int64_t *reg_cnt_host,
                                 const int64_t *reg_pad_host, float reg_den, const float *gnorm,
                                 float *const *d_tab_host, uint8_t *emb_mask, void *stream) {
-    FR_REQUIRE(emb && u && p && n && coef && g_out && gnorm, "fr_rank_loss_bwd: null pointer");
+    FR_REQUIRE(emb && u && p && n && coef && g_mf && g_reg && gnorm, "fr_rank_loss_bwd: null pointer");
     FR_REQUIRE(B > 0 && d > 0, "fr_rank_loss_bwd: B=%d d=%d", B, d);
     Groups g;
     if (int rc = fill_groups(g, n_groups, reg_tab_host, reg_idx_host, reg_cnt_host, reg_pad_host, d_tab_host))
         return rc;
     const int grid = grid_for(B + g.start[g.n]);
     fr::LaunchTimer _lt("rank_loss_bwd_kernel", (cudaStream_t)stream);
-    rank_loss_bwd_kernel<<<grid, kWarps * 32, 0, (cudaStream_t)stream>>>(emb, d, item_off, u, p, n, B, coef, g_out,
-                                                                         d_emb, g, reg_den, gnorm, emb_mask);
+    rank_loss_bwd_kernel<<<grid, kWarps * 32, 0, (cudaStream_t)stream>>>(emb, d, item_off, u, p, n, B, coef, g_mf,
+                                                                         g_reg, d_emb, g, reg_den, gnorm, emb_mask);
     return fr::check_launch("fr_rank_loss_bwd");
 }
 
diff --git a/multi-modal-food-recommendation_b200/csrc/spmm.cu b/multi-modal-food-recommendation_b200/csrc/spmm.cu
--- a/multi-modal-food-recommendation_b200/csrc/spmm.cu
+++ b/multi-modal-food-recommendation_b200/csrc/spmm.cu
@@ -19,6 +19,7 @@
     int z_split;
     const unsigned char *x_mask;
     unsigned char *y_mask;
+    const unsigned char *z_mask;
     float *peer[8];
     int n_peers;
     long long row_off;
@@ -119,11 +120,12 @@
     if (s.w == -2) return;
     const unsigned gmask = (LPR == 32) ? 0xffffffffu : (((1u << LPR) - 1u) << (g * LPR));
     if (s.w < 0) {
+        const bool z_row = Z != nullptr && (!MASKED || sp.z_mask == nullptr || sp.z_mask[s.x] != 0);
         bool nz = false;
 #pragma unroll
         for (int t = 0; t < VPL; ++t)
-            nz |= epilogue_store<D, ACT, PUSH>(acc[t], s.x, 4 * (lg + LPR * t),
-                                               (Z != nullptr && s.x >= sp.z_split) ? sp.Z1_adj : Z, alpha, beta, bias, Y, &sp);
+            nz |= epilogue_store<D, ACT, PUSH>(acc[t], s.x, 4 * (lg + LPR * t), z_row ? (s.x >= sp.z_split ? sp.Z1_adj : Z) : nullptr,
+                                               alpha, beta, bias, Y, &sp);
         if (sp.y_mask != nullptr) {
             nz = __any_sync(gmask, nz);
             if (lg == 0) sp.y_mask[s.x] = nz ? 1 : 0;
@@ -168,10 +170,11 @@
         lr = pr;
     }
     bool nz_long = false;
+    const bool z_row = Z != nullptr && (!MASKED || sp.z_mask == nullptr || sp.z_mask[lr.w] != 0);
 #pragma unroll
     for (int t = 0; t < VPL; ++t)
-        nz_long |= epilogue_store<D, ACT, PUSH>(acc[t], lr.w, 4 * (lg + LPR * t),
-                                                (Z != nullptr && lr.w >= sp.z_split) ? sp.Z1_adj : Z, alpha, beta, bias, Y, &sp);
+        nz_long |= epilogue_store<D, ACT, PUSH>(acc[t], lr.w, 4 * (lg + LPR * t), z_row ? (lr.w >= sp.z_split ? sp.Z1_adj : Z) : nullptr,
+                                                alpha, beta, bias, Y, &sp);
     if (sp.y_mask != nullptr) {
         nz_long = __any_sync(gmask, nz_long);
         if (lg == 0) sp.y_mask[lr.w] = nz_long ? 1 : 0;
@@ -217,6 +220,7 @@
     sp.z_split = T.z_split;
     sp.x_mask = nullptr;
     sp.y_mask = nullptr;
+    sp.z_mask = nullptr;
     sp.n_peers = 0;
     sp.row_off = 0;
     const long long w = (long long)m.y * kWarpsPerBlock + (threadIdx.x >> 5);
@@ -385,7 +389,8 @@
                       int32_t x_split, const float *Z0, const float *Z1, int32_t z_split, float alpha,
                       float beta, const float *bias, int32_t act, float *Y, float *partial,
                       int32_t *counters, const uint8_t *x_mask, uint8_t *y_mask, void *stream,
-                      float *const *peers_host = nullptr, int32_t n_peers = 0, int64_t row_off = 0) {
+                      float *const *peers_host = nullptr, int32_t n_peers = 0, int64_t row_off = 0,
+                      const uint8_t *z_mask = nullptr) {
     FR_REQUIRE(n_seg >= 0 && n_long >= 0, "fr_spmm_csr_f32: negative extent");
     if (n_seg == 0) return FR_OK;
     FR_REQUIRE(seg && X0 && (Y || n_peers > 0), "fr_spmm_csr_f32: null seg/X/Y");
@@ -403,8 +408,10 @@
     sp.z_split = Z1 ? z_split : 0x7fffffff;
     sp.Z1_adj = Z1 ? Z1 - (size_t)z_split * d : Z0;
     FR_REQUIRE(x_mask == nullptr || X1 == nullptr, "fr_spmm_csr_f32_masked: a row mask needs a single-table X");
+    FR_REQUIRE(z_mask == nullptr || (x_mask != nullptr && Z1 == nullptr), "fr_spmm_csr_f32_masked: z_mask needs x_mask and a single-table Z");
     sp.x_mask = x_mask;
     sp.y_mask = y_mask;
+    sp.z_mask = z_mask;
     FR_REQUIRE(n_peers >= 0 && n_peers <= 8 && row_off >= 0 && (n_peers == 0 || peers_host != nullptr),
                "fr_spmm_csr_f32_push: 1..8 peer tables");
     FR_REQUIRE(n_peers == 0 || (X1 == nullptr && Z1 == nullptr && x_mask == nullptr && y_mask == nullptr && act == 0),
@@ -450,9 +457,9 @@
 extern "C" int fr_spmm_csr_f32_masked(const int32_t *seg, int64_t n_seg, const int32_t *long_rows, int64_t n_long,
                                       const int32_t *col_idx, const float *val, int32_t d, const float *X, const float *Z,
                                       float alpha, float beta, float *Y, float *partial, int32_t *counters,
-                                      const uint8_t *x_mask, uint8_t *y_mask, void *stream) {
+                                      const uint8_t *x_mask, uint8_t *y_mask, const uint8_t *z_mask, void *stream) {
     return spmm_entry(seg, n_seg, long_rows, n_long, col_idx, val, d, X, nullptr, 0, Z, nullptr, 0, alpha, beta, nullptr, 0, Y,
-                      partial, counters, x_mask, y_mask, stream);
+                      partial, counters, x_mask, y_mask, stream, nullptr, 0, 0, z_mask);
 }
 
 extern "C" int fr_spmm_csr_f32(const int32_t *seg, int64_t n_seg, const int32_t *long_rows, int64_t n_long,
diff --git a/multi-modal-food-recommendation_b200/models/pricai_modelx.py b/multi-modal-food-recommendation_b200/models/pricai_modelx.py
--- a/multi-modal-food-recommendation_b200/models/pricai_modelx.py
+++ b/multi-modal-food-recommendation_b200/models/pricai_modelx.py
@@ -137,7 +137,8 @@
         uw, iw = self.user_embedding.weight, self.item_embedding.weight
         mf_loss_g, reg = ops.rank_loss(all_emb, self.n_users, user, pos_item, neg_item,
                                        [(uw, user), (iw, pos_item), (iw, neg_item)],
-                                       reg_den=float(neg_item.shape[0]) / self.reg_weight, gamma=self.mf_loss.gamma)
+                                       reg_den=float(neg_item.shape[0]) / self.reg_weight, gamma=self.mf_loss.gamma,
+                                       sole_consumer=True)
         if fork:
             cur = torch.cuda.current_stream()
             cur.wait_stream(self._side_streams()[0])
diff --git a/multi-modal-food-recommendation_b200/ops.py b/multi-modal-food-recommendation_b200/ops.py
--- a/multi-modal-food-recommendation_b200/ops.py
+++ b/multi-modal-food-recommendation_b200/ops.py
@@ -43,7 +43,7 @@
     return mask
 
 
-def spmm_masked(graph: PropGraph, X, Z, alpha, beta, x_mask, want_mask: bool):
+def spmm_masked(graph: PropGraph, X, Z, alpha, beta, x_mask, want_mask: bool, z_mask=None):
     d = X.shape[1]
     out = torch.empty((graph.n_rows, d), dtype=torch.float32, device=X.device)
     y_mask = torch.empty(graph.n_rows, dtype=torch.uint8, device=X.device) if want_mask else None
@@ -54,7 +54,7 @@
     _lib.check(_L.fr_spmm_csr_f32_masked(
         graph.seg.data_ptr(), graph.n_seg, graph.long_rows.data_ptr(), graph.n_long, graph.col.data_ptr(),
         graph.val.data_ptr(), d, X.data_ptr(), _lib.ptr(Z), float(alpha), float(beta), out.data_ptr(),
-        graph.partial(d).data_ptr(), graph.counters.data_ptr(), x_mask.data_ptr(), _lib.ptr(y_mask),
+        graph.partial(d).data_ptr(), graph.counters.data_ptr(), x_mask.data_ptr(), _lib.ptr(y_mask), _lib.ptr(z_mask),
         _lib.stream_ptr()), "fr_spmm_csr_f32_masked")
     if prof is not None:
         ev1 = torch.cuda.Event(enable_timing=True)
@@ -68,7 +68,7 @@
     t, m = g, mask
     for layer in range(n_layers):
         last = layer == n_layers - 1
-        t, m = spmm_masked(graph, t, g, inv if last else 1.0, inv if last else 1.0, m, want_mask=True)
+        t, m = spmm_masked(graph, t, g, inv if last else 1.0, inv if last else 1.0, m, want_mask=True, z_mask=mask)
     return t, m
 
 
@@ -160,9 +160,9 @@
 
 
 def propagate_mean(graph: PropGraph, ego: torch.Tensor, n_layers: int, bottom: torch.Tensor | None = None) -> torch.Tensor:
-    if bottom is None:
-        return _PropagateMean.apply(ego, graph, n_layers)
-    return _PropagateMean2.apply(ego, bottom, graph, n_layers)
+    out = _PropagateMean.apply(ego, graph, n_layers) if bottom is None else _PropagateMean2.apply(ego, bottom, graph, n_layers)
+    out._fr_reads_masked_rows_only = n_layers > 0 and USE_ROW_MASKS
+    return out
 
 
 class PropGroup:
@@ -312,7 +312,7 @@
 class _RankLoss(torch.autograd.Function):
 
     @staticmethod
-    def forward(ctx, emb, item_off, u, p, n, gamma, reg_den, reg_idx, reg_pad, *reg_tabs):
+    def forward(ctx, emb, item_off, u, p, n, gamma, reg_den, reg_idx, reg_pad, sparse_grad, *reg_tabs):
         _chk_f32(emb, "emb")
         B, d = u.numel(), emb.shape[1]
         for t in reg_tabs:
@@ -324,10 +324,15 @@
         coef = torch.empty(B, dtype=torch.float32, device=dev)
         gnorm = torch.empty(max(len(reg_tabs), 1), dtype=torch.float32, device=dev)
         cnt = (C.c_int64 * max(len(reg_tabs), 1))(*[int(i.numel()) for i in reg_idx])
+        ctx.d_emb = ctx.emb_mask = None
+        if sparse_grad and ctx.needs_input_grad[0]:
+            ctx.d_emb = torch.empty_like(emb)
+            ctx.emb_mask = torch.empty(emb.shape[0], dtype=torch.uint8, device=dev)
         _lib.check(_L.fr_rank_loss_fwd(
             emb.data_ptr(), d, int(item_off), u.data_ptr(), p.data_ptr(), n.data_ptr(), B, float(gamma),
             len(reg_tabs), _ptr_array(reg_tabs), _ptr_array(reg_idx), cnt, float(reg_den), out.data_ptr(),
-            coef.data_ptr(), gnorm.data_ptr(), _workspace(dev).data_ptr(), _lib.stream_ptr()), "fr_rank_loss_fwd")
+            coef.data_ptr(), gnorm.data_ptr(), _workspace(dev).data_ptr(), _lib.ptr(ctx.d_emb), _lib.ptr(ctx.emb_mask),
+            emb.shape[0], _lib.stream_ptr()), "fr_rank_loss_fwd")
         ctx.save_for_backward(emb, u, p, n, coef, gnorm, *reg_idx, *reg_tabs)
         ctx.meta = (int(item_off), float(reg_den), len(reg_tabs), tuple(int(x) for x in reg_pad))
         return out[0], out[1]
@@ -339,31 +344,33 @@
         reg_idx = ctx.saved_tensors[6:6 + ng]
         reg_tabs = ctx.saved_tensors[6 + ng:6 + 2 * ng]
         B, d = u.numel(), emb.shape[1]
-        g_out = torch.stack([g_mf.reshape(()), g_reg.reshape(())]).to(torch.float32).contiguous()
-        shapes = [emb.shape] if ctx.needs_input_grad[0] else []
+        g_mf, g_reg = (g.to(torch.float32).contiguous() for g in (g_mf, g_reg))
+        sparse = ctx.d_emb is not None
+        shapes = [emb.shape] if (ctx.needs_input_grad[0] and not sparse) else []
         keys = []
         for k, t in enumerate(reg_tabs):
-            if ctx.needs_input_grad[9 + k] and t.data_ptr() not in keys:
+            if ctx.needs_input_grad[10 + k] and t.data_ptr() not in keys:
                 keys.append(t.data_ptr())
                 shapes.append(t.shape)
         _ROW_MASKS.clear()
         n_flat = sum(sh[0] * sh[1] for sh in shapes)
-        want_mask = USE_ROW_MASKS and ctx.needs_input_grad[0]
+        want_mask = USE_ROW_MASKS and ctx.needs_input_grad[0] and not sparse
         n_mask_words = (emb.shape[0] + 3) // 4 if want_mask else 0
-        flat = torch.zeros(n_flat + n_mask_words, dtype=torch.float32, device=emb.device)
-        emb_mask = flat[n_flat:].view(torch.uint8)[:emb.shape[0]] if want_mask else None
+        flat = torch.zeros(n_flat + n_mask_words, dtype=torch.float32, device=emb.device) if n_flat + n_mask_words else None
+        emb_mask = flat[n_flat:].view(torch.uint8)[:emb.shape[0]] if want_mask else ctx.emb_mask
         views, o = [], 0
         for sh in shapes:
             views.append(flat[o:o + sh[0] * sh[1]].view(sh[0], sh[1]))
             o += sh[0] * sh[1]
-        d_emb = views.pop(0) if ctx.needs_input_grad[0] else None
+        d_emb = ctx.d_emb if sparse else (views.pop(0) if ctx.needs_input_grad[0] else None)
+        ctx.d_emb = ctx.emb_mask = None
         uniq = dict(zip(keys, views))
-        d_tabs = [uniq[t.data_ptr()] if ctx.needs_input_grad[9 + k] else None for k, t in enumerate(reg_tabs)]
+        d_tabs = [uniq[t.data_ptr()] if ctx.needs_input_grad[10 + k] else None for k, t in enumerate(reg_tabs)]
         cnt = (C.c_int64 * max(ng, 1))(*[int(i.numel()) for i in reg_idx])
         pad = (C.c_int64 * max(ng, 1))(*pads)
         _lib.check(_L.fr_rank_loss_bwd(
             emb.data_ptr(), d, item_off, u.data_ptr(), p.data_ptr(), n.data_ptr(), B, coef.data_ptr(),
-            g_out.data_ptr(), _lib.ptr(d_emb), ng, _ptr_array(reg_tabs), _ptr_array(reg_idx), cnt, pad, reg_den,
+            g_mf.data_ptr(), g_reg.data_ptr(), _lib.ptr(d_emb), ng, _ptr_array(reg_tabs), _ptr_array(reg_idx), cnt, pad, reg_den,
             gnorm.data_ptr(), _ptr_array(d_tabs), _lib.ptr(emb_mask), _lib.stream_ptr()), "fr_rank_loss_bwd")
         if emb_mask is not None:
             _register_mask(d_emb, emb_mask)
@@ -374,15 +381,17 @@
             else:
                 seen.add(t.data_ptr())
                 grads.append(d_tabs[k])
-        return (d_emb, None, None, None, None, None, None, None, None, *grads)
-
-
-def rank_loss(emb: torch.Tensor, item_off: int, u, p, n, reg_groups, reg_den: float, gamma: float = 1e-10):
+        return (d_emb, None, None, None, None, None, None, None, None, None, *grads)
+
+
+def rank_loss(emb: torch.Tensor, item_off: int, u, p, n, reg_groups, reg_den: float, gamma: float = 1e-10,
+              sole_consumer: bool = False):
     u, p, n = _idx(u, "u"), _idx(p, "p"), _idx(n, "n")
     tabs = [g[0] for g in reg_groups]
     idxs = [_idx(g[1].reshape(-1), "reg idx") for g in reg_groups]
     pads = [(-1 if (len(g) < 3 or g[2] is None) else int(g[2])) for g in reg_groups]
-    return _RankLoss.apply(emb, item_off, u, p, n, gamma, reg_den, idxs, pads, *tabs)
+    sparse_grad = sole_consumer and bool(getattr(emb, "_fr_reads_masked_rows_only", False)) and USE_ROW_MASKS
+    return _RankLoss.apply(emb, item_off, u, p, n, gamma, reg_den, idxs, pads, sparse_grad, *tabs)
 
 
 class _GatherRows(torch.autograd.Function):
@@ -485,14 +494,14 @@
     return out, (Dm, rowmean, dfds, gm)
 
 
-def _dcor_backward(tabs, idx, pairs, state, g_terms, d_tabs, masks=None):
+def _dcor_backward(tabs, idx, pairs, state, g_terms, d_tabs):
     Dm, rowmean, dfds, gm = state
     V, P, n, d = len(tabs), len(pairs), idx.numel(), tabs[0].shape[1]
     pr = (C.c_int32 * (2 * P))(*[x for ab in pairs for x in ab])
     ws = torch.empty(int(_L.fr_dcor_bwd_ws_floats(n)), dtype=torch.float32, device=idx.device)
     _lib.check(_L.fr_dcor_bwd(_ptr_array(tabs), V, d, idx.data_ptr(), n, pr, P, Dm.data_ptr(), rowmean.data_ptr(),
-                              dfds.data_ptr(), gm.data_ptr(), g_terms.data_ptr(), _ptr_array(d_tabs),
-                              _ptr_array(masks) if masks is not None else None, ws.data_ptr(), _lib.stream_ptr()), "fr_dcor_bwd")
+                              dfds.data_ptr(), gm.data_ptr(), g_terms.data_ptr(), _ptr_array(d_tabs), None, ws.data_ptr(),
+                              _lib.stream_ptr()), "fr_dcor_bwd")
 
 
 def _term_grads(g_terms, g_total, P):
@@ -532,8 +541,8 @@
 class _GradHolder:
 
     def __init__(self):
-        self.d_tabs = None
-        self.masks = None
+        self.d_rows = None
+        self.idx = None
         self.stream = None
         self.done = False
         self.consumed = False
@@ -546,7 +555,7 @@
 
         def _end_of_pass():
             lost = self.done and not self.consumed
-            self.d_tabs = self.masks = self.stream = None
+            self.d_rows = self.idx = self.stream = None
             self.done = self.consumed = self._armed = False
             if lost:
                 raise _lib.FoodRecError(
@@ -571,14 +580,20 @@
         state, tabs = ctx.saved_tensors[1:5], ctx.saved_tensors[5:]
         h = ctx.holder
         h.arm()
-        d_tabs = [torch.zeros_like(t) for t in tabs]
-        masks = None
-        if USE_ROW_MASKS and not h.consumed:
-            masks = [torch.zeros(t.shape[0], dtype=torch.uint8, device=t.device) for t in tabs]
-        _dcor_backward(tabs, idx, ctx.pairs, state, _term_grads(None, g_total, len(ctx.pairs)), d_tabs, masks)
+        g = _term_grads(None, g_total, len(ctx.pairs))
         if h.consumed:
+            d_tabs = [torch.zeros_like(t) for t in tabs]
+            _dcor_backward(tabs, idx, ctx.pairs, state, g, d_tabs)
             return (None, None, None, None, *d_tabs)
-        h.d_tabs, h.masks, h.stream, h.done = d_tabs, masks, torch.cuda.current_stream(), True
+        Dm, rowmean, dfds, gm = state
+        V, P, n, d = len(tabs), len(ctx.pairs), idx.numel(), tabs[0].shape[1]
+        d_rows = torch.empty((V, n, d), dtype=torch.float32, device=idx.device)
+        pr = (C.c_int32 * (2 * P))(*[x for ab in ctx.pairs for x in ab])
+        ws = torch.empty(int(_L.fr_dcor_bwd_ws_floats(n)), dtype=torch.float32, device=idx.device)
+        _lib.check(_L.fr_dcor_bwd_rows(_ptr_array(tabs), V, d, idx.data_ptr(), n, pr, P, Dm.data_ptr(), rowmean.data_ptr(),
+                                       dfds.data_ptr(), gm.data_ptr(), g.data_ptr(), _ptr_array(list(d_rows)), ws.data_ptr(),
+                                       _lib.stream_ptr()), "fr_dcor_bwd_rows")
+        h.d_rows, h.idx, h.stream, h.done = d_rows, idx, torch.cuda.current_stream(), True
         return (None, None, None, None) + (None,) * len(tabs)
 
 
@@ -602,21 +617,21 @@
         g_item = g_item.contiguous()
         rows = (C.c_int64 * len(ctx.shapes))(*[int(sh[0]) for sh in ctx.shapes])
         src_mask = _take_mask(g_item)
+        d_tabs = [torch.empty(sh, dtype=torch.float32, device=ctx.dev) for sh in ctx.shapes]
+        add, add_idx, n_add = None, None, 0
         if h.done and not h.consumed:
             cur = torch.cuda.current_stream()
             if h.stream is not None and h.stream != cur:
                 cur.wait_stream(h.stream)
-                for t in h.d_tabs + (h.masks or []):
-                    t.record_stream(cur)
-            d_tabs, masks, acc = h.d_tabs, h.masks, 1
-        else:
-            d_tabs, acc = [torch.empty(sh, dtype=torch.float32, device=ctx.dev) for sh in ctx.shapes], 0
-            masks = ([torch.empty(sh[0], dtype=torch.uint8, device=ctx.dev) for sh in ctx.shapes]
-                     if (USE_ROW_MASKS and src_mask is not None) else None)
+                h.d_rows.record_stream(cur)
+                h.idx.record_stream(cur)
+            add, add_idx, n_add = _ptr_array(list(h.d_rows)), h.idx.data_ptr(), h.idx.numel()
+        masks = ([torch.empty(sh[0], dtype=torch.uint8, device=ctx.dev) for sh in ctx.shapes]
+                 if (USE_ROW_MASKS and (src_mask is not None or n_add)) else None)
         h.consumed = True
-        _lib.check(_L.fr_spread_rows(g_item.data_ptr(), d, ctx.n_items, _ptr_array(d_tabs), rows, len(d_tabs), acc,
-                                     _lib.ptr(src_mask), _ptr_array(masks) if masks is not None else None,
-                                     _lib.stream_ptr()), "fr_spread_rows")
+        _lib.check(_L.fr_spread_rows_add(g_item.data_ptr(), d, ctx.n_items, _ptr_array(d_tabs), rows, len(d_tabs), 0,
+                                         _lib.ptr(src_mask), _ptr_array(masks) if masks is not None else None,
+                                         add, add_idx, n_add, _lib.stream_ptr()), "fr_spread_rows_add")
         if masks is not None:
             for t, m in zip(d_tabs, masks):
                 _register_mask(t, m)
diff --git a/multi-modal-food-recommendation_b200/train.py b/multi-modal-food-recommendation_b200/train.py
--- a/multi-modal-food-recommendation_b200/train.py
+++ b/multi-modal-food-recommendation_b200/train.py
@@ -107,16 +107,18 @@
         side = torch.cuda.Stream(device=dev)
         side.wait_stream(torch.cuda.current_stream(dev))
         with torch.cuda.stream(side):
-            for _ in range(warmup):
-                eager_step(model, optimizer, self.static, grad_hook)
+            for _ in range(max(warmup, 1)):
+                out = eager_step(model, optimizer, self.static, grad_hook)
         torch.cuda.current_stream(dev).wait_stream(side)
         torch.cuda.synchronize(dev)
+        self.seeds = [torch.ones_like(t) for t in (out if isinstance(out, tuple) else (out,))]
         self.graph = torch.cuda.CUDAGraph()
         optimizer.zero_grad(set_to_none=True)
         with torch.cuda.graph(self.graph):
             losses = model.calculate_loss(self.static)
-            loss = sum(losses) if isinstance(losses, tuple) else losses
-            loss.backward()
+            terms = losses if isinstance(losses, tuple) else (losses,)
+            diff = [(t, s) for t, s in zip(terms, self.seeds) if t.requires_grad]
+            torch.autograd.backward([t for t, _ in diff], grad_tensors=[s for _, s in diff])
             if grad_hook is not None:
                 grad_hook(model)
             optimizer.step()
```

After: 0.9785 (median of 6 runs). 1.08x the previous value.
